# alibaba-damo-academy/Inferix

Measured on AMD Instinct MI355X. Metric: latent_frames_per_sec, higher is better.
Workload: dtype bf16; 1 GPU; Self-Forcing 480p bf16 (Wan2.1-T2V-1.3B causal DiT, 30 layers), block_size=3, 21 latent frames = 7 blocks x (4 denoise + 1 context) generator forwards, KV prefix 4680..32760 keys in the KV manager's cache (identity page map; page-table form: `streaming_steady`); `value` counts the generator calls (SURVEY 8d), the per-block VAE decode of config 2 is measured beside it under --full (`per_block_decod; batch=1, parallelism=single, layers=30, pair_forwards=True, pair_mode=streams

## Files before the change

### include/inferix_hip.h

```cpp
#ifndef INFERIX_HIP_H
#define INFERIX_HIP_H

#include <stdint.h>

#ifdef __cplusplus
extern "C" {
#endif

#define IFX_OK 0
#define IFX_EINVAL (-1)
#define IFX_ELAUNCH (-2)
#define IFX_EUNSUP (-3)

typedef uint16_t ifx_bf16;

#define IFX_ABI_MINOR 7
int ifx_version(void);
const char* ifx_last_error(void);
const char* ifx_arch(void);
int ifx_set_option(const char* key, int32_t value);
int ifx_get_option(const char* key, int32_t* value);
int32_t ifx_device_error(int32_t clear);

typedef struct {
  ifx_bf16* k;
  ifx_bf16* v;
  const int32_t* page_table;
  int32_t page_size;
  int32_t num_slots;
  int32_t kv_heads;
  int32_t head_dim;
  int32_t seg_split;
  int32_t seg_delta;
} ifx_kv_view;

int ifx_attn_fwd_paged(const ifx_bf16* q, ifx_bf16* out, float* lse, const ifx_kv_view* kv,
                       int32_t q_rows, int32_t heads, int32_t kv_start, int32_t kv_len, float scale,
                       void* stream);

int32_t ifx_attn_split_plan(int32_t q_rows, int32_t heads, int32_t kv_start, int32_t kv_len,
                            int64_t* workspace_bytes);
int ifx_attn_fwd_paged_split(const ifx_bf16* q, ifx_bf16* out, float* lse, const ifx_kv_view* kv,
                             int32_t q_rows, int32_t heads, int32_t kv_start, int32_t kv_len, float scale,
                             int32_t num_splits, void* workspace, int64_t workspace_bytes, void* stream);

int ifx_attn_fwd_paged_ld(const ifx_bf16* q, int32_t ldq, ifx_bf16* out, int32_t ldo, float* lse, const ifx_kv_view* kv,
                          int32_t q_rows, int32_t heads, int32_t kv_start, int32_t kv_len, float scale, int32_t num_splits,
                          void* workspace, int64_t workspace_bytes, void* stream);

int ifx_attn_fwd_dedup(const ifx_bf16* q, ifx_bf16* out, const ifx_kv_view* kv, int32_t q_rows, int32_t heads, int32_t kv_len,
                       int32_t last_key_multiplicity, float scale, void* stream);

int ifx_attn_fwd_ranges(const ifx_bf16* q, int32_t ldq, ifx_bf16* out, int32_t ldo, const ifx_kv_view* kv, int32_t q_rows,
                        int32_t heads, int32_t n_ranges, const int32_t* q_ranges, const int32_t* k_ranges, float scale,
                        void* stream);

int ifx_attn_fwd_partial(const ifx_bf16* q, const ifx_kv_view* kv, int32_t q_rows, int32_t heads, int32_t kv_start,
                         int32_t kv_len, float scale, int32_t num_splits, void* workspace, int64_t workspace_bytes,
                         int32_t slot_base, int32_t slot_cap, int32_t* slots_used, void* stream);
int ifx_attn_merge_partials(const void* workspace, int32_t slot_cap, int32_t slots_used, ifx_bf16* out, float* lse,
                            int32_t q_rows, int32_t heads, void* stream);

int ifx_lse_merge(ifx_bf16* out_a, float* lse_a, const ifx_bf16* out_b, const float* lse_b,
                  int32_t rows, int32_t heads, void* stream);

typedef struct {
  const double* freqs;
  int32_t max_pos;
  int32_t start_frame;
  int32_t height, width;
  int32_t hw_offset;
  int32_t hw_local;
  float q_scale;
  int32_t flags;
} ifx_rope_grid;

int ifx_rmsnorm_rope_kv_append(const ifx_bf16* qkv, int32_t qkv_row_stride, ifx_bf16* q_out,
                               const ifx_bf16* wq, const ifx_bf16* wk, const ifx_rope_grid* rope,
                               const ifx_kv_view* kv, int32_t local_start, int32_t rows,
                               int32_t dim, float eps, void* stream);

int ifx_rmsnorm(const ifx_bf16* x, int32_t x_row_stride, ifx_bf16* y, int32_t y_row_stride,
                const ifx_bf16* w, int32_t rows, int32_t dim, float eps, void* stream);

enum { IFX_LN_PLAIN = 0, IFX_LN_AFFINE = 1, IFX_LN_MODULATE = 2 };
int ifx_layernorm(const ifx_bf16* x, ifx_bf16* y, int32_t rows, int32_t dim, float eps, int32_t mode,
                  const ifx_bf16* gamma, const ifx_bf16* beta, const ifx_bf16* mod,
                  int32_t mod_slots, int32_t shift_slot, int32_t scale_slot, int32_t rows_per_group,
                  void* stream);

enum { IFX_EPI_BIAS = 0, IFX_EPI_GELU_TANH = 1, IFX_EPI_RESIDUAL = 2, IFX_EPI_GATE_RES = 3, IFX_EPI_GELU_ERF = 4 };
typedef struct {
  int32_t epilogue;
  const ifx_bf16* residual;
  int32_t ld_res;
  const ifx_bf16* mod;
  int32_t mod_slots;
  int32_t gate_slot;
  int32_t rows_per_group;
  ifx_bf16* y2;
  int32_t ldy2;
  int32_t split_col;
} ifx_epilogue;
int ifx_gemm_bf16(const ifx_bf16* x, int32_t ldx, const ifx_bf16* w, const ifx_bf16* bias,
                  ifx_bf16* y, int32_t ldy, int32_t M, int32_t N, int32_t K,
                  const ifx_epilogue* epi, void* stream);

int64_t ifx_gemm_workspace_bytes(int32_t M, int32_t N, int32_t K);
int ifx_gemm_bf16_ws(const ifx_bf16* x, int32_t ldx, const ifx_bf16* w, const ifx_bf16* bias, ifx_bf16* y, int32_t ldy,
                     int32_t M, int32_t N, int32_t K, const ifx_epilogue* epi, void* workspace, int64_t workspace_bytes,
                     void* stream);

enum { IFX_Q_FP8_E4M3 = 0, IFX_Q_INT8 = 1 };
int ifx_quant_per_token(const ifx_bf16* x, int32_t ldx, void* q, int32_t ldq, float* scale, int32_t rows,
                        int32_t K, int32_t format, void* stream);
int ifx_gemm_q8(const void* xq, int32_t ldx, const float* x_scale, const void* wq, const float* w_scale,
                const ifx_bf16* bias, ifx_bf16* y, int32_t ldy, int32_t M, int32_t N, int32_t K, int32_t format,
                const ifx_epilogue* epi, void* stream);
int64_t ifx_gemm_q8_workspace_bytes(int32_t M, int32_t N, int32_t K);
int ifx_gemm_q8_ws(const void* xq, int32_t ldx, const float* x_scale, const void* wq, const float* w_scale, const ifx_bf16* bias,
                   ifx_bf16* y, int32_t ldy, int32_t M, int32_t N, int32_t K, int32_t format, const ifx_epilogue* epi,
                   void* workspace, int64_t workspace_bytes, void* stream);
int ifx_layernorm_quant(const ifx_bf16* x, void* q, int32_t ldq, float* scale, int32_t rows, int32_t dim, float eps,
                        int32_t mode, const ifx_bf16* gamma, const ifx_bf16* beta, const ifx_bf16* mod, int32_t mod_slots,
                        int32_t shift_slot, int32_t scale_slot, int32_t rows_per_group, int32_t format, void* stream);

int ifx_gemm_q8_quant_out(const void* xq, int32_t ldx, const float* x_scale, const void* wq, const float* w_scale,
                          const ifx_bf16* bias, void* yq, int32_t ldyq, int32_t M, int32_t N, int32_t K, int32_t format,
                          const ifx_epilogue* epi, const float* out_divisor, int32_t via_bf16, void* stream);
int ifx_layernorm_quant_static(const ifx_bf16* x, void* q, int32_t ldq, const float* divisors, int32_t n_out, int32_t rows,
                               int32_t dim, float eps, int32_t mode, const ifx_bf16* gamma, const ifx_bf16* beta,
                               int32_t via_bf16, void* stream);

int ifx_quant_static(const ifx_bf16* x, int32_t ldx, void* q, int32_t ldq, const float* divisor, int32_t divisor_len,
                     float* row_scale, int32_t rows, int32_t K, int32_t format, int32_t via_bf16, void* stream);
int ifx_quant_per_tensor(const ifx_bf16* x, int32_t ldx, void* q, int32_t ldq, float* row_scale, void* amax_workspace,
                         int32_t rows, int32_t K, int32_t format, void* stream);

int ifx_kv_roll(const ifx_kv_view* kv, int32_t sink_tokens, int32_t evicted, int32_t rolled,
                ifx_bf16* scratch, void* stream);

int ifx_kv_scatter_shards(const ifx_bf16* gathered, int32_t world, int32_t frames, int32_t hw_local,
                          int32_t frame_tokens, int32_t local_start, const ifx_kv_view* kv, void* stream);

#define IFX_MAX_PEERS 8
#define IFX_PEER_HANDLE_BYTES 64
typedef struct {
  int32_t count;
  ifx_bf16* k[IFX_MAX_PEERS];
  ifx_bf16* v[IFX_MAX_PEERS];
} ifx_peer_caches;
typedef struct {
  int32_t count;
  int32_t* flags[IFX_MAX_PEERS];
} ifx_peer_flags;
int ifx_peer_alloc(int64_t bytes, int32_t fine_grained, void** ptr);
int ifx_peer_free(void* ptr);
int ifx_peer_export(const void* ptr, uint8_t* handle, int64_t* offset);
int ifx_peer_open(const uint8_t* handle, void** ptr);
int ifx_peer_close(void* ptr);
int ifx_rmsnorm_rope_kv_push(const ifx_bf16* kv_rows, int32_t kv_row_stride, const ifx_bf16* wk, const ifx_rope_grid* rope,
                             const ifx_peer_caches* peers, const ifx_kv_view* geometry, int32_t local_start, int32_t frame_tokens,
                             int32_t slot_hw_local, int32_t slot_hw_offset, int32_t rows, int32_t dim, float eps, void* stream);
int ifx_peer_signal(const ifx_peer_flags* peers, int32_t index, int32_t value, void* stream);
int ifx_peer_wait(const int32_t* flags, int32_t count, int32_t value, int32_t timeout_ms, int32_t* status, void* stream);

typedef struct {
  const ifx_bf16* x;
  int64_t in_frame_stride;
  const int32_t* in_slots;
  int32_t hs, ws, cin, upsample;
  const ifx_bf16* w;
  const ifx_bf16* bias;
  int32_t kt, ks;
  ifx_bf16* y;
  int64_t out_frame_stride;
  const int32_t* out_slots;
  int32_t cout, t_out;
  const ifx_bf16* residual;
  const void* zero_page;
  int32_t in_planar;
} ifx_conv3d_desc;
int ifx_conv3d_cl(const ifx_conv3d_desc* desc, void* stream);

#define IFX_NORM_SILU 1
#define IFX_NORM_OUT_PLANAR 2
int ifx_rmsnorm_cl(const ifx_bf16* x, const ifx_bf16* gamma, ifx_bf16* y, int64_t out_frame_stride,
                   const int32_t* out_slots, int32_t frames, int32_t frame_pixels, int32_t channels,
                   int32_t flags, void* stream);

int ifx_softmax_rows(const ifx_bf16* scores, ifx_bf16* probs, int32_t rows, int32_t cols, int32_t ld, float scale,
                     void* stream);

int ifx_t5_attention(const ifx_bf16* q, int32_t ldq, const ifx_bf16* k, int32_t ldk, const ifx_bf16* v, int32_t ldv,
                     ifx_bf16* out, int32_t ldo, const ifx_bf16* rel_bias, const int32_t* seq_lens, int32_t batch,
                     int32_t seq_len_padded, int32_t heads, void* stream);

int ifx_t5_gated_gelu(const ifx_bf16* gate_fc1, ifx_bf16* h, int32_t rows, int32_t ffn, void* stream);

typedef struct {
  const ifx_bf16* in;
  int32_t ld_in, rows, layout, q_heads, kv_heads, head_dim;
  const float* rope;
  const float *qn_w, *qn_b, *kn_w, *kn_b;
  const ifx_bf16 *xn_w, *xn_b;
  float eps;
  int32_t layernorm_1p;
  ifx_bf16* q_out;
  int32_t ld_q;
  ifx_bf16* qx_out;
  int32_t ld_qx;
  ifx_bf16* k_out;
  ifx_bf16* v_out;
  int32_t ld_kv, kv_head_stride;
  int32_t row0, split, row1;
  float q_scale;
  int32_t rope_half;
  int32_t q_group;
  int64_t q_group_stride;
} ifx_magi_head_prep_desc;
int ifx_magi_head_prep(const ifx_magi_head_prep_desc* desc, void* stream);

int ifx_magi_gate_norm_residual(const ifx_bf16* x, int32_t ldx, const ifx_bf16* residual, int32_t ld_res,
                                const int32_t* condition_map, const ifx_bf16* gate, int32_t ld_gate, const float* norm_w,
                                const float* norm_b, int32_t layernorm_1p, ifx_bf16* y, int32_t ldy, int32_t rows, int32_t dim,
                                float eps, void* stream);

enum { IFX_ACT_SILU = 0, IFX_ACT_TANH = 1 };
int ifx_act_rows(const ifx_bf16* x, ifx_bf16* y, int64_t n, int32_t mode, void* stream);
int ifx_silu_and_mul(const ifx_bf16* x, int32_t ldx, ifx_bf16* y, int32_t ldy, void* q, int32_t ldq, const float* divisor,
                     int32_t divisor_len, int32_t rows, int32_t f, void* stream);
int ifx_kv_split_rows(const ifx_bf16* kv, ifx_bf16* k_cache, ifx_bf16* v_cache, int32_t rows, int32_t heads, int32_t row0,
                      int32_t split, int32_t row1, void* stream);

int ifx_vit_head_prep(ifx_bf16* qkv, int32_t ld, const ifx_bf16* sin_table, const ifx_bf16* cos_table, int32_t batch, int32_t tokens,
                      int32_t heads, int32_t cls_tokens, int32_t do_norm, int32_t do_rope, float eps, void* stream);
// ... 14 lines not shown
```

### inferix_amd/_hip.py

```python
from __future__ import annotations

import ctypes as C
import os
from typing import Optional

import torch

_HERE = os.path.dirname(os.path.abspath(__file__))
LIB_PATH = os.environ.get("IFX_HIP_LIB", os.path.join(_HERE, "libinferix_hip.so"))

IFX_LN_PLAIN, IFX_LN_AFFINE, IFX_LN_MODULATE = 0, 1, 2
IFX_EPI_BIAS, IFX_EPI_GELU_TANH, IFX_EPI_RESIDUAL, IFX_EPI_GATE_RES, IFX_EPI_GELU_ERF = 0, 1, 2, 3, 4
IFX_ACT_SILU, IFX_ACT_TANH = 0, 1
IFX_Q_FP8_E4M3, IFX_Q_INT8 = 0, 1


class HipLibraryMissing(RuntimeError):
    pass


class HipKernelError(RuntimeError):
    pass


class KvView(C.Structure):
    _fields_ = [("k", C.c_void_p), ("v", C.c_void_p), ("page_table", C.c_void_p),
                ("page_size", C.c_int32), ("num_slots", C.c_int32), ("kv_heads", C.c_int32),
                ("head_dim", C.c_int32), ("seg_split", C.c_int32), ("seg_delta", C.c_int32)]


class RopeGrid(C.Structure):
    _fields_ = [("freqs", C.c_void_p), ("max_pos", C.c_int32), ("start_frame", C.c_int32),
                ("height", C.c_int32), ("width", C.c_int32), ("hw_offset", C.c_int32),
                ("hw_local", C.c_int32), ("q_scale", C.c_float), ("flags", C.c_int32)]


class Conv3dDesc(C.Structure):
    _fields_ = [("x", C.c_void_p), ("in_frame_stride", C.c_int64), ("in_slots", C.POINTER(C.c_int32)),
                ("hs", C.c_int32), ("ws", C.c_int32), ("cin", C.c_int32), ("upsample", C.c_int32),
                ("w", C.c_void_p), ("bias", C.c_void_p), ("kt", C.c_int32), ("ks", C.c_int32),
                ("y", C.c_void_p), ("out_frame_stride", C.c_int64), ("out_slots", C.POINTER(C.c_int32)),
                ("cout", C.c_int32), ("t_out", C.c_int32), ("residual", C.c_void_p), ("zero_page", C.c_void_p),
                ("in_planar", C.c_int32)]


class Epilogue(C.Structure):
    _fields_ = [("epilogue", C.c_int32), ("residual", C.c_void_p), ("ld_res", C.c_int32),
                ("mod", C.c_void_p), ("mod_slots", C.c_int32), ("gate_slot", C.c_int32),
                ("rows_per_group", C.c_int32), ("y2", C.c_void_p), ("ldy2", C.c_int32), ("split_col", C.c_int32)]


class MagiHeadPrepDesc(C.Structure):
    _fields_ = [("inp", C.c_void_p), ("ld_in", C.c_int32), ("rows", C.c_int32), ("layout", C.c_int32),
                ("q_heads", C.c_int32), ("kv_heads", C.c_int32), ("head_dim", C.c_int32), ("rope", C.c_void_p),
                ("qn_w", C.c_void_p), ("qn_b", C.c_void_p), ("kn_w", C.c_void_p), ("kn_b", C.c_void_p),
                ("xn_w", C.c_void_p), ("xn_b", C.c_void_p), ("eps", C.c_float), ("layernorm_1p", C.c_int32),
                ("q_out", C.c_void_p), ("ld_q", C.c_int32), ("qx_out", C.c_void_p), ("ld_qx", C.c_int32),
                ("k_out", C.c_void_p), ("v_out", C.c_void_p), ("ld_kv", C.c_int32), ("kv_head_stride", C.c_int32),
                ("row0", C.c_int32), ("split", C.c_int32), ("row1", C.c_int32), ("q_scale", C.c_float), ("rope_half", C.c_int32),
                ("q_group", C.c_int32), ("q_group_stride", C.c_int64)]


IFX_MAX_PEERS, IFX_PEER_HANDLE_BYTES = 8, 64


class PeerCaches(C.Structure):
    _fields_ = [("count", C.c_int32), ("k", C.c_void_p * IFX_MAX_PEERS), ("v", C.c_void_p * IFX_MAX_PEERS)]


class PeerFlags(C.Structure):
    _fields_ = [("count", C.c_int32), ("flags", C.c_void_p * IFX_MAX_PEERS)]


_vp, _i32, _f32 = C.c_void_p, C.c_int32, C.c_float
SIGNATURES = {
    "ifx_version": (C.c_int, []),
    "ifx_last_error": (C.c_char_p, []),
    "ifx_arch": (C.c_char_p, []),
    "ifx_set_option": (C.c_int, [C.c_char_p, _i32]),
    "ifx_get_option": (C.c_int, [C.c_char_p, C.POINTER(_i32)]),
    "ifx_device_error": (_i32, [_i32]),
    "ifx_attn_fwd_paged": (C.c_int, [_vp, _vp, _vp, C.POINTER(KvView), _i32, _i32, _i32, _i32, _f32, _vp]),
    "ifx_attn_split_plan": (_i32, [_i32, _i32, _i32, _i32, C.POINTER(C.c_int64)]),
    "ifx_attn_fwd_paged_split": (C.c_int, [_vp, _vp, _vp, C.POINTER(KvView), _i32, _i32, _i32, _i32, _f32, _i32, _vp,
                                           C.c_int64, _vp]),
    "ifx_conv3d_cl": (C.c_int, [C.POINTER(Conv3dDesc), _vp]),
    "ifx_rmsnorm_cl": (C.c_int, [_vp, _vp, _vp, C.c_int64, C.POINTER(_i32), _i32, _i32, _i32, _i32, _vp]),
    "ifx_softmax_rows": (C.c_int, [_vp, _vp, _i32, _i32, _i32, _f32, _vp]),
    "ifx_t5_attention": (C.c_int, [_vp, _i32, _vp, _i32, _vp, _i32, _vp, _i32, _vp, _vp, _i32, _i32, _i32, _vp]),
    "ifx_t5_gated_gelu": (C.c_int, [_vp, _vp, _i32, _i32, _vp]),
    "ifx_kv_scatter_shards": (C.c_int, [_vp, _i32, _i32, _i32, _i32, _i32, C.POINTER(KvView), _vp]),
    "ifx_peer_alloc": (C.c_int, [C.c_int64, _i32, C.POINTER(C.c_void_p)]),
    "ifx_peer_free": (C.c_int, [_vp]),
    "ifx_peer_export": (C.c_int, [_vp, C.c_char_p, C.POINTER(C.c_int64)]),
    "ifx_peer_open": (C.c_int, [C.c_char_p, C.POINTER(C.c_void_p)]),
    "ifx_peer_close": (C.c_int, [_vp]),
    "ifx_rmsnorm_rope_kv_push": (C.c_int, [_vp, _i32, _vp, C.POINTER(RopeGrid), C.POINTER(PeerCaches), C.POINTER(KvView), _i32, _i32,
                                           _i32, _i32, _i32, _i32, _f32, _vp]),
    "ifx_peer_signal": (C.c_int, [C.POINTER(PeerFlags), _i32, _i32, _vp]),
    "ifx_peer_wait": (C.c_int, [_vp, _i32, _i32, _i32, _vp, _vp]),
    "ifx_attn_fwd_partial": (C.c_int, [_vp, C.POINTER(KvView), _i32, _i32, _i32, _i32, _f32, _i32, _vp, C.c_int64, _i32,
                                       _i32, C.POINTER(_i32), _vp]),
    "ifx_attn_merge_partials": (C.c_int, [_vp, _i32, _i32, _vp, _vp, _i32, _i32, _vp]),
    "ifx_lse_merge": (C.c_int, [_vp, _vp, _vp, _vp, _i32, _i32, _vp]),
    "ifx_rmsnorm_rope_kv_append": (C.c_int, [_vp, _i32, _vp, _vp, _vp, C.POINTER(RopeGrid), C.POINTER(KvView),
                                             _i32, _i32, _i32, _f32, _vp]),
    "ifx_rmsnorm": (C.c_int, [_vp, _i32, _vp, _i32, _vp, _i32, _i32, _f32, _vp]),
    "ifx_layernorm": (C.c_int, [_vp, _vp, _i32, _i32, _f32, _i32, _vp, _vp, _vp, _i32, _i32, _i32, _i32, _vp]),
    "ifx_gemm_bf16": (C.c_int, [_vp, _i32, _vp, _vp, _vp, _i32, _i32, _i32, _i32, C.POINTER(Epilogue), _vp]),
    "ifx_kv_roll": (C.c_int, [C.POINTER(KvView), _i32, _i32, _i32, _vp, _vp]),
    "ifx_quant_per_token": (C.c_int, [_vp, _i32, _vp, _i32, _vp, _i32, _i32, _i32, _vp]),
    "ifx_layernorm_quant": (C.c_int, [_vp, _vp, _i32, _vp, _i32, _i32, _f32, _i32, _vp, _vp, _vp, _i32, _i32, _i32, _i32, _i32, _vp]),
    "ifx_gemm_q8": (C.c_int, [_vp, _i32, _vp, _vp, _vp, _vp, _vp, _i32, _i32, _i32, _i32, _i32, C.POINTER(Epilogue), _vp]),
    "ifx_gemm_q8_ws": (C.c_int, [_vp, _i32, _vp, _vp, _vp, _vp, _vp, _i32, _i32, _i32, _i32, _i32, C.POINTER(Epilogue), _vp, C.c_int64, _vp]),
    "ifx_gemm_q8_workspace_bytes": (C.c_int64, [_i32, _i32, _i32]),
    "ifx_attn_fwd_paged_ld": (C.c_int, [_vp, _i32, _vp, _i32, _vp, C.POINTER(KvView), _i32, _i32, _i32, _i32, _f32, _i32, _vp,
                                        C.c_int64, _vp]),
    "ifx_gemm_q8_quant_out": (C.c_int, [_vp, _i32, _vp, _vp, _vp, _vp, _vp, _i32, _i32, _i32, _i32, _i32, C.POINTER(Epilogue), _vp, _i32, _vp]),
    "ifx_layernorm_quant_static": (C.c_int, [_vp, _vp, _i32, _vp, _i32, _i32, _i32, _f32, _i32, _vp, _vp, _i32, _vp]),
    "ifx_quant_static": (C.c_int, [_vp, _i32, _vp, _i32, _vp, _i32, _vp, _i32, _i32, _i32, _i32, _vp]),
    "ifx_quant_per_tensor": (C.c_int, [_vp, _i32, _vp, _i32, _vp, _vp, _i32, _i32, _i32, _vp]),
    "ifx_magi_head_prep": (C.c_int, [C.POINTER(MagiHeadPrepDesc), _vp]),
    "ifx_magi_gate_norm_residual": (C.c_int, [_vp, _i32, _vp, _i32, _vp, _vp, _i32, _vp, _vp, _i32, _vp, _i32, _i32, _i32, _f32,
                                              _vp]),
    "ifx_act_rows": (C.c_int, [_vp, _vp, C.c_int64, _i32, _vp]),
    "ifx_silu_and_mul": (C.c_int, [_vp, _i32, _vp, _i32, _vp, _i32, _vp, _i32, _i32, _i32, _vp]),
    "ifx_kv_split_rows": (C.c_int, [_vp, _vp, _vp, _i32, _i32, _i32, _i32, _i32, _vp]),
    "ifx_attn_fwd_dedup": (C.c_int, [_vp, _vp, C.POINTER(KvView), _i32, _i32, _i32, _i32, _f32, _vp]),
    "ifx_attn_fwd_ranges": (C.c_int, [_vp, _i32, _vp, _i32, C.POINTER(KvView), _i32, _i32, _i32, C.POINTER(_i32), C.POINTER(_i32), _f32, _vp]),
    "ifx_gemm_workspace_bytes": (C.c_int64, [_i32, _i32, _i32]),
    "ifx_gemm_bf16_ws": (C.c_int, [_vp, _i32, _vp, _vp, _vp, _i32, _i32, _i32, _i32, C.POINTER(Epilogue), _vp, C.c_int64, _vp]),
    "ifx_vit_head_prep": (C.c_int, [_vp, _i32, _vp, _vp, _i32, _i32, _i32, _i32, _i32, _i32, _f32, _vp]),
    "ifx_vit_attention": (C.c_int, [_vp, _i32, _vp, _i32, _vp, _i32, _vp, _i32, _i32, _i32, _i32, _vp]),
    "ifx_vit_unpatch_conv": (C.c_int, [_vp, _i32, _i32, _i32, _vp, _vp, _vp, _i32, _i32, _i32, _i32, _i32, _i32, _i32, _i32, _vp]),
    "ifx_vit_tile_blend": (C.c_int, [_vp, _vp, _vp, _vp] + [_i32] * 14 + [_vp]),
}

_lib: Optional[C.CDLL] = None
ABI_MINOR = 7


def load() -> C.CDLL:
    global _lib
    if _lib is not None:
        return _lib
    if not os.path.exists(LIB_PATH):
        raise HipLibraryMissing(
            f"{LIB_PATH} not found: build it with `python -c 'import __graft_entry__ as g; g.build()'` "
            "(hipcc --offload-arch=gfx950).  inferix_amd has no CPU or eager fallback.")
    lib = C.CDLL(LIB_PATH)
    for name, (res, args) in SIGNATURES.items():
        fn = getattr(lib, name)
        fn.restype = res
        fn.argtypes = args
    got = (lib.ifx_version() >> 8) & 255
    if got != ABI_MINOR:
        raise HipLibraryMissing(f"{LIB_PATH} has ABI minor {got}, these bindings are for {ABI_MINOR} (include/inferix_hip.h "
                                "IFX_ABI_MINOR): rebuild with __graft_entry__.build()")
    _lib = lib
    return lib


def check(rc: int, what: str) -> None:
    if rc != 0:
        msg = load().ifx_last_error().decode("utf-8", "replace")
        raise HipKernelError(f"{what} failed (code {rc}): {msg}")


def version() -> str:
    v = load().ifx_version()
    return f"{v >> 16}.{(v >> 8) & 255}.{v & 255}"
```

### inferix_amd/csrc/ifx_gemm.hip

```cpp
#include "ifx_gemm_epilogue.h"

namespace ifx {

constexpr int BM = 128, BN = 128, BK = 64;

template <int EPI>
__global__ __launch_bounds__(256, 2) void gemm_bf16_kernel(const unsigned short* __restrict__ x, int ldx,
                                                           const unsigned short* __restrict__ w,
                                                           unsigned short* __restrict__ y, int ldy, int M, int N,
                                                           int K, int tiles_m, int tiles_n, EpiArgs ea) {
  extern __shared__ __attribute__((aligned(16))) unsigned char smem[];
  const int tid = threadIdx.x, lane = tid & 63, wave = tid >> 6;
  const int wm = wave & 1, wn = wave >> 1;
  constexpr int GM = 8;
  const int total = tiles_m * tiles_n, per_xcd = (total + 7) / 8;
  const int t_id = (blockIdx.x & 7) * per_xcd + (blockIdx.x >> 3);
  if ((int)(blockIdx.x >> 3) >= per_xcd || t_id >= total) return;
  const int grp_sz = GM * tiles_n;
  const int first_m = (t_id / grp_sz) * GM;
  const int gm = min(GM, tiles_m - first_m);
  const int rem = t_id % grp_sz;
  const int tile_m = first_m + rem % gm, tile_n = rem / gm;
  const int m_base = tile_m * BM, n_base = tile_n * BN;

  const unsigned short* gx[4];
  const unsigned short* gw[4];
  int lds_off[4];
#pragma unroll
  for (int p = 0; p < 4; ++p) {
    const int q = tid + 256 * p, row = q >> 3, c = q & 7;
    const int mr = min(m_base + row, M - 1), nr = min(n_base + row, N - 1);
    gx[p] = x + (size_t)mr * ldx + c * 8;
    gw[p] = w + (size_t)nr * K + c * 8;
    lds_off[p] = row * 128 + ((c ^ (row & 7)) << 4);
  }
  u32x4 rx[4], rw[4];
  auto gload = [&](int kt) {
#pragma unroll
    for (int p = 0; p < 4; ++p) {
      rx[p] = *reinterpret_cast<const u32x4*>(gx[p] + (size_t)kt * BK);
      rw[p] = *reinterpret_cast<const u32x4*>(gw[p] + (size_t)kt * BK);
    }
  };
  auto lstore = [&](int buf) {
    unsigned char* bx = smem + buf * 32768;
    unsigned char* bw = bx + 16384;
#pragma unroll
    for (int p = 0; p < 4; ++p) {
      *reinterpret_cast<u32x4*>(bx + lds_off[p]) = rx[p];
      *reinterpret_cast<u32x4*>(bw + lds_off[p]) = rw[p];
    }
  };

  f32x4 acc[4][4];
#pragma unroll
  for (int i = 0; i < 4; ++i)
#pragma unroll
    for (int j = 0; j < 4; ++j) acc[i][j] = f32x4{0.f, 0.f, 0.f, 0.f};

  const int KT = K / BK;
  gload(0);
  lstore(0);
  __syncthreads();

  const int fr = lane & 15, fq = lane >> 4;
  for (int kt = 0; kt < KT; ++kt) {
    const int buf = kt & 1;
    if (kt + 1 < KT) gload(kt + 1);
    const unsigned char* bx = smem + buf * 32768;
    const unsigned char* bw = bx + 16384;
#pragma unroll
    for (int ks = 0; ks < 2; ++ks) {
      bf16x8 a[4], b[4];
      const int c = ks * 4 + fq;
#pragma unroll
      for (int i = 0; i < 4; ++i) {
        const int row = wn * 64 + i * 16 + fr;
        a[i] = *reinterpret_cast<const bf16x8*>(bw + row * 128 + ((c ^ (row & 7)) << 4));
      }
#pragma unroll
      for (int j = 0; j < 4; ++j) {
        const int row = wm * 64 + j * 16 + fr;
        b[j] = *reinterpret_cast<const bf16x8*>(bx + row * 128 + ((c ^ (row & 7)) << 4));
      }
#pragma unroll
      for (int i = 0; i < 4; ++i)
#pragma unroll
        for (int j = 0; j < 4; ++j)
          acc[i][j] = __builtin_amdgcn_mfma_f32_16x16x32_bf16(a[i], b[j], acc[i][j], 0, 0, 0);
    }
    if (kt + 1 < KT) lstore(buf ^ 1);
    __syncthreads();
  }

#pragma unroll
  for (int j = 0; j < 4; ++j) {
    const int m = m_base + wm * 64 + j * 16 + fr;
    if (m >= M) continue;
    const unsigned short* gate_row = nullptr;
    if (EPI == IFX_EPI_GATE_RES)
      gate_row = ea.mod + ((size_t)(m / ea.rows_per_group) * ea.mod_slots + ea.gate_slot) * N;
#pragma unroll
    for (int i = 0; i < 4; ++i) {
      const int n = n_base + wn * 64 + i * 16 + fq * 4;
      if (n >= N) continue;
      float v[4] = {acc[i][j][0], acc[i][j][1], acc[i][j][2], acc[i][j][3]};
      if (ea.bias) {
        const u16x4 bv = *reinterpret_cast<const u16x4*>(ea.bias + n);
#pragma unroll
        for (int e = 0; e < 4; ++e) v[e] += bf2f(bv[e]);
      }
      u16x4 vb, rv = {}, gv = {};
#pragma unroll
      for (int e = 0; e < 4; ++e) vb[e] = f2bf(v[e]);
      if (EPI == IFX_EPI_RESIDUAL || EPI == IFX_EPI_GATE_RES)
        rv = *reinterpret_cast<const u16x4*>(ea.residual + (size_t)m * ea.ld_res + n);
      if (EPI == IFX_EPI_GATE_RES) gv = *reinterpret_cast<const u16x4*>(gate_row + n);
      const u16x4 o = epi_combine<EPI, 4>(vb, rv, gv, ea.gelu_erf());
      *reinterpret_cast<u16x4*>(y + (size_t)m * ldy + n) = o;
    }
  }
}

}

using namespace ifx;

extern "C" int ifx_gemm_bf16_ws(const ifx_bf16* x, int32_t ldx, const ifx_bf16* w, const ifx_bf16* bias, ifx_bf16* y,
                                int32_t ldy, int32_t M, int32_t N, int32_t K, const ifx_epilogue* epi, void* workspace,
                                int64_t workspace_bytes, void* stream) {
  IFX_REQUIRE(x && w && y && M >= 0 && N > 0 && K > 0, "ifx_gemm_bf16: null/empty operand");
  IFX_REQUIRE(K % BK == 0, "ifx_gemm_bf16: K (%d) must be a multiple of %d", K, BK);
  IFX_REQUIRE(N % 4 == 0 && ldx % 8 == 0 && ldy % 4 == 0, "ifx_gemm_bf16: N %% 4, ldx %% 8, ldy %% 4 required");
  int mode;
  EpiArgsP ea;
  if (const int rc = resolve_epilogue(epi, bias, "ifx_gemm_bf16", &mode, &ea)) return rc;
  IFX_REQUIRE(!(((uintptr_t)x | (uintptr_t)w) & 15), "ifx_gemm_bf16: x and w must be 16-byte aligned");
  IFX_REQUIRE(!(((uintptr_t)y | (uintptr_t)bias | (uintptr_t)ea.residual | (uintptr_t)ea.mod) & 7),
              "ifx_gemm_bf16: y, bias, residual and mod must be 8-byte aligned");
  if (M == 0) return IFX_OK;
  GemmRequest r = gemm_request(M, N, K, mode, ea, y, ldy, workspace, workspace_bytes);
  r.y2 = epi != nullptr && epi->y2 != nullptr;
  const GemmPlan plan = gemm_plan(r, gemm_variant(), gemm_small_split());
  IFX_REQUIRE(plan.path != kGemmPathRefuseY2,
              "ifx_gemm_bf16: the second destination (y2) needs the bias epilogue, N %% 64 == 0, 8-byte aligned bias and the ping-pong tiles");
  hipStream_t s = (hipStream_t)stream;
  void* const ws = plan.ws_bytes > 0 ? workspace : nullptr;
  switch (plan.path) {
    case kGemmPathW4: return launch_gemm_w4(x, ldx, w, y, ldy, M, N, K, mode, ea, s, plan.ks, ws);
    case kGemmPathPp:
      if (plan.y2) ea.y2 = epi->y2, ea.ldy2 = epi->ldy2, ea.split_col = epi->split_col;
      return launch_gemm_pp(x, ldx, w, y, ldy, M, N, K, mode, ea, s, plan.tj, plan.ks, ws);
    case kGemmPathLdsDma: return launch_gemm_lds_dma(plan.tile, x, ldx, w, y, ldy, M, N, K, mode, ea, s);
    default: break;
  }
  const int tiles_m = (M + BM - 1) / BM, tiles_n = (N + BN - 1) / BN;
  const dim3 grid(((tiles_m * tiles_n + 7) / 8) * 8), block(256);
  const size_t lds = 65536;
  const int rc = dispatch_epilogue(mode, "ifx_gemm_bf16", [&](auto epi_c) {
    constexpr int E = decltype(epi_c)::value;
    static bool attr_set = false;
    if (!attr_set) {
      (void)hipFuncSetAttribute((const void*)gemm_bf16_kernel<E>, hipFuncAttributeMaxDynamicSharedMemorySize, (int)lds);
      attr_set = true;
    }
    hipLaunchKernelGGL((gemm_bf16_kernel<E>), grid, block, lds, s, x, ldx, w, y, ldy, M, N, K, tiles_m, tiles_n, ea);
  });
  if (rc != IFX_OK) return rc;
  return check_launch("ifx_gemm_bf16");
}

extern "C" int ifx_gemm_bf16(const ifx_bf16* x, int32_t ldx, const ifx_bf16* w, const ifx_bf16* bias, ifx_bf16* y,
                             int32_t ldy, int32_t M, int32_t N, int32_t K, const ifx_epilogue* epi, void* stream) {
  return ifx_gemm_bf16_ws(x, ldx, w, bias, y, ldy, M, N, K, epi, nullptr, 0, stream);
}

extern "C" int64_t ifx_gemm_workspace_bytes(int32_t M, int32_t N, int32_t K) {
  if (M <= 0 || N <= 0 || K <= 0) return 0;
  const GemmVariant v = gemm_variant_row(gemm_variant());
  const bool mult64 = N % 64 == 0 && K % 64 == 0;
  if (v.kind == kGemmPp && v.takes_ws) return (int64_t)gemm_pp_workspace_bytes(M, N, K);
  if (v.kind == kGemmPpStreamK) return mult64 ? (int64_t)gemm_pp_stream_k_workspace_bytes() : 0;
  if (v.kind == kGemmPpKParts) return mult64 && (K / 64) % v.ks == 0 ? (int64_t)gemm_pp_small_workspace_bytes(M, N, v.ks) : 0;
  GemmRequest r{M, N, K, IFX_EPI_BIAS};
  r.ws_bytes = INT64_MAX;
  return gemm_plan(r, gemm_variant(), gemm_small_split()).ws_bytes;
}
```

### inferix_amd/csrc/ifx_gemm_epilogue.h

```cpp
#pragma once
#include <type_traits>

#include "ifx_common.h"
#include "ifx_gemm_plan.h"

namespace ifx {

struct EpiArgs {
  const unsigned short* bias = nullptr;
  const unsigned short* residual = nullptr;
  int ld_res = 0;
  const unsigned short* mod = nullptr;
  int mod_slots = 1, gate_slot = 0, rows_per_group = 1;
  __host__ __device__ bool gelu_erf() const { return gate_slot != 0; }
};

struct EpiArgsQ : EpiArgs {
  const float* sa = nullptr;
  const float* sw = nullptr;
  const float* qdiv = nullptr;
  int q_via_bf16 = 0;
};

struct EpiArgsP : EpiArgsQ {
  unsigned short* y2 = nullptr;
  int ldy2 = 0, split_col = 0;
};

template <int W>
using u16v = unsigned short __attribute__((ext_vector_type(W)));

template <int EPI, int W>
__device__ __forceinline__ u16v<W> epi_combine(const u16v<W> vv, const u16v<W> rv, const u16v<W> gv, const bool erf) {
  u16v<W> o;
  if constexpr (EPI == IFX_EPI_BIAS) {
    o = vv;
  } else if constexpr (EPI == IFX_EPI_GELU_TANH) {
    if (erf) {
#pragma unroll
      for (int e = 0; e < W; ++e) o[e] = f2bf(gelu_erf_f(bf2f(vv[e])));
    } else {
#pragma unroll
      for (int e = 0; e < W; ++e) o[e] = f2bf(gelu_tanh_fast(bf2f(vv[e])));
    }
  } else if constexpr (EPI == IFX_EPI_RESIDUAL) {
#pragma unroll
    for (int e = 0; e < W; ++e) o[e] = f2bf(bf2f(rv[e]) + bf2f(vv[e]));
  } else {
    static_assert(EPI == IFX_EPI_GATE_RES, "epilogue");
#pragma unroll
    for (int e = 0; e < W; ++e) o[e] = f2bf(bf2f(rv[e]) + rbf(bf2f(vv[e]) * bf2f(gv[e])));
  }
  return o;
}

template <int EPI, int W>
__device__ __forceinline__ u16v<W> epi_apply(const u16v<W> vv, int m, int n, int N, const EpiArgs& ea) {
  u16v<W> rv = vv, gv = vv;
  if constexpr (EPI == IFX_EPI_RESIDUAL || EPI == IFX_EPI_GATE_RES)
    rv = *reinterpret_cast<const u16v<W>*>(ea.residual + (size_t)m * ea.ld_res + n);
  if constexpr (EPI == IFX_EPI_GATE_RES)
    gv = *reinterpret_cast<const u16v<W>*>(ea.mod + ((size_t)(m / ea.rows_per_group) * ea.mod_slots + ea.gate_slot) * N + n);
  return epi_combine<EPI, W>(vv, rv, gv, ea.gelu_erf());
}

template <int EPI>
__device__ __forceinline__ void epi_store_row(const u16x8 vv, int m, int n, int N, const EpiArgs& ea, unsigned short* __restrict__ y,
                                              int ldy) {
  *reinterpret_cast<u16x8*>(y + (size_t)m * ldy + n) = epi_apply<EPI, 8>(vv, m, n, N, ea);
}


template <typename F>
static inline int dispatch_epilogue(int mode, const char* what, F&& launch) {
  switch (mode) {
    case IFX_EPI_BIAS: launch(std::integral_constant<int, IFX_EPI_BIAS>{}); return IFX_OK;
    case IFX_EPI_GELU_TANH: launch(std::integral_constant<int, IFX_EPI_GELU_TANH>{}); return IFX_OK;
    case IFX_EPI_RESIDUAL: launch(std::integral_constant<int, IFX_EPI_RESIDUAL>{}); return IFX_OK;
    case IFX_EPI_GATE_RES: launch(std::integral_constant<int, IFX_EPI_GATE_RES>{}); return IFX_OK;
    default: set_error("%s: unknown epilogue %d", what, mode); return IFX_EINVAL;
  }
}

static inline int resolve_epilogue(const ifx_epilogue* epi, const unsigned short* bias, const char* who, int* mode, EpiArgs* ea) {
  *mode = epi ? epi->epilogue : IFX_EPI_BIAS;
  *ea = EpiArgs{};
  ea->bias = bias;
  if (*mode == IFX_EPI_GELU_ERF) {
    *mode = IFX_EPI_GELU_TANH;
    ea->gate_slot = 1;
  }
  if (*mode == IFX_EPI_RESIDUAL || *mode == IFX_EPI_GATE_RES) {
    IFX_REQUIRE(epi->residual && epi->ld_res % 4 == 0, "%s: residual epilogue needs residual/ld_res", who);
    ea->residual = epi->residual;
    ea->ld_res = epi->ld_res;
  }
  if (*mode == IFX_EPI_GATE_RES) {
    IFX_REQUIRE(epi->mod && epi->rows_per_group > 0 && epi->gate_slot >= 0 && epi->gate_slot < epi->mod_slots,
                "%s: gate epilogue needs mod/mod_slots/gate_slot/rows_per_group", who);
    ea->mod = epi->mod;
    ea->mod_slots = epi->mod_slots;
    ea->gate_slot = epi->gate_slot;
    ea->rows_per_group = epi->rows_per_group;
  }
  return IFX_OK;
}

static inline PpOperands pp_operands(const EpiArgs& ea) {
  return {!((uintptr_t)ea.bias & 7), !((uintptr_t)ea.residual & 15) && ea.ld_res % 8 == 0, !((uintptr_t)ea.mod & 15), ea.rows_per_group};
}

static inline GemmRequest gemm_request(int M, int N, int K, int mode, const EpiArgs& ea, const void* y, int ldy, const void* workspace,
                                       int64_t workspace_bytes) {
  GemmRequest r;
  r.M = M, r.N = N, r.K = K, r.mode = mode;
  r.wide_ok = N % 8 == 0 && ldy % 8 == 0 && (ea.residual == nullptr || ea.ld_res % 8 == 0) &&
              !(((uintptr_t)y | (uintptr_t)ea.residual | (uintptr_t)ea.mod) & 15);
  r.ops = pp_operands(ea);
  r.ws_bytes = workspace != nullptr ? workspace_bytes : 0;
  return r;
}

int launch_gemm_lds_dma(int tile, const unsigned short* x, int ldx, const unsigned short* w, unsigned short* y, int ldy, int M, int N,
                        int K, int mode, const EpiArgs& ea, hipStream_t s);
int launch_gemm_w4(const unsigned short* x, int ldx, const unsigned short* w, unsigned short* y, int ldy, int M, int N, int K,
                   int mode, const EpiArgs& ea, hipStream_t s, int splits, void* workspace);
int launch_gemm_pp(const unsigned short* x, int ldx, const unsigned short* w, unsigned short* y, int ldy, int M, int N, int K,
                   int mode, const EpiArgsP& ea, hipStream_t s, int tj, int ks, void* workspace, int q8_int8 = 0);

}
```

### inferix_amd/csrc/ifx_gemm_pp.hip

```cpp
#include <limits.h>
#include <stdlib.h>

#include "ifx_gemm_epilogue.h"

#ifndef IFX_PP_TRACE
#define IFX_PP_TRACE 0
#endif
#ifndef IFX_PP_LAB
#define IFX_PP_LAB IFX_PP_TRACE
#endif


namespace ifx {

namespace gpp {
constexpr int BN = 256, BK = 64;
constexpr int SLOT = 16384, STAGE = 4 * SLOT, SCRATCH = 2 * STAGE;
constexpr int LDS_BYTES = SCRATCH + 32768;
constexpr int X_UP = 0, W_LO = SLOT, W_HI = 2 * SLOT, X_DN = 3 * SLOT;
constexpr int LX_STAGE = 16384, LX_DN = 8192, LW_BASE = 32768, LW_STAGE = 32768;
typedef int v4i __attribute__((ext_vector_type(4)));
typedef int v8i __attribute__((ext_vector_type(8)));
typedef int v16i __attribute__((ext_vector_type(16)));
typedef __attribute__((address_space(3))) void* lds_ptr_t;

__device__ __forceinline__ void dma16(v4i rsrc, unsigned lds, int voff, int soff) {
  asm volatile("s_mov_b32 m0, %0\n\ts_nop 0\n\tbuffer_load_dwordx4 %1, %2, %3 offen lds"
               :
               : "s"(lds), "v"(voff), "s"(rsrc), "s"(soff)
               : "memory");
}
__device__ __forceinline__ v4i make_rsrc(const void* base, unsigned num_bytes) {
  const unsigned long long a = (unsigned long long)base;
  v4i r;
  r[0] = (int)(unsigned)a;
  r[1] = (int)((unsigned)(a >> 32) & 0xffffu);
  r[2] = (int)num_bytes;
  r[3] = 0x00020000;
  return r;
}
template <int N>
__device__ __forceinline__ void wait_vm() {
  asm volatile("s_waitcnt vmcnt(%0)" ::"n"(N) : "memory");
}
template <int N, bool ON>
__device__ __forceinline__ void wait_vm_if() {
  if constexpr (ON) wait_vm<N>();
}
__device__ __forceinline__ void wait_lds() { __builtin_amdgcn_s_waitcnt(0xC07F); }

struct Cursor {
  int i, kt, g, rot, k0, len;
  int kb;
  unsigned stg;
  v4i rs;
};
}

template <int EPI, int TJ, int KS, int Q8 = 0, int LW = 0>
__global__ __launch_bounds__(LW ? 768 : 512, LW ? 3 : 2) void gemm_pp_kernel(const unsigned short* __restrict__ x, int ldx,
                                                         const unsigned short* __restrict__ w, unsigned short* __restrict__ y,
                                                         int ldy, int M, int N, int K, int tiles_m, int total, int per_xcd,
                                                         int wg_per_xcd, EpiArgsP ea, unsigned long long* __restrict__ trace, int dbg,
                                                         float* __restrict__ ws_part, unsigned* __restrict__ ws_flag,
                                                         unsigned* __restrict__ err_word, long long spin_ticks) {
  using namespace gpp;
  static_assert(!LW || (TJ == 2 && KS == 1 && Q8 == 0), "the loader-wave form is the unsplit bf16 128-token tile");
  dbg = IFX_PP_LAB ? dbg : (dbg & 32);
  constexpr int BM = 64 * TJ;
  constexpr int GM = 4;
  constexpr bool RES = EPI == IFX_EPI_RESIDUAL || EPI == IFX_EPI_GATE_RES;
  extern __shared__ __attribute__((aligned(16))) unsigned char smem[];
  const int tid = threadIdx.x, lane = tid & 63;
  const int wave = __builtin_amdgcn_readfirstlane(tid >> 6);
  const int grp = wave >> 2, w4 = wave & 3;
  constexpr int ES = Q8 ? 1 : 2;
  const unsigned char* const xb = reinterpret_cast<const unsigned char*>(x);
  const unsigned char* const wb = reinterpret_cast<const unsigned char*>(w);
  constexpr bool SK = KS == 0;
  constexpr int KSD = KS > 0 ? KS : 1;
  const int S = K * ES / 128;
  const int KT = S / KSD;
  const int tiles_n = total / KSD / tiles_m;

  const int xcd = blockIdx.x & 7, slot_i = blockIdx.x >> 3;
  const int id_first = xcd * per_xcd + slot_i;
  const int id_end = min(xcd * per_xcd + per_xcd, total);
  if (!SK && id_first >= id_end) return;
  const int sk_P = (int)gridDim.x, sk_p = xcd * (sk_P >> 3) + slot_i;
  auto sk_start = [&](int q) __attribute__((always_inline)) { return (int)((long)q * total * S / sk_P); };
  const int sk_u0 = SK ? sk_start(sk_p) : 0, sk_u1 = SK ? sk_start(sk_p + 1) : 0;
  const int sk_t0 = SK ? sk_u0 / S : 0;
  const int n_my = SK ? (sk_u1 - 1) / S - sk_t0 + 1 : (id_end - id_first + wg_per_xcd - 1) / wg_per_xcd;
  const int G = SK ? sk_u1 - sk_u0 : n_my * KT;
  auto item_split = [&](int i) __attribute__((always_inline)) { return KS > 1 ? (id_first + i * wg_per_xcd) % KSD : 0; };
  auto item_tile = [&](int i) __attribute__((always_inline)) { return SK ? sk_t0 + i : (id_first + i * wg_per_xcd) / KSD; };
  auto item_k0 = [&](int i) __attribute__((always_inline)) { return SK ? (i == 0 ? sk_u0 - sk_t0 * S : 0) : item_split(i) * KT; };
  auto item_len = [&](int i) __attribute__((always_inline)) {
    return SK ? min(S, sk_u1 - (sk_t0 + i) * S) - (i == 0 ? sk_u0 - sk_t0 * S : 0) : KT;
  };
  auto item_dumps = [&](int i) __attribute__((always_inline)) { return SK ? (i == 0 && sk_u0 > sk_t0 * S) : (KS > 1 && item_split(i) >= 1); };
  auto item_parts = [&](int i) __attribute__((always_inline)) {
    if (!SK) return KS > 1 ? KS - 1 : 0;
    const int t_end = (sk_t0 + i + 1) * S;
    int n = 0;
    while (sk_p + 1 + n < sk_P && sk_start(sk_p + 1 + n) < t_end) ++n;
    return sk_u1 < t_end ? n : 0;
  };
  auto tile_base = [&](int i, int& m_base, int& n_base) __attribute__((always_inline)) {
    const int t_id = item_tile(i);
    const int grp_sz = GM * tiles_n;
    const int first_m = (t_id / grp_sz) * GM;
    const int gm = min(GM, tiles_m - first_m);
    const int rem = t_id % grp_sz;
    m_base = (first_m + rem % gm) * BM;
    n_base = (rem / gm) * BN;
  };

  const int r8 = lane >> 3, pc = lane & 7;
  const int prow = w4 * 8 + r8;
  const int ld_op = grp == 0 ? K : ldx;
  const int voff = prow * ld_op * ES + ((pc ^ ((prow >> 1) & 7)) << 4);
  const int voff_w = LW ? prow * K * ES + ((pc ^ ((prow >> 1) & 7)) << 4) : 0;
  const int voff_x = LW ? prow * ldx * ES + ((pc ^ ((prow >> 1) & 7)) << 4) : 0;
  const unsigned lds_piece0 = (unsigned)(unsigned long long)(lds_ptr_t)smem + w4 * 1024;
  auto cur_desc = [&](Cursor& c, bool is_w) __attribute__((always_inline)) {
    int mb, nb;
    tile_base(c.i, mb, nb);
    if (dbg & 1) mb = nb = 0;
    c.rot = (!SK && (dbg & 4)) ? ((nb / BN) * 3) % KT : 0;
    c.k0 = item_k0(c.i);
    c.len = item_len(c.i);
    c.kb = c.k0 * 128;
    if (is_w) c.rs = make_rsrc(wb + (size_t)nb * K * ES, (unsigned)min(((long)N - nb) * (long)K * ES, 0xffffffffL));
    else c.rs = make_rsrc(xb + (size_t)mb * ldx * ES, (unsigned)min(((long)M - mb - 1) * (long)ldx * ES + (long)K * ES, 0xffffffffL));
  };
  auto cur_init = [&](Cursor& c, bool is_w) __attribute__((always_inline)) {
    c.i = 0, c.kt = 0, c.g = 0, c.stg = 0;
    cur_desc(c, is_w);
  };
  auto cur_next = [&](Cursor& c, bool is_w) __attribute__((always_inline)) {
    ++c.g;
    if constexpr (LW) c.stg = !is_w ? c.stg ^ LX_STAGE : c.stg == 2 * LW_STAGE ? 0 : c.stg + LW_STAGE;
    else c.stg ^= STAGE;
    c.kb += 128;
    if (++c.kt == c.len) {
      c.kt = 0;
      if (++c.i < n_my) cur_desc(c, is_w);
    }
  };
  auto issue = [&](const Cursor& c, bool is_w, int slot, int row0, int pieces) __attribute__((always_inline)) {
    const int kk = c.kt + c.rot;
    const int kb = IFX_PP_LAB ? ((!SK && kk >= KT ? kk - KT : kk) + c.k0) * 128 : c.kb;
    const unsigned p = lds_piece0 + c.stg + slot;
    if ((dbg & 8) && c.g >= 2) return;
    const int vo = LW ? (is_w ? voff_w : voff_x) : voff;
    const int pitch = LW ? (is_w ? K : ldx) : ld_op;
#pragma unroll
    for (int q = 0; q < 4; ++q)
      if (q < pieces) dma16(c.rs, p + q * 4096, vo, kb + (row0 + q * 32) * pitch * ES);
  };
  const bool opw = grp == 0;
  auto req_w = [&](Cursor& c) __attribute__((always_inline)) {
    if constexpr (!LW) issue(c, opw, W_LO, 0, 4), issue(c, opw, W_HI, 128, 4), cur_next(c, opw);
  };
  auto req_x = [&](Cursor& c, int slot, int row0) __attribute__((always_inline)) {
    if constexpr (!LW) issue(c, opw, slot, row0, TJ), cur_next(c, opw);
  };
  Cursor ca, cb;
  cur_init(ca, opw);
  cur_init(cb, opw);

  constexpr bool MF16 = Q8 == 0;
  const int l31 = lane & 31, hi = lane >> 5, l15 = lane & 15, q4 = lane >> 4;
  int lane_ks[4];
#pragma unroll
  for (int ks = 0; ks < 4; ++ks)
    lane_ks[ks] = MF16 ? l15 * 128 + ((((4 * ks + q4) & 7) ^ ((l15 >> 1) & 7)) << 4)
                       : l31 * 128 + (((2 * ks + hi) ^ ((l31 >> 1) & 7)) << 4);
  const int w_frag_off = (w4 >> 1) * SLOT + (w4 & 1) * 8192 + W_LO;
  const int x_frag_off = grp == 0 ? X_UP : X_DN;
  bf16x8 fx[4][TJ], fw[4][2], fx16[2 * TJ][2];
  int rg = 0;
  int rw = 0;
  const int w_off_lw = (w4 >> 1) * SLOT + (w4 & 1) * 8192, x_off_lw = grp == 0 ? 0 : LX_DN;
  auto read_frags = [&]() __attribute__((always_inline)) {
    const unsigned char* st = smem + (rg & 1) * STAGE;
    const unsigned char* const wst = LW ? smem + LW_BASE + rw * LW_STAGE + w_off_lw : st + w_frag_off;
    const unsigned char* const xst = LW ? smem + (rg & 1) * LX_STAGE + x_off_lw : st + x_frag_off;
    if constexpr (LW) rw = rw == 2 ? 0 : rw + 1;
    if constexpr (MF16) {
#pragma unroll
      for (int kk = 0; kk < 2; ++kk) {
#pragma unroll
        for (int c = 0; c < 4; ++c) fw[c][kk] = *reinterpret_cast<const bf16x8*>(wst + lane_ks[kk] + c * 2048);
#pragma unroll
        for (int t = 0; t < 2 * TJ; ++t) fx16[t][kk] = *reinterpret_cast<const bf16x8*>(xst + lane_ks[kk] + t * 2048);
      }
    } else {
#pragma unroll
      for (int ks = 0; ks < 4; ++ks) {
#pragma unroll
        for (int i = 0; i < 2; ++i) fw[ks][i] = *reinterpret_cast<const bf16x8*>(st + w_frag_off + lane_ks[ks] + i * 4096);
#pragma unroll
        for (int j = 0; j < TJ; ++j) fx[ks][j] = *reinterpret_cast<const bf16x8*>(st + x_frag_off + lane_ks[ks] + j * 4096);
      }
    }
    ++rg;
  };

  f32x16 acc[2][TJ];
  f32x4 acc16[4][2 * TJ];
  auto quad = [&](int i, int j, int g) __attribute__((always_inline)) {
    if constexpr (MF16) return acc16[g][2 * j + i];
    else return f32x4{acc[i][j][4 * g], acc[i][j][4 * g + 1], acc[i][j][4 * g + 2], acc[i][j][4 * g + 3]};
  };
  auto mfma16 = [&](bool first) __attribute__((always_inline)) {
    const f32x4 z = {0.f, 0.f, 0.f, 0.f};
#pragma unroll
    for (int kk = 0; kk < 2; ++kk)
// ... 173 lines not shown
        const int g_lo = min(e_m0, M - 1) / ea.rows_per_group, g_hi = m_hi / ea.rows_per_group;
        e_split = (g_lo + 1) * ea.rows_per_group;
        e_gate[0] = *reinterpret_cast<const u32x4*>(ea.mod + ((size_t)g_lo * ea.mod_slots + ea.gate_slot) * N + e_n0 + cc * 8);
        e_gate[1] = *reinterpret_cast<const u32x4*>(ea.mod + ((size_t)g_hi * ea.mod_slots + ea.gate_slot) * N + e_n0 + cc * 8);
      }
    }
    unsigned char* const wr = MF16 ? tw + (ln & 15) * 128 + ((ln >> 4) & 1) * 8 : tw + l31 * 128 + hi * 8;
    const unsigned char* const rd = tw + rr * 128;
    const bool to_y2 = ea.y2 != nullptr && e_n0 >= ea.split_col;
    const int ldo = to_y2 ? ea.ldy2 : ldy;
    unsigned short* const yrow = (to_y2 ? ea.y2 - ea.split_col : y) + (size_t)(e_m0 + rr) * ldo + e_n0 + cc * 8;
    if constexpr (PRIV) {
      asm volatile("" : "+v"(q_bias[0]), "+v"(q_bias[1]), "+v"(q_sw[0]), "+v"(q_sw[1]), "+v"(q_sw[2]), "+v"(q_sw[3]));
    } else {
#pragma unroll
      for (int i = 0; i < (MF16 ? 1 : 2); ++i)
#pragma unroll
        for (int g = 0; g < 4; ++g) asm volatile("" : "+v"(e_bias[i][g]));
    }
    if constexpr (Q8) {
      if constexpr (!PRIV) {
#pragma unroll
        for (int i = 0; i < 2; ++i)
#pragma unroll
          for (int g = 0; g < 4; ++g) asm volatile("" : "+v"(e_sw[i][g]));
      }
#pragma unroll
      for (int j = 0; j < TJ; ++j) asm volatile("" : "+v"(e_sa[j]));
      if constexpr (EPI == IFX_EPI_GELU_TANH) asm volatile("" : "+v"(e_qd[0]), "+v"(e_qd[1]));
    }
#pragma unroll
    for (int j = 0; j < TJ; ++j) {
      if (j + 1 < TJ) fetch_res(j + 1);
#pragma unroll
      for (int i = 0; i < 2; ++i) {
#pragma unroll
        for (int g = 0; g < 4; ++g) {
          const f32x4 aq = quad(i, j, g);
          float v[4] = {aq[0], aq[1], aq[2], aq[3]};
          if constexpr (Q8 == 2 && KS <= 1) {
#pragma unroll
            for (int e = 0; e < 4; ++e) v[e] = (float)__builtin_bit_cast(int, v[e]);
          }
          if constexpr (KS > 1) {
            f32x4 pq[KSD - 1];
#pragma unroll
            for (int q = 0; q < KSD - 1; ++q)
              pq[q] = __builtin_bit_cast(f32x4, __builtin_amdgcn_raw_buffer_load_b128(rs_ws, ln * 16 + ((i * TJ + j) * 4 + g) * 1024,
                                                                                      part_so + q * (BM * BN * 4), 16));
            if constexpr (Q8 == 2) {
              int vi[4];
#pragma unroll
              for (int e = 0; e < 4; ++e) vi[e] = __builtin_bit_cast(int, v[e]);
#pragma unroll
              for (int q = 0; q < KSD - 1; ++q)
#pragma unroll
                for (int e = 0; e < 4; ++e) {
                  const float pe = pq[q][e];
                  vi[e] += __builtin_bit_cast(int, pe);
                }
#pragma unroll
              for (int e = 0; e < 4; ++e) v[e] = (float)vi[e];
            } else {
#pragma unroll
              for (int q = 0; q < KSD - 1; ++q)
#pragma unroll
                for (int e = 0; e < 4; ++e) v[e] += pq[q][e];
            }
          }
          if constexpr (SK) {
            for (int q = 0; q < part_n; ++q) {
              const f32x4 pq = __builtin_bit_cast(f32x4, __builtin_amdgcn_raw_buffer_load_b128(
                                                             rs_ws, ln * 16 + ((i * TJ + j) * 4 + g) * 1024, part_so + q * (BM * BN * 4), 16));
#pragma unroll
              for (int e = 0; e < 4; ++e) v[e] += pq[e];
            }
          }
          if constexpr (Q8) {
            f32x4 swv;
            if constexpr (PRIV) {
#pragma unroll
              for (int e = 0; e < 4; ++e)
                swv[e] = __builtin_bit_cast(float, __builtin_amdgcn_ds_bpermute(((ln & 32) | (i * 4 + g)) << 2, q_sw[e]));
            } else {
              swv = e_sw[i][g];
            }
#pragma unroll
            for (int e = 0; e < 4; ++e) v[e] = __fmul_rn(v[e], __fmul_rn(e_sa[j], swv[e]));
          }
          u32x2 b;
          if constexpr (PRIV) {
            b[0] = (unsigned)__builtin_amdgcn_ds_bpermute(((ln & 32) | (i * 4 + g)) << 2, q_bias[0]);
            b[1] = (unsigned)__builtin_amdgcn_ds_bpermute(((ln & 32) | (i * 4 + g)) << 2, q_bias[1]);
          } else {
            b = e_bias[MF16 ? 0 : i][g];
          }
          v[0] += __builtin_bit_cast(float, b[0] << 16);
          v[1] += __builtin_bit_cast(float, b[0] & 0xffff0000u);
          v[2] += __builtin_bit_cast(float, b[1] << 16);
          v[3] += __builtin_bit_cast(float, b[1] & 0xffff0000u);
          u16x4 o;
#pragma unroll
          for (int e = 0; e < 4; ++e) o[e] = f2bf(v[e]);
          if constexpr (MF16) *reinterpret_cast<u16x4*>(wr + i * 2048 + (((2 * g + hi) ^ cc) << 4)) = o;
          else *reinterpret_cast<u16x4*>(wr + (((i * 4 + g) ^ (l31 & 7)) << 4)) = o;
        }
      }
      wait_lds();
#pragma unroll
      for (int p = 0; p < 4; ++p) {
        const int mrow = p * 8 + rr;
        const int m = e_m0 + j * 32 + mrow;
        const u16x8 vv = *reinterpret_cast<const u16x8*>(rd + p * 1024 + ((cc ^ (mrow & 7)) << 4));
        if constexpr (RES) asm volatile("" : "+v"(e_res[j & 1][p]));
        if constexpr (EPI == IFX_EPI_GATE_RES) {
          if (j == 0 && p == 0) asm volatile("" : "+v"(e_gate[0]), "+v"(e_gate[1]));
        }
        u16x8 o;
        if constexpr (EPI == IFX_EPI_GELU_TANH) {
          if (ea.gelu_erf()) {
#pragma unroll
            for (int e = 0; e < 8; ++e) o[e] = f2bf(gelu_erf_f(bf2f(vv[e])));
          } else {
#pragma unroll
            for (int e = 0; e < 8; ++e) o[e] = f2bf(gelu_tanh_fast(bf2f(vv[e])));
          }
        } else {
          u16x8 rv = vv, gv = vv;
          if constexpr (RES) rv = __builtin_bit_cast(u16x8, e_res[j & 1][p]);
          if constexpr (EPI == IFX_EPI_GATE_RES) gv = __builtin_bit_cast(u16x8, m >= e_split ? e_gate[1] : e_gate[0]);
          o = epi_combine<EPI, 8>(vv, rv, gv, false);
        }
        if constexpr (Q8 && EPI == IFX_EPI_GELU_TANH) {
          if (ea.qdiv != nullptr) {
            unsigned wq[2];
#pragma unroll
            for (int h = 0; h < 2; ++h) {
              float t[4];
#pragma unroll
              for (int e = 0; e < 4; ++e) {
                const float q = fminf(fmaxf(bf2f(o[4 * h + e]) / e_qd[h][e], -448.0f), 448.0f);
                t[e] = ea.q_via_bf16 ? rbf(q) : q;
              }
              unsigned pk = __builtin_amdgcn_cvt_pk_fp8_f32(t[0], t[1], 0u, false);
              wq[h] = __builtin_amdgcn_cvt_pk_fp8_f32(t[2], t[3], pk, true);
            }
            if (m < M && n_ok)
              *reinterpret_cast<u32x2*>(reinterpret_cast<unsigned char*>(y) + (size_t)(e_m0 + rr + j * 32 + p * 8) * ldy + e_n0 + cc * 8) =
                  u32x2{wq[0], wq[1]};
            continue;
          }
        }
        if (m < M && n_ok) *reinterpret_cast<u16x8*>(yrow + (size_t)(j * 32 + p * 8) * ldo) = o;
      }
    }
  };

#if IFX_PP_TRACE
  unsigned long long seg[6] = {0, 0, 0, 0, 0, 0};
  unsigned long long t_last = __builtin_readcyclecounter();
  int seg_i = 0;
#define PP_STAMP()                                                 \
  do {                                                             \
    const unsigned long long t_now = __builtin_readcyclecounter(); \
    seg[seg_i] += t_now - t_last;                                  \
    t_last = t_now;                                                \
    seg_i = seg_i == 5 ? 0 : seg_i + 1;                            \
  } while (0)
#else
#define PP_STAMP() \
  do {             \
  } while (0)
#endif
#ifndef IFX_PP_STAGGER
#define IFX_PP_STAGGER 0
#endif
  auto roles = [&](auto stagger_tag) __attribute__((always_inline)) {
  constexpr bool reads_first = decltype(stagger_tag)::value;

  int kt = 0, it = 0;
  int klen = item_len(0);
  if (grp == 0) {
    req_w(ca);
    wait_vm_if<0, !LW>();
    __builtin_amdgcn_s_barrier();
    for (int g = 0; g < G; ++g) {
      PP_STAMP();
      const bool epi = g > 0 && kt == 0;
      const bool issued = ca.g < G;
      const bool early_reads = reads_first && !epi;
      if (epi && KS != 1 && item_dumps(it - 1)) {
        if (issued) req_w(ca);
        PP_STAMP();
        dump_partial(it - 1);
        wait_vm<0>();
        flag_pending = flag_of(it - 1) + 1;
        PP_STAMP();
        read_frags();
      } else if (epi) {
        if (KS != 1) consumer_sync(it - 1);
        epilogue(it - 1, [&]() __attribute__((always_inline)) {
          if (issued) req_w(ca);
          PP_STAMP();
        });
        PP_STAMP();
        read_frags();
      } else if (early_reads) {
        read_frags();
        if (issued) req_w(ca);
        PP_STAMP();
        PP_STAMP();
      } else {
        if (issued) req_w(ca);
        PP_STAMP();
        PP_STAMP();
        read_frags();
      }
      wait_lds();
      __builtin_amdgcn_sched_barrier(0);
      PP_STAMP();
      __builtin_amdgcn_s_barrier();
      __builtin_amdgcn_sched_barrier(0);
      PP_STAMP();
      if (KS != 1 && flag_pending) {
        if (wave == 0 && !(dbg & 32)) __hip_atomic_store(ws_flag + flag_pending - 1, 1u, __ATOMIC_RELAXED, __HIP_MEMORY_SCOPE_AGENT);
        flag_pending = 0;
      }
      if (!(dbg & 2)) {
        if (kt == 0) mfma_first();
        else mfma_next();
      }
      if (++kt == klen) kt = 0, ++it, klen = it < n_my ? item_len(it) : 0;
      wait_vm_if<0, !LW>();
      __builtin_amdgcn_sched_barrier(0);
      PP_STAMP();
      __builtin_amdgcn_s_barrier();
      __builtin_amdgcn_sched_barrier(0);
    }
    if (KS != 1 && item_dumps(it - 1)) {
      dump_partial(it - 1);
      wait_vm<0>();
      flag_pending = flag_of(it - 1) + 1;
    } else {
      if (KS != 1) consumer_sync(it - 1);
      epilogue(it - 1, [&]() __attribute__((always_inline)) {});
    }
    if (KS != 1) {
      __builtin_amdgcn_s_barrier();
      if (flag_pending && wave == 0 && !(dbg & 32)) __hip_atomic_store(ws_flag + flag_pending - 1, 1u, __ATOMIC_RELAXED, __HIP_MEMORY_SCOPE_AGENT);
    }
  } else {
    req_x(cb, X_UP, 0);
    req_x(ca, X_DN, 32 * TJ);
    if (cb.g < G) req_x(cb, X_UP, 0);
    if (G > 1) wait_vm_if<2 * TJ, !LW>();
    else wait_vm_if<TJ, !LW>();
    __builtin_amdgcn_s_barrier();
    if (G > 1) wait_vm_if<TJ, !LW>();
    else wait_vm_if<0, !LW>();
    __builtin_amdgcn_s_barrier();
    for (int g = 0; g < G; ++g) {
      PP_STAMP();
      const bool lower = ca.g < G, upper = cb.g < G;
      if (reads_first) {
        read_frags();
        if (lower) req_x(ca, X_DN, 32 * TJ);
        if (upper) req_x(cb, X_UP, 0);
        PP_STAMP();
        PP_STAMP();
      } else {
        if (lower) req_x(ca, X_DN, 32 * TJ);
        if (upper) req_x(cb, X_UP, 0);
        PP_STAMP();
        PP_STAMP();
        read_frags();
      }
      wait_lds();
      if (upper) wait_vm_if<2 * TJ, !LW>();
      else if (lower) wait_vm_if<TJ, !LW>();
      else wait_vm_if<0, !LW>();
      __builtin_amdgcn_sched_barrier(0);
      PP_STAMP();
      __builtin_amdgcn_s_barrier();
      __builtin_amdgcn_sched_barrier(0);
      PP_STAMP();
      if (!(dbg & 2)) {
        if (kt == 0) mfma_first();
        else mfma_next();
      }
      if (++kt == klen) kt = 0, ++it, klen = it < n_my ? item_len(it) : 0;
      if (upper) wait_vm_if<TJ, !LW>();
      else wait_vm_if<0, !LW>();
      __builtin_amdgcn_sched_barrier(0);
      PP_STAMP();
      if (kt == 0) {
        if (KS != 1 && item_dumps(it - 1)) {
          dump_partial(it - 1);
          wait_vm<0>();
        } else {
          if (KS != 1) consumer_sync(it - 1);
          epilogue(it - 1, [&]() __attribute__((always_inline)) {});
        }
      }
      if (g + 1 < G || KS != 1) {
        __builtin_amdgcn_s_barrier();
        __builtin_amdgcn_sched_barrier(0);
      }
    }
  }
  };
  auto loader = [&]() __attribute__((always_inline)) {
    Cursor cw, cu, cl;
    cur_init(cw, true), cur_init(cu, false), cur_init(cl, false);
    auto w_step = [&]() __attribute__((always_inline)) {
      issue(cw, true, LW_BASE, 0, 4), issue(cw, true, LW_BASE + SLOT, 128, 4), cur_next(cw, true);
    };
    auto up_step = [&]() __attribute__((always_inline)) { issue(cu, false, 0, 0, TJ), cur_next(cu, false); };
    auto lo_step = [&]() __attribute__((always_inline)) { issue(cl, false, LX_DN, 32 * TJ, TJ), cur_next(cl, false); };
    w_step(), up_step();
    if (G > 1) w_step();
    lo_step();
    if (G > 1) up_step(), wait_vm<8 + 2 * TJ>();
    else wait_vm<TJ>();
    __builtin_amdgcn_s_barrier();
    __builtin_amdgcn_sched_barrier(0);
#if IFX_PP_TRACE
    t_last = __builtin_readcyclecounter();
#endif
    for (int g = 0; g < G; ++g) {
      const bool more = g + 1 < G, more2 = g + 2 < G;
      if (more2) w_step();
      PP_STAMP();
      if (more2) wait_vm<TJ + 8>();
      else if (more) wait_vm<TJ>();
      else wait_vm<0>();
      __builtin_amdgcn_sched_barrier(0);
      PP_STAMP();
      __builtin_amdgcn_s_barrier();
      __builtin_amdgcn_sched_barrier(0);
      PP_STAMP();
      if (more) lo_step();
      if (more2) up_step();
      PP_STAMP();
      if (more2) wait_vm<8 + 2 * TJ>();
      else if (more) wait_vm<TJ>();
      else wait_vm<0>();
      __builtin_amdgcn_sched_barrier(0);
      PP_STAMP();
      __builtin_amdgcn_s_barrier();
      __builtin_amdgcn_sched_barrier(0);
      PP_STAMP();
    }
  };
  if (LW && grp == 2) loader();
  else if (IFX_PP_STAGGER && (w4 & 1)) roles(std::true_type{});
  else roles(std::false_type{});
#if IFX_PP_TRACE
  if (trace != nullptr && blockIdx.x == 0 && lane == 0 && (wave & 3) == 0) {
#pragma unroll
    for (int k = 0; k < 6; ++k) trace[grp * 8 + k] = seg[k];
    trace[grp * 8 + 6] = (unsigned long long)G;
  }
#endif
}

int launch_gemm_pp(const unsigned short* x, int ldx, const unsigned short* w, unsigned short* y, int ldy, int M, int N, int K,
                   int mode, const EpiArgsP& ea, hipStream_t s, int tj, int ks, void* workspace, int q8_int8) {
  using namespace gpp;
  const bool q8 = ea.sa != nullptr;
  IFX_REQUIRE(ea.y2 == nullptr || !(q8 || ea.split_col <= 0 || ea.split_col % BN != 0 || ea.split_col >= N || ea.ldy2 % 8 != 0 || ((uintptr_t)ea.y2 & 15)),
              "ifx_gemm_bf16: the second destination needs bf16 operands, 0 < split_col < N a multiple of %d, ldy2 %% 8 == 0 and a 16-byte aligned y2", BN);
  IFX_REQUIRE(!q8 || !(K % 128 != 0 || ldx % 16 != 0 || ((uintptr_t)ea.sw & 15) || ((uintptr_t)ea.qdiv & 15)),
              "ifx_gemm_q8: the ping-pong tile needs K %% 128 == 0, ldx %% 16 == 0 and 16-byte aligned scale vectors (K = %d, ldx = %d)", K, ldx);
  IFX_REQUIRE(N % 64 == 0 && K % 64 == 0, "ifx_gemm_bf16: the ping-pong tile needs N and K to be multiples of 64 (N = %d, K = %d)", N, K);
  IFX_REQUIRE(mode != IFX_EPI_GATE_RES || ea.rows_per_group >= 32 * tj,
              "ifx_gemm_bf16: the ping-pong tile needs gate groups of at least %d rows (rows_per_group = %d)", 32 * tj, ea.rows_per_group);
  IFX_REQUIRE(pp_epilogue_fits(mode, pp_operands(ea), 0),
              "ifx_gemm_bf16: the ping-pong tile needs 8-byte aligned bias and 16-byte aligned residual / gate rows");
  static int cu_of_dev[16] = {0};
  int dev = 0, n_cu = 0;
  if (hipGetDevice(&dev) == hipSuccess && dev >= 0 && dev < 16) {
    if (cu_of_dev[dev] == 0) {
      int v = 0;
      cu_of_dev[dev] = hipDeviceGetAttribute(&v, hipDeviceAttributeMultiprocessorCount, dev) == hipSuccess && v > 0 ? v : 256;
    }
    n_cu = cu_of_dev[dev];
  }
  if (n_cu <= 0) n_cu = 256;
  const int BM = 64 * tj;
  const int tiles_m = (M + BM - 1) / BM, tiles_n = (N + BN - 1) / BN;
  const int steps = K / (q8 ? 128 : 64);
  const bool halves = ks == 2 && (tj == 4 || (tj == 3 && !q8)) && steps % 2 == 0, parts = !q8 && tj == 2 && (ks == 2 || ks == 4 || ks == 8) && steps % ks == 0;
  IFX_REQUIRE(ks == 0 || ks == 1 || (workspace != nullptr && tiles_m * tiles_n * (ks - 1) <= 1024 && (halves || parts)),
              tj >= 3 ? "ifx_gemm_bf16: the %d-way K split on the 256- / 192-token tile needs two parts (8-bit operands: 256 tokens), a workspace, an even number of K-steps and at most 1024 tiles"
                      : "ifx_gemm_bf16: the %d-way K split needs the bf16 128-token tile, a workspace, K / 64 divisible by it and at most 1024 partial slots", ks);
  const int total = tiles_m * tiles_n * (ks ? ks : 1), per_xcd = (total + 7) / 8;
  int wg_per_xcd = min(per_xcd, max(1, n_cu / 8));
  if (ks == 0) {
    const long units = (long)total * (K * (q8 ? 1 : 2) / 128);
    IFX_REQUIRE(!q8 && tj == 2 && workspace != nullptr && units >= 8, "ifx_gemm_bf16: stream-K needs the bf16 128-token tile, a workspace and at least 8 K-steps");
    wg_per_xcd = (int)max(1L, min((long)min(n_cu, 256) / 8, units / 6 / 8));
  }
  const dim3 grid(wg_per_xcd * 8);
  unsigned* ws_flag = ks == 1 ? nullptr : (unsigned*)workspace;
  float* ws_part = ws_flag ? (float*)((char*)workspace + 4096) : nullptr;
  static unsigned long long* trace = nullptr;
  static const int dbg = lab_env_int("IFX_PP_DEBUG", 0);
  const int dbg_launch = dbg | (spin_fault() ? 32 : 0);
  unsigned* const err_word = device_error_word();
  const long long spin_ticks = spin_timeout_ticks();
#if IFX_PP_TRACE
  if (!trace) {
    const char* e = getenv("IFX_PP_TRACE_PTR");
    if (e) trace = (unsigned long long*)strtoull(e, nullptr, 0);
  }
#endif
#define IFX_LAUNCH_PP(E, T, S, Q, L)                                                                                                 \
  do {                                                                                                                               \
    static bool attr_set = false;                                                                                                    \
    if (!attr_set) {                                                                                                                 \
      (void)hipFuncSetAttribute((const void*)gemm_pp_kernel<E, T, S, Q, L>, hipFuncAttributeMaxDynamicSharedMemorySize, (int)LDS_BYTES); \
      attr_set = true;                                                                                                               \
    }                                                                                                                                \
    hipLaunchKernelGGL((gemm_pp_kernel<E, T, S, Q, L>), grid, dim3(L ? 768 : 512), LDS_BYTES, s, x, ldx, w, y, ldy, M, N, K, tiles_m, \
                       total, per_xcd, wg_per_xcd, ea, trace, dbg_launch, ws_part, ws_flag, err_word, spin_ticks);                   \
  } while (0)
  const int fmt = !q8 ? 0 : q8_int8 ? 2 : 1;
  const int lw = fmt == 0 && tj == 2 && ks == 1 && gemm_pp_variant() != 1;
  int rc = INT_MIN;
#define IFX_PP_CASE(T, S, Q, L) \
  if (tj == T && ks == S && fmt == Q && lw == L) rc = dispatch_epilogue(mode, "ifx_gemm(pp)", [&](auto epi_c) { IFX_LAUNCH_PP(decltype(epi_c)::value, T, S, Q, L); });
  IFX_PP_CASE(4, 1, 0, 0) IFX_PP_CASE(3, 1, 0, 0) IFX_PP_CASE(2, 1, 0, 0) IFX_PP_CASE(2, 1, 0, 1)
  IFX_PP_CASE(4, 2, 0, 0) IFX_PP_CASE(3, 2, 0, 0)
  IFX_PP_CASE(2, 0, 0, 0) IFX_PP_CASE(2, 2, 0, 0) IFX_PP_CASE(2, 4, 0, 0) IFX_PP_CASE(2, 8, 0, 0)
  IFX_PP_CASE(4, 1, 1, 0) IFX_PP_CASE(3, 1, 1, 0) IFX_PP_CASE(2, 1, 1, 0) IFX_PP_CASE(4, 2, 1, 0)
  IFX_PP_CASE(4, 1, 2, 0) IFX_PP_CASE(3, 1, 2, 0) IFX_PP_CASE(2, 1, 2, 0) IFX_PP_CASE(4, 2, 2, 0)
#undef IFX_PP_CASE
#undef IFX_LAUNCH_PP
  IFX_REQUIRE(rc != INT_MIN, q8 ? "ifx_gemm_q8: no ping-pong tile of %d tokens" : "ifx_gemm_bf16: no ping-pong tile of %d tokens", 64 * tj);
  if (rc != IFX_OK) return rc;
  return check_launch("ifx_gemm_bf16(pp)");
}

}
```

### inferix_amd/csrc/ifx_norm.hip

```cpp
#include "ifx_rows.h"

namespace ifx {

template <int NCH, int QUANT = 0>
__global__ __launch_bounds__(256) void layernorm_kernel(
    const unsigned short* __restrict__ x, unsigned short* __restrict__ y, int rows, int dim, float eps,
    int mode, const unsigned short* __restrict__ gamma, const unsigned short* __restrict__ beta,
    const unsigned short* __restrict__ mod, int mod_slots, int shift_slot, int scale_slot,
    int rows_per_group, unsigned char* __restrict__ q, int ldq, float* __restrict__ qscale, int n_out, int via_bf16) {
  const int lane = threadIdx.x & 63;
  const int r = blockIdx.x * 4 + (threadIdx.x >> 6);
  if (r >= rows) return;
  u16x8 xr[NCH], pa[NCH], pb[NCH];
  load_chunks<NCH>(xr, x + (size_t)r * dim, dim, lane);
  {
    const unsigned short* pa_p = nullptr;
    const unsigned short* pb_p = nullptr;
    if (mode == IFX_LN_MODULATE) {
      const size_t g0 = (size_t)(r / rows_per_group) * mod_slots;
      pa_p = mod + (g0 + scale_slot) * dim;
      pb_p = mod + (g0 + shift_slot) * dim;
    } else if (mode == IFX_LN_AFFINE) {
      pa_p = gamma;
      pb_p = beta;
    }
    if (pa_p != nullptr) {
      load_chunks<NCH>(pa, pa_p, dim, lane);
      load_chunks<NCH>(pb, pb_p, dim, lane);
    } else {
#pragma unroll
      for (int c = 0; c < NCH; ++c) {
        pa[c] = u16x8{0, 0, 0, 0, 0, 0, 0, 0};
        pb[c] = u16x8{0, 0, 0, 0, 0, 0, 0, 0};
      }
    }
  }
  Row<NCH> row;
  row.from(xr, dim, lane);
  float mean, rstd;
  ln_stats(row, dim, eps, lane, mean, rstd);

  u16x8 qrow[QUANT != 0 ? NCH : 1];
  if (QUANT != 0) {
#pragma unroll
    for (int c = 0; c < NCH; ++c) qrow[c] = u16x8{0, 0, 0, 0, 0, 0, 0, 0};
  }
#pragma unroll
  for (int c = 0; c < NCH; ++c) {
    const int col = c * 512 + lane * 8;
    if (col >= dim) continue;
    u16x8 o;
    if (mode == IFX_LN_MODULATE) {
      const u16x8 sc = pa[c], sh = pb[c];
#pragma unroll
      for (int i = 0; i < 8; ++i) {
        float t = rbf((row.v[c][i] - mean) * rstd);
        float s1 = rbf(1.0f + bf2f(sc[i]));
        t = rbf(t * s1);
        o[i] = f2bf(t + bf2f(sh[i]));
      }
    } else if (mode == IFX_LN_AFFINE) {
      const u16x8 g = pa[c], b = pb[c];
#pragma unroll
      for (int i = 0; i < 8; ++i)
        o[i] = f2bf((row.v[c][i] - mean) * rstd * bf2f(g[i]) + bf2f(b[i]));
    } else {
#pragma unroll
      for (int i = 0; i < 8; ++i) o[i] = f2bf((row.v[c][i] - mean) * rstd);
    }
    if (QUANT == 0) *reinterpret_cast<u16x8*>(y + (size_t)r * dim + col) = o;
    else qrow[c] = o;
  }
  if constexpr (QUANT == 3) {
    const float* divs = qscale;
    for (int j = 0; j < n_out; ++j) {
#pragma unroll
      for (int c = 0; c < NCH; ++c) {
        const int col = c * 512 + lane * 8;
        if (col >= dim) continue;
        const f32x4 d0 = *reinterpret_cast<const f32x4*>(divs + (size_t)j * dim + col);
        const f32x4 d1 = *reinterpret_cast<const f32x4*>(divs + (size_t)j * dim + col + 4);
        float v[8];
#pragma unroll
        for (int i = 0; i < 8; ++i) v[i] = bf2f(qrow[c][i]);
        *reinterpret_cast<u32x2*>(q + (size_t)r * ldq + (size_t)j * dim + col) = div_clamp8<true>(v, d0, d1, via_bf16);
      }
    }
  } else if constexpr (QUANT != 0) {
    quant_row_dynamic<QUANT == 1, NCH>(qrow, q + (size_t)r * ldq, qscale + r, dim, lane);
  }
}

template <int NCH>
__global__ __launch_bounds__(256) void rmsnorm_kernel(const unsigned short* __restrict__ x, int ldx,
                                                      unsigned short* __restrict__ y, int ldy,
                                                      const unsigned short* __restrict__ w, int rows,
                                                      int dim, float eps) {
  const int lane = threadIdx.x & 63;
  const int r = blockIdx.x * 4 + (threadIdx.x >> 6);
  if (r >= rows) return;
  u16x8 xr[NCH], wv[NCH];
  load_chunks<NCH>(xr, x + (size_t)r * ldx, dim, lane);
  load_chunks<NCH>(wv, w, dim, lane);
  Row<NCH> row;
  row.from(xr, dim, lane);
  const float rs = 1.0f / sqrtf(wave_sum(row.sumsq()) / (float)dim + eps);
#pragma unroll
  for (int c = 0; c < NCH; ++c) {
    const int col = c * 512 + lane * 8;
    u16x8 o;
#pragma unroll
    for (int i = 0; i < 8; ++i) o[i] = f2bf(rbf(row.v[c][i] * rs) * bf2f(wv[c][i]));
    if (col < dim) *reinterpret_cast<u16x8*>(y + (size_t)r * ldy + col) = o;
  }
}

template <int NCH>
__global__ __launch_bounds__(256) void rmsnorm_rope_append_kernel(
    const unsigned short* __restrict__ qkv, int ld, unsigned short* __restrict__ q_out,
    const unsigned short* __restrict__ wq, const unsigned short* __restrict__ wk, RopeArgs ra, int has_rope,
    unsigned short* __restrict__ kc, unsigned short* __restrict__ vc, KvAddr ka, int local_start, int rows,
    int dim, int head_dim, float eps) {
  const int lane = threadIdx.x & 63;
  const int r = blockIdx.x * 4 + (threadIdx.x >> 6);
  if (r >= rows) return;
  const unsigned short* base = qkv + (size_t)r * ld;

  size_t slot_off = 0;
  if (kc != nullptr) slot_off = (size_t)ka.slot(local_start + r) * dim;
  const RopeToken tk(ra, has_rope, r, head_dim, lane);

  const bool has_kv = kc != nullptr;
  const bool copy_v = vc != nullptr;
  u16x8 qraw[NCH], kraw[NCH], vraw[NCH], wqv[NCH], wkv[NCH];
  load_chunks<NCH>(qraw, base, dim, lane);
  load_chunks<NCH>(wqv, wq, dim, lane);
  if (has_kv) {
    load_chunks<NCH>(kraw, base + dim, dim, lane);
    if (copy_v) load_chunks<NCH>(vraw, base + 2 * dim, dim, lane);
    load_chunks<NCH>(wkv, wk, dim, lane);
  }
  if (has_kv && copy_v) {
#pragma unroll
    for (int c = 0; c < NCH; ++c) {
      const int col = c * 512 + lane * 8;
      if (col < dim) *reinterpret_cast<u16x8*>(vc + slot_off + col) = vraw[c];
    }
  }
  Row<NCH> row;
  rmsnorm_rope_row<NCH>(row, qraw, wqv, tk, ra, has_rope, ra.q_scale, dim, head_dim, eps, lane,
                        [&](int, int col, const u16x8& o) { *reinterpret_cast<u16x8*>(q_out + (size_t)r * dim + col) = o; });
  if (!has_kv) return;
  rmsnorm_rope_row<NCH>(row, kraw, wkv, tk, ra, has_rope, 1.0f, dim, head_dim, eps, lane,
                        [&](int, int col, const u16x8& o) { *reinterpret_cast<u16x8*>(kc + slot_off + col) = o; });
}

__global__ __launch_bounds__(256) void kv_copy_rows_kernel(const unsigned short* __restrict__ src,
                                                           unsigned short* __restrict__ dst, KvAddr ka,
                                                           int src_tok0, int dst_tok0, int ntok, int row_elems,
                                                           int src_is_paged, int dst_is_paged) {
  const int chunks = row_elems / 8;
  const size_t total = (size_t)ntok * chunks;
  for (size_t i = (size_t)blockIdx.x * blockDim.x + threadIdx.x; i < total; i += (size_t)gridDim.x * blockDim.x) {
    const int t = (int)(i / chunks), c = (int)(i - (size_t)t * chunks);
    const size_t s = (size_t)(src_is_paged ? ka.slot(src_tok0 + t) : (src_tok0 + t)) * row_elems + c * 8;
    const size_t d = (size_t)(dst_is_paged ? ka.slot(dst_tok0 + t) : (dst_tok0 + t)) * row_elems + c * 8;
    *reinterpret_cast<u16x8*>(dst + d) = *reinterpret_cast<const u16x8*>(src + s);
  }
}

__global__ __launch_bounds__(256) void kv_scatter_shards_kernel(const unsigned short* __restrict__ gathered,
                                                                unsigned short* __restrict__ kc,
                                                                unsigned short* __restrict__ vc, KvAddr ka, int world,
                                                                int frames, int hw_local, int frame_tokens,
                                                                int local_start, int row_elems) {
  const int n_local = frames * hw_local;
  const int chunks = row_elems / 8;
  const size_t total = (size_t)world * n_local * chunks;
  for (size_t i = (size_t)blockIdx.x * blockDim.x + threadIdx.x; i < total; i += (size_t)gridDim.x * blockDim.x) {
    const int row = (int)(i / chunks), c = (int)(i - (size_t)row * chunks);
    const int r = row / n_local, j = row - r * n_local;
    const int f = j / hw_local, w = j - f * hw_local;
    const int tok = local_start + f * frame_tokens + r * hw_local + w;
    const size_t d = (size_t)ka.slot(tok) * row_elems + c * 8;
    const unsigned short* ks = gathered + ((size_t)(2 * r) * n_local + j) * row_elems + c * 8;
    *reinterpret_cast<u16x8*>(kc + d) = *reinterpret_cast<const u16x8*>(ks);
    *reinterpret_cast<u16x8*>(vc + d) = *reinterpret_cast<const u16x8*>(ks + (size_t)n_local * row_elems);
  }
}

template <typename F>
static int dispatch_norm(int dim, F&& f, const char* too_wide = "row kernels support dim <= 5120 (got %d)") {
  return dispatch_nch<1, 2, 3, 4, 6, 8, 10>(dim, too_wide, f);
}

template <typename F>
static int dispatch_layernorm(int dim, F&& f) {
  if (dim > 5120 && dim <= 6144 && dim % 512 == 0) return f(std::integral_constant<int, 12>{});
  return dispatch_norm(dim, f, "LayerNorm row kernels support dim <= 5120, and 5632 and 6144 (got %d)");
}

}

using namespace ifx;

extern "C" int ifx_layernorm(const ifx_bf16* x, ifx_bf16* y, int32_t rows, int32_t dim, float eps, int32_t mode,
                             const ifx_bf16* gamma, const ifx_bf16* beta, const ifx_bf16* mod, int32_t mod_slots,
                             int32_t shift_slot, int32_t scale_slot, int32_t rows_per_group, void* stream) {
  IFX_REQUIRE(x && y && rows >= 0 && dim > 0 && dim % 8 == 0, "ifx_layernorm: bad x/y/rows/dim(%d)", dim);
  if (const int rc = check_ln_mode("ifx_layernorm", mode, gamma, beta, mod, mod_slots, shift_slot, scale_slot, rows_per_group))
    return rc;
  if (rows == 0) return IFX_OK;
  return dispatch_layernorm(dim, [&](auto nch) {
    return launch_rows("ifx_layernorm", layernorm_kernel<decltype(nch)::value, 0>, rows, stream, x, y, rows, dim, eps, mode, gamma, beta,
                       mod, mod_slots, shift_slot, scale_slot, rows_per_group > 0 ? rows_per_group : 1, (unsigned char*)nullptr, 0,
                       (float*)nullptr, 0, 0);
  });
}

extern "C" int ifx_layernorm_quant(const ifx_bf16* x, void* q, int32_t ldq, float* scale, int32_t rows, int32_t dim, float eps,
                                   int32_t mode, const ifx_bf16* gamma, const ifx_bf16* beta, const ifx_bf16* mod,
                                   int32_t mod_slots, int32_t shift_slot, int32_t scale_slot, int32_t rows_per_group,
                                   int32_t format, void* stream) {
  IFX_REQUIRE(x && q && scale && rows >= 0 && dim > 0 && dim % 8 == 0 && ldq >= dim && ldq % 8 == 0,
              "ifx_layernorm_quant: bad x/q/scale/rows/dim(%d)/ldq(%d)", dim, ldq);
  IFX_REQUIRE(format == IFX_Q_FP8_E4M3 || format == IFX_Q_INT8, "ifx_layernorm_quant: unknown format %d", format);
  if (const int rc = check_ln_mode("ifx_layernorm_quant", mode, gamma, beta, mod, mod_slots, shift_slot, scale_slot, rows_per_group))
    return rc;
  if (rows == 0) return IFX_OK;
  return dispatch_layernorm(dim, [&](auto nch) {
    return dispatch_q8_format(format, [&](auto fp8) {
      return launch_rows("ifx_layernorm_quant", layernorm_kernel<decltype(nch)::value, decltype(fp8)::value ? 1 : 2>, rows, stream, x,
                         (unsigned short*)nullptr, rows, dim, eps, mode, gamma, beta, mod, mod_slots, shift_slot, scale_slot,
                         rows_per_group > 0 ? rows_per_group : 1, (unsigned char*)q, ldq, scale, 0, 0);
    });
  });
}

extern "C" int ifx_layernorm_quant_static(const ifx_bf16* x, void* q, int32_t ldq, const float* divisors, int32_t n_out, int32_t rows,
                                          int32_t dim, float eps, int32_t mode, const ifx_bf16* gamma, const ifx_bf16* beta,
                                          int32_t via_bf16, void* stream) {
  IFX_REQUIRE(x && q && divisors && rows >= 0 && dim > 0 && dim % 8 == 0 && n_out >= 1 && n_out <= 8 && ldq >= n_out * dim && ldq % 8 == 0,
              "ifx_layernorm_quant_static: bad x/q/divisors/rows/dim(%d)/n_out(%d)/ldq(%d)", dim, n_out, ldq);
  IFX_REQUIRE(mode == IFX_LN_PLAIN || mode == IFX_LN_AFFINE, "ifx_layernorm_quant_static: mode %d (plain or affine)", mode);
  if (mode == IFX_LN_AFFINE) IFX_REQUIRE(gamma && beta, "ifx_layernorm_quant_static: affine mode needs gamma/beta");
  if (rows == 0) return IFX_OK;
  return dispatch_layernorm(dim, [&](auto nch) {
    return launch_rows("ifx_layernorm_quant_static", layernorm_kernel<decltype(nch)::value, 3>, rows, stream, x, (unsigned short*)nullptr,
                       rows, dim, eps, mode, gamma, beta, (const unsigned short*)nullptr, 0, 0, 0, 1, (unsigned char*)q, ldq,
                       const_cast<float*>(divisors), n_out, via_bf16);
  });
}

extern "C" int ifx_rmsnorm(const ifx_bf16* x, int32_t ldx, ifx_bf16* y, int32_t ldy, const ifx_bf16* w,
                           int32_t rows, int32_t dim, float eps, void* stream) {
  IFX_REQUIRE(x && y && w && rows >= 0 && dim > 0 && dim % 8 == 0 && ldx % 8 == 0 && ldy % 8 == 0,
              "ifx_rmsnorm: bad arguments (dim %d)", dim);
  IFX_REQUIRE(ldx >= dim && ldy >= dim, "ifx_rmsnorm: row strides ldx (%d) and ldy (%d) must be >= dim (%d)", ldx, ldy, dim);
  if (rows == 0) return IFX_OK;
  return dispatch_norm(dim, [&](auto nch) {
    return launch_rows("ifx_rmsnorm", rmsnorm_kernel<decltype(nch)::value>, rows, stream, x, ldx, y, ldy, w, rows, dim, eps);
  });
}

extern "C" int ifx_rmsnorm_rope_kv_append(const ifx_bf16* qkv, int32_t ld, ifx_bf16* q_out, const ifx_bf16* wq,
                                          const ifx_bf16* wk, const ifx_rope_grid* rope, const ifx_kv_view* kv,
                                          int32_t local_start, int32_t rows, int32_t dim, float eps,
                                          void* stream) {
  IFX_REQUIRE(qkv && q_out && wq && rows >= 0 && dim > 0 && dim % 8 == 0 && ld % 8 == 0,
              "ifx_rmsnorm_rope_kv_append: bad arguments");
  int head_dim = 128;
  KvAddr ka{nullptr, 1};
  unsigned short *kc = nullptr, *vc = nullptr;
  if (kv) {
    IFX_REQUIRE(wk && kv->k && kv->v && kv->kv_heads * kv->head_dim == dim,
                "ifx_rmsnorm_rope_kv_append: kv view (heads %d x head_dim %d) does not match dim %d",
                kv->kv_heads, kv->head_dim, dim);
    IFX_REQUIRE(local_start >= 0 && local_start + rows <= kv->num_slots,
                "ifx_rmsnorm_rope_kv_append: append [%d, %d) exceeds cache capacity %d", local_start,
                local_start + rows, kv->num_slots);
    if (const int rc = check_writer_view("ifx_rmsnorm_rope_kv_append", kv)) return rc;
    head_dim = kv->head_dim;
    kc = kv->k;
    vc = kv->v;
    ka = KvAddr{kv->page_table, kv->page_size};
  }
  RopeArgs ra{};
  if (const int rc = resolve_rope("ifx_rmsnorm_rope_kv_append", rope, head_dim, dim, rows, &ra)) return rc;
  if (rope) {
    IFX_REQUIRE(rope->q_scale >= 0.f && rope->q_scale == rope->q_scale, "ifx_rmsnorm_rope_kv_append: q_scale must be >= 0 (0 = 1)");
    ra.q_scale = rope->q_scale > 0.f ? rope->q_scale : 1.0f;
    if (rope->flags & 1) {
      IFX_REQUIRE(kv != nullptr, "ifx_rmsnorm_rope_kv_append: flags bit 0 (V in place) needs a cache view");
      vc = nullptr;
    }
  }
  {
    const int cols = kc == nullptr ? 1 : (vc == nullptr ? 2 : 3);
    IFX_REQUIRE(ld >= cols * dim, "ifx_rmsnorm_rope_kv_append: qkv_row_stride (ld %d) must cover the %d x dim (%d) columns read", ld, cols,
                dim);
  }
  if (rows == 0) return IFX_OK;
  return dispatch_norm(dim, [&](auto nch) {
    return launch_rows("ifx_rmsnorm_rope_kv_append", rmsnorm_rope_append_kernel<decltype(nch)::value>, rows, stream, qkv, ld, q_out, wq,
                       wk, ra, rope ? 1 : 0, kc, vc, ka, local_start, rows, dim, head_dim, eps);
  });
}

struct PeerDest {
  unsigned short* k[IFX_MAX_PEERS];
  unsigned short* v[IFX_MAX_PEERS];
  int n;
};

template <int NCH>
__global__ __launch_bounds__(256) void rmsnorm_rope_kv_push_kernel(
    const unsigned short* __restrict__ kv, int ld, const unsigned short* __restrict__ wk, RopeArgs ra, int has_rope, PeerDest pd,
    KvAddr ka, int local_start, int frame_tokens, int slot_hw_local, int slot_hw_offset, int rows, int dim, int head_dim, float eps) {
  const int lane = threadIdx.x & 63;
  const int r = blockIdx.x * 4 + (threadIdx.x >> 6);
  if (r >= rows) return;
  const unsigned short* base = kv + (size_t)r * ld;
  const int sf = r / slot_hw_local;
  const size_t slot_off = (size_t)ka.slot(local_start + sf * frame_tokens + slot_hw_offset + (r - sf * slot_hw_local)) * dim;
  const RopeToken tk(ra, has_rope, r, head_dim, lane);
  u16x8 kraw[NCH], vraw[NCH], wkv[NCH];
  load_chunks<NCH>(kraw, base, dim, lane);
  load_chunks<NCH>(vraw, base + dim, dim, lane);
  load_chunks<NCH>(wkv, wk, dim, lane);
  Row<NCH> row;
  rmsnorm_rope_row<NCH>(row, kraw, wkv, tk, ra, has_rope, 1.0f, dim, head_dim, eps, lane, [&](int c, int col, const u16x8& o) {
    for (int p = 0; p < pd.n; ++p) {
      *reinterpret_cast<u16x8*>(pd.k[p] + slot_off + col) = o;
      *reinterpret_cast<u16x8*>(pd.v[p] + slot_off + col) = vraw[c];
    }
  });
}

extern "C" int ifx_rmsnorm_rope_kv_push(const ifx_bf16* kv_rows, int32_t ld, const ifx_bf16* wk, const ifx_rope_grid* rope,
                                        const ifx_peer_caches* peers, const ifx_kv_view* geometry, int32_t local_start,
                                        int32_t frame_tokens, int32_t slot_hw_local, int32_t slot_hw_offset, int32_t rows, int32_t dim,
                                        float eps, void* stream) {
  IFX_REQUIRE(kv_rows && wk && peers && geometry && rows >= 0 && dim > 0 && dim % 8 == 0 && ld % 8 == 0 && ld >= 2 * dim,
              "ifx_rmsnorm_rope_kv_push: bad arguments");
  IFX_REQUIRE(peers->count >= 1 && peers->count <= IFX_MAX_PEERS, "ifx_rmsnorm_rope_kv_push: %d destinations (1..%d)", peers->count,
              IFX_MAX_PEERS);
  IFX_REQUIRE(geometry->kv_heads * geometry->head_dim == dim, "ifx_rmsnorm_rope_kv_push: cache rows (heads %d x head_dim %d) != dim %d",
              geometry->kv_heads, geometry->head_dim, dim);
  IFX_REQUIRE(slot_hw_local > 0 && frame_tokens >= slot_hw_local && slot_hw_offset >= 0 && slot_hw_offset + slot_hw_local <= frame_tokens,
              "ifx_rmsnorm_rope_kv_push: bad shard geometry (frame %d tokens, shard [%d, %d))", frame_tokens, slot_hw_offset,
              slot_hw_offset + slot_hw_local);
  if (rows == 0) return IFX_OK;
  const int last_f = (rows - 1) / slot_hw_local;
  const int last_token = local_start + last_f * frame_tokens + slot_hw_offset + (rows - 1 - last_f * slot_hw_local);
  IFX_REQUIRE(local_start >= 0 && last_token < geometry->num_slots, "ifx_rmsnorm_rope_kv_push: token %d exceeds the cache capacity %d",
              last_token, geometry->num_slots);
  if (geometry->page_table) IFX_REQUIRE(geometry->page_size > 0, "ifx_rmsnorm_rope_kv_push: page_size must be > 0");
  PeerDest pd{};
  pd.n = peers->count;
  for (int p = 0; p < pd.n; ++p) {
    IFX_REQUIRE(peers->k[p] && peers->v[p], "ifx_rmsnorm_rope_kv_push: destination %d is null", p);
    pd.k[p] = peers->k[p];
    pd.v[p] = peers->v[p];
  }
  const int head_dim = geometry->head_dim;
  RopeArgs ra{};
  if (const int rc = resolve_rope("ifx_rmsnorm_rope_kv_push", rope, head_dim, dim, rows, &ra)) return rc;
  const KvAddr ka{geometry->page_table, geometry->page_size, geometry->page_table ? 0 : geometry->seg_split,
                  geometry->page_table ? 0 : geometry->seg_delta};
  return dispatch_norm(dim, [&](auto nch) {
    return launch_rows("ifx_rmsnorm_rope_kv_push", rmsnorm_rope_kv_push_kernel<decltype(nch)::value>, rows, stream, kv_rows, ld, wk, ra,
                       rope ? 1 : 0, pd, ka, local_start, frame_tokens, slot_hw_local, slot_hw_offset, rows, dim, head_dim, eps);
  });
}

extern "C" int ifx_kv_roll(const ifx_kv_view* kv, int32_t sink_tokens, int32_t evicted, int32_t rolled,
                           ifx_bf16* scratch, void* stream) {
  IFX_REQUIRE(kv && kv->k && kv->v && scratch, "ifx_kv_roll: null argument");
  IFX_REQUIRE(sink_tokens >= 0 && evicted >= 0 && rolled >= 0 &&
                  sink_tokens + evicted + rolled <= kv->num_slots,
              "ifx_kv_roll: span out of range");
  if (const int rc = check_writer_view("ifx_kv_roll", kv)) return rc;
  if (rolled == 0 || evicted == 0) return IFX_OK;
  const int row_elems = kv->kv_heads * kv->head_dim;
  KvAddr ka{kv->page_table, kv->page_size};
  const int blocks = 1024;
  for (int which = 0; which < 2; ++which) {
    unsigned short* c = which == 0 ? kv->k : kv->v;
    hipLaunchKernelGGL(kv_copy_rows_kernel, dim3(blocks), dim3(256), 0, (hipStream_t)stream, c, scratch, ka,
                       sink_tokens + evicted, 0, rolled, row_elems, 1, 0);
    hipLaunchKernelGGL(kv_copy_rows_kernel, dim3(blocks), dim3(256), 0, (hipStream_t)stream, scratch, c, ka, 0,
                       sink_tokens, rolled, row_elems, 0, 1);
  }
  return check_launch("ifx_kv_roll");
}

extern "C" int ifx_kv_scatter_shards(const ifx_bf16* gathered, int32_t world, int32_t frames, int32_t hw_local,
                                     int32_t frame_tokens, int32_t local_start, const ifx_kv_view* kv, void* stream) {
  IFX_REQUIRE(gathered && kv && kv->k && kv->v, "ifx_kv_scatter_shards: null argument");
  IFX_REQUIRE(world > 0 && frames > 0 && hw_local > 0 && world * hw_local <= frame_tokens && local_start >= 0,
              "ifx_kv_scatter_shards: bad shard geometry (world %d, frames %d, hw_local %d, frame_tokens %d)", world,
              frames, hw_local, frame_tokens);
  IFX_REQUIRE(local_start + (frames - 1) * frame_tokens + world * hw_local <= kv->num_slots,
              "ifx_kv_scatter_shards: tokens [%d, %d) exceed the cache capacity %d", local_start,
              local_start + (frames - 1) * frame_tokens + world * hw_local, kv->num_slots);
  if (const int rc = check_writer_view("ifx_kv_scatter_shards", kv)) return rc;
  const int row_elems = kv->kv_heads * kv->head_dim;
  IFX_REQUIRE(row_elems % 8 == 0, "ifx_kv_scatter_shards: row of %d elements is not 16-byte granular", row_elems);
  const size_t total = (size_t)world * frames * hw_local * (row_elems / 8);
  const int blocks = (int)((total + 255) / 256 < 4096 ? (total + 255) / 256 : 4096);
  hipLaunchKernelGGL(kv_scatter_shards_kernel, dim3(blocks), dim3(256), 0, (hipStream_t)stream, gathered, kv->k, kv->v,
                     KvAddr{kv->page_table, kv->page_size}, world, frames, hw_local, frame_tokens, local_start, row_elems);
  return check_launch("ifx_kv_scatter_shards");
}
// ... 1 lines not shown
```

### inferix_amd/csrc/ifx_rows.h

```cpp
#pragma once
#include <type_traits>

#include "ifx_common.h"

namespace ifx {

template <int NCH>
__device__ __forceinline__ void load_chunks(u16x8 (&u)[NCH], const unsigned short* p, int dim, int lane) {
#pragma unroll
  for (int c = 0; c < NCH; ++c) {
    const int col = c * 512 + lane * 8;
    u[c] = *reinterpret_cast<const u16x8*>(p + (col < dim ? col : 0));
  }
}

template <int NCH>
struct Row {
  float v[NCH][8];
  __device__ __forceinline__ void from(const u16x8 (&u)[NCH], int dim, int lane) {
#pragma unroll
    for (int c = 0; c < NCH; ++c) {
      const bool ok = c * 512 + lane * 8 < dim;
#pragma unroll
      for (int i = 0; i < 8; ++i) v[c][i] = ok ? bf2f(u[c][i]) : 0.f;
    }
  }
  __device__ __forceinline__ float sum() const {
    float s = 0.f;
#pragma unroll
    for (int c = 0; c < NCH; ++c)
#pragma unroll
      for (int i = 0; i < 8; ++i) s += v[c][i];
    return s;
  }
  __device__ __forceinline__ float sumsq() const {
    float s = 0.f;
#pragma unroll
    for (int c = 0; c < NCH; ++c)
#pragma unroll
      for (int i = 0; i < 8; ++i) s += v[c][i] * v[c][i];
    return s;
  }
};

template <int NCH>
__device__ __forceinline__ void ln_stats(const Row<NCH>& row, int dim, float eps, int lane, float& mean, float& rstd) {
  const float inv_n = 1.0f / (float)dim;
  mean = wave_sum(row.sum()) * inv_n;
  float ss = 0.f;
#pragma unroll
  for (int c = 0; c < NCH; ++c) {
    if (c * 512 + lane * 8 < dim) {
#pragma unroll
      for (int i = 0; i < 8; ++i) {
        const float d = row.v[c][i] - mean;
        ss += d * d;
      }
    }
  }
  rstd = 1.0f / sqrtf(wave_sum(ss) * inv_n + eps);
}

template <bool FP8>
__device__ __forceinline__ u32x2 pack8(const float (&v)[8]) {
  if (FP8) {
    unsigned w0 = 0, w1 = 0;
    w0 = __builtin_amdgcn_cvt_pk_fp8_f32(v[0], v[1], w0, false);
    w0 = __builtin_amdgcn_cvt_pk_fp8_f32(v[2], v[3], w0, true);
    w1 = __builtin_amdgcn_cvt_pk_fp8_f32(v[4], v[5], w1, false);
    w1 = __builtin_amdgcn_cvt_pk_fp8_f32(v[6], v[7], w1, true);
    return u32x2{w0, w1};
  }
  unsigned w[2] = {0, 0};
#pragma unroll
  for (int i = 0; i < 8; ++i) w[i >> 2] |= ((unsigned)(int)rintf(v[i]) & 0xffu) << (8 * (i & 3));
  return u32x2{w[0], w[1]};
}

template <bool FP8, int NCH>
__device__ __forceinline__ void quant_row_dynamic(const u16x8 (&u)[NCH], unsigned char* qr, float* scale, int dim, int lane) {
  constexpr float QMAX = FP8 ? 448.0f : 127.0f;
  float amax = 0.f;
#pragma unroll
  for (int c = 0; c < NCH; ++c)
#pragma unroll
    for (int i = 0; i < 8; ++i) amax = fmaxf(amax, fabsf(bf2f(u[c][i])));
  amax = wave_max(amax);
  const float s = amax > 0.f ? amax / QMAX : 1.0f;
  if (lane == 0) *scale = s;
  const RowDivisor rdiv(s);
  auto emit = [&](auto fastc) {
#pragma unroll
    for (int c = 0; c < NCH; ++c) {
      const int col = c * 512 + lane * 8;
      float v[8];
#pragma unroll
      for (int i = 0; i < 8; ++i) v[i] = fminf(fmaxf(rdiv.template div<decltype(fastc)::value>(bf2f(u[c][i])), -QMAX), QMAX);
      const u32x2 pk = pack8<FP8>(v);
      if (col < dim) *reinterpret_cast<u32x2*>(qr + col) = pk;
    }
  };
  if (rdiv.fast()) emit(std::true_type{});
  else emit(std::false_type{});
}

template <bool FP8>
__device__ __forceinline__ u32x2 div_clamp8(const float (&x)[8], const f32x4 d0, const f32x4 d1, int via_bf16) {
  constexpr float QMAX = FP8 ? 448.0f : 127.0f;
  float v[8];
#pragma unroll
  for (int i = 0; i < 8; ++i) {
    const float t = fminf(fmaxf(x[i] / (i < 4 ? d0[i] : d1[i - 4]), -QMAX), QMAX);
    v[i] = via_bf16 ? rbf(t) : t;
  }
  return pack8<FP8>(v);
}

struct RopeArgs {
  const double* freqs;
  int max_pos, start_frame, height, width, hw_offset, hw_local;
  float q_scale = 1.0f;
};

__device__ __forceinline__ void rope4(float (&t)[8], int jp0, const RopeArgs& ra, int half, int n_t,
                                      int n_h, int pos_t, int pos_h, int pos_w) {
#pragma unroll
  for (int p = 0; p < 4; ++p) {
    const int j = jp0 + p;
    const int pos = (j < n_t) ? pos_t : ((j < n_t + n_h) ? pos_h : pos_w);
    const double2 cs = *reinterpret_cast<const double2*>(ra.freqs + ((size_t)pos * half + j) * 2);
    const double a = (double)t[2 * p], b = (double)t[2 * p + 1];
    const double re = __dmul_rn(a, cs.x) - __dmul_rn(b, cs.y);
    const double im = __dmul_rn(a, cs.y) + __dmul_rn(b, cs.x);
    t[2 * p] = (float)re;
    t[2 * p + 1] = (float)im;
  }
}

__device__ __forceinline__ void rope4_cs(float (&t)[8], const double2 (&cs)[4]) {
#pragma unroll
  for (int p = 0; p < 4; ++p) {
    const double a = (double)t[2 * p], b = (double)t[2 * p + 1];
    const double re = __dmul_rn(a, cs[p].x) - __dmul_rn(b, cs[p].y);
    const double im = __dmul_rn(a, cs[p].y) + __dmul_rn(b, cs[p].x);
    t[2 * p] = (float)re;
    t[2 * p + 1] = (float)im;
  }
}

struct RopeToken {
  int pos_t = 0, pos_h = 0, pos_w = 0;
  int half, n_t, n_h;
  bool shared_cs;
  double2 cs4[4];
  __device__ __forceinline__ RopeToken(const RopeArgs& ra, int has_rope, int r, int head_dim, int lane)
      : half(head_dim >> 1), n_t(half - 2 * (half / 3)), n_h(half / 3), shared_cs(has_rope && (512 % head_dim) == 0) {
    if (has_rope) {
      const int f = r / ra.hw_local;
      const int p = ra.hw_offset + (r - f * ra.hw_local);
      pos_t = ra.start_frame + f;
      pos_h = p / ra.width;
      pos_w = p - pos_h * ra.width;
    }
    if (shared_cs) {
      const int jp0 = ((lane * 8) % head_dim) >> 1;
#pragma unroll
      for (int p = 0; p < 4; ++p) {
        const int j = jp0 + p;
        const int pos = (j < n_t) ? pos_t : ((j < n_t + n_h) ? pos_h : pos_w);
        cs4[p] = *reinterpret_cast<const double2*>(ra.freqs + ((size_t)pos * half + j) * 2);
      }
    }
  }
};

template <int NCH, typename Put>
__device__ __forceinline__ void rmsnorm_rope_row(Row<NCH>& row, const u16x8 (&raw)[NCH], const u16x8 (&wv)[NCH], const RopeToken& tk,
                                                 const RopeArgs& ra, int has_rope, float out_scale, int dim, int head_dim, float eps,
                                                 int lane, Put&& put) {
  row.from(raw, dim, lane);
  const float rs = 1.0f / sqrtf(wave_sum(row.sumsq()) / (float)dim + eps);
#pragma unroll
  for (int c = 0; c < NCH; ++c) {
    const int col = c * 512 + lane * 8;
    float t[8];
#pragma unroll
    for (int i = 0; i < 8; ++i) t[i] = rbf(rbf(row.v[c][i] * rs) * bf2f(wv[c][i]));
    if (tk.shared_cs) rope4_cs(t, tk.cs4);
    else if (has_rope && col < dim) rope4(t, (col % head_dim) >> 1, ra, tk.half, tk.n_t, tk.n_h, tk.pos_t, tk.pos_h, tk.pos_w);
    u16x8 o;
#pragma unroll
    for (int i = 0; i < 8; ++i) o[i] = f2bf(t[i] * out_scale);
    if (col < dim) put(c, col, o);
  }
}

// ... 53 lines not shown
```

### inferix_amd/hip_ops.py

```python
from __future__ import annotations

import ctypes as C
import threading
from dataclasses import dataclass
from typing import Sequence, Optional, Tuple

import torch

from . import _hip

BF16 = torch.bfloat16
F32 = torch.float32


class KernelTimer:

    def __init__(self, names=("attn_self",)):
        self.names = set(names)
        self.records = []

    def wants(self, name: str) -> bool:
        return name in self.names

    def summary(self):
# ... 692 lines not shown
def magi_head_prep(mixed: torch.Tensor, *, layout: int, q_heads: int, kv_heads: int, eps: float, layernorm_1p: bool,
                   k_out: torch.Tensor, v_out: torch.Tensor, kv_head_stride: int, ld_kv: int, row0: int = 0,
                   split: Optional[int] = None, row1: int = 0, rope: Optional[torch.Tensor] = None, qn=None, kn=None, xn=None,
                   q_out: Optional[torch.Tensor] = None, qx_out: Optional[torch.Tensor] = None, q_scale: float = 0.0,
                   q_group: int = 0) -> None:
    rows = mixed.shape[0]
    assert mixed.dim() == 2 and mixed.stride(1) == 1
    d = _hip.MagiHeadPrepDesc()
    d.inp, d.ld_in, d.rows, d.layout = _dev(mixed, "mixed"), mixed.stride(0), rows, layout
    d.q_heads, d.kv_heads, d.head_dim = q_heads, kv_heads, 128
    d.eps, d.layernorm_1p = float(eps), 1 if layernorm_1p else 0
    if layout == 0:
        assert rope is not None and rope.is_contiguous() and rope.dim() == 2 and rope.shape[0] == rows
        assert rope.shape[1] % 16 == 0 and rope.shape[1] <= 128, "rope rows are (sin | cos) of at most 64 pairs, a multiple of 8 each"
        d.rope = _dev(rope, "rope", F32)
        d.rope_half = rope.shape[1] // 2
        d.qn_w, d.qn_b = _dev(qn[0], "q_layernorm.weight", F32), _dev(qn[1], "q_layernorm.bias", F32)
        d.kn_w, d.kn_b = _dev(kn[0], "k_layernorm.weight", F32), _dev(kn[1], "k_layernorm.bias", F32)
        if q_group > 0:
            assert q_out.dim() == 3 and q_out.is_contiguous() and q_out.shape == (q_heads // q_group, rows, q_group * 128), q_out.shape
            d.q_out, d.ld_q, d.q_group, d.q_group_stride = _dev(q_out, "q_out"), q_group * 128, int(q_group), rows * q_group * 128
        else:
            d.q_out, d.ld_q = _dev(q_out, "q_out"), q_out.stride(0)
            assert q_out.shape[0] >= rows
        d.qx_out, d.ld_qx = _dev(qx_out, "qx_out"), qx_out.stride(0)
        assert qx_out.shape[0] >= rows
    d.xn_w, d.xn_b = _dev(xn[0], "layernorm_xattn.weight"), _dev(xn[1], "layernorm_xattn.bias")
    d.k_out, d.v_out, d.ld_kv, d.kv_head_stride = _dev(k_out, "k_out"), _dev(v_out, "v_out"), int(ld_kv), int(kv_head_stride)
    d.row0, d.split, d.row1 = int(row0), int(rows if split is None else split), int(row1)
    d.q_scale = float(q_scale)
    n_heads = (2 * q_heads + 2 * kv_heads) if layout == 0 else 2 * kv_heads
    with _timed("magi_head_prep", 0.0, 4.0 * rows * n_heads * 128):
        _hip.check(_hip.load().ifx_magi_head_prep(C.byref(d), _stream()), "ifx_magi_head_prep")


def kv_split_rows(kv: torch.Tensor, k_cache: torch.Tensor, v_cache: torch.Tensor, row0: int, split: int, row1: int) -> None:
    n, heads, hd2 = kv.shape
    assert hd2 == 256 and kv.is_contiguous() and k_cache.is_contiguous() and v_cache.is_contiguous()
    assert k_cache.shape[1:] == (heads, 128) and v_cache.shape == k_cache.shape
    assert 0 <= split <= n and row0 + split <= k_cache.shape[0] and row1 + (n - split) <= k_cache.shape[0]
    _hip.check(_hip.load().ifx_kv_split_rows(_dev(kv, "kv"), _dev(k_cache, "k_cache"), _dev(v_cache, "v_cache"), n, heads, int(row0),
                                             int(split), int(row1), _stream()), "ifx_kv_split_rows")


def magi_gate_norm_residual(x: torch.Tensor, residual: torch.Tensor, condition_map: torch.Tensor, gate: torch.Tensor,
                            norm_w: torch.Tensor, norm_b: torch.Tensor, eps: float, layernorm_1p: bool,
                            out: Optional[torch.Tensor] = None) -> torch.Tensor:
    rows, dim, ldx = _rows2d(x, "x")
    _, _, ldr = _rows2d(residual, "residual")
    out = torch.empty(rows, dim, dtype=BF16, device=x.device) if out is None else out
    _, _, ldy = _rows2d(out, "out")
    assert gate.dim() == 2 and gate.shape[1] == dim and gate.stride(1) == 1
    assert condition_map.dtype == torch.int32 and condition_map.is_cuda and condition_map.numel() == rows and condition_map.is_contiguous()
    with _timed("magi_gate_norm", 0.0, 6.0 * rows * dim):
        _hip.check(_hip.load().ifx_magi_gate_norm_residual(
            _dev(x, "x"), ldx, _dev(residual, "residual"), ldr, condition_map.data_ptr(), _dev(gate, "gate"), gate.stride(0),
            _dev(norm_w, "norm_w", F32), _dev(norm_b, "norm_b", F32), 1 if layernorm_1p else 0, _dev(out, "out"), ldy, rows, dim,
            float(eps), _stream()), "ifx_magi_gate_norm_residual")
    return out


def act_rows(x: torch.Tensor, mode: int, out: Optional[torch.Tensor] = None) -> torch.Tensor:
    assert x.is_contiguous()
    out = torch.empty_like(x) if out is None else out
    _hip.check(_hip.load().ifx_act_rows(_dev(x, "x"), _dev(out, "out"), x.numel(), int(mode), _stream()), "ifx_act_rows")
    return out


def silu_and_mul(x: torch.Tensor, out: Optional[torch.Tensor] = None, quant_divisor: Optional[torch.Tensor] = None,
                 q: Optional[torch.Tensor] = None):
    xp = _dev(x, "x")
    rows, two_f, ldx = _rows2d(x, "x")
    if two_f % 2:
        raise ValueError(f"silu_and_mul: x has {two_f} columns, not gate | up halves")
    f = two_f // 2
    dp, dn, qp, ldq = None, 0, None, 0
    if quant_divisor is not None:
        quant_divisor = quant_divisor.reshape(-1)
        q = torch.empty(rows, f, dtype=torch.uint8, device=x.device) if q is None else q
        dp, dn, qp, ldq = _dev(quant_divisor, "quant_divisor", F32), quant_divisor.numel(), _dev(q, "q", torch.uint8), q.stride(0)
    elif q is not None:
        raise ValueError("silu_and_mul: q needs quant_divisor")
    elif out is None:
        out = torch.empty(rows, f, dtype=BF16, device=x.device)
    yp, ldy = (_dev(out, "out"), out.stride(0)) if out is not None else (None, 0)
    for t, name in ((out, "out"), (q if quant_divisor is not None else None, "q")):
        if t is not None and (t.dim() != 2 or tuple(t.shape) != (rows, f)):
            raise ValueError(f"silu_and_mul: {name} must be [{rows}, {f}], got {tuple(t.shape)}")
    with _timed("silu_and_mul", 0.0, rows * f * (4.0 + (2.0 if out is not None else 0.0) + (1.0 if qp is not None else 0.0))):
        _hip.check(_hip.load().ifx_silu_and_mul(xp, ldx, yp, ldy, qp, ldq, dp, dn, rows, f, _stream()), "ifx_silu_and_mul")
    if quant_divisor is None:
        return out
    return q if out is None else (out, q)


def quant_static(x: torch.Tensor, divisor: torch.Tensor, fmt: int, via_bf16: bool, q: Optional[torch.Tensor] = None,
                 row_scale: Optional[torch.Tensor] = None) -> torch.Tensor:
    rows, K, ldx = _rows2d(x, "x")
    q = torch.empty(rows, K, dtype=torch.uint8, device=x.device) if q is None else q
    divisor = divisor.reshape(-1)
    with _timed("quant_static", 0.0, 3.0 * rows * K):
        _hip.check(_hip.load().ifx_quant_static(_dev(x, "x"), ldx, _dev(q, "q", torch.uint8), q.stride(0), _dev(divisor, "divisor", F32),
                                                divisor.numel(), _dev(row_scale, "row_scale", F32) if row_scale is not None else None,
                                                rows, K, int(fmt), 1 if via_bf16 else 0, _stream()), "ifx_quant_static")
    return q


_AMAX_WS: dict = {}


def quant_per_tensor(x: torch.Tensor, fmt: int, q: Optional[torch.Tensor] = None,
                     scale: Optional[torch.Tensor] = None) -> Tuple[torch.Tensor, torch.Tensor]:
    rows, K, ldx = _rows2d(x, "x")
    q = torch.empty(rows, K, dtype=torch.uint8, device=x.device) if q is None else q
    scale = torch.empty(rows, dtype=F32, device=x.device) if scale is None else scale
    key = (x.device.index, _stream())
    ws = _AMAX_WS.get(key)
    if ws is None:
        ws = _AMAX_WS[key] = torch.zeros(1, dtype=torch.int32, device=x.device)
    _hip.check(_hip.load().ifx_quant_per_tensor(_dev(x, "x"), ldx, _dev(q, "q", torch.uint8), q.stride(0), _dev(scale, "scale", F32),
                                                ws.data_ptr(), rows, K, int(fmt), _stream()), "ifx_quant_per_tensor")
    return q, scale


def attention_ranges(q: torch.Tensor, kv: KvCacheView, q_ranges, k_ranges, out: torch.Tensor, heads: int, scale: float = 0.0,
                     tag: str = "attn") -> torch.Tensor:
    n = len(q_ranges)
    assert 1 <= n <= 8 and len(k_ranges) == n and q.dim() == 2 and out.dim() == 2 and q.stride(1) == 1 and out.stride(1) == 1
    rows = q.shape[0]
    qa = (C.c_int32 * (2 * n))(*[int(v) for r in q_ranges for v in r])
    ka = (C.c_int32 * (2 * n))(*[int(v) for r in k_ranges for v in r])
    ks = kv.struct()
    d = heads * 128
    flops = sum(4.0 * (qe - qs) * (ke - kb) * d for (qs, qe), (kb, ke) in zip(q_ranges, k_ranges))
    with _timed(tag, flops, 0.0):
        _hip.check(_hip.load().ifx_attn_fwd_ranges(_dev(q, "q"), q.stride(0), _dev(out, "out"), out.stride(0), C.byref(ks), rows, heads,
                                                   n, qa, ka, float(scale), _stream()), "ifx_attn_fwd_ranges")
    return out


def attention_dedup(q: torch.Tensor, kv: KvCacheView, kv_len: int, last_key_multiplicity: int, out: Optional[torch.Tensor] = None,
                    scale: float = 0.0, tag: str = "attn") -> torch.Tensor:
    assert q.dim() == 3 and q.is_contiguous()
    rows, heads, hd = q.shape
    out = torch.empty_like(q) if out is None else out
    ks = kv.struct()
    nk = kv_len - 1 + last_key_multiplicity
    with _timed(tag, 4.0 * rows * nk * heads * hd, 0.0):
        _hip.check(_hip.load().ifx_attn_fwd_dedup(_dev(q, "q"), _dev(out, "out"), C.byref(ks), rows, heads, int(kv_len),
                                                  int(last_key_multiplicity), float(scale), _stream()), "ifx_attn_fwd_dedup")
    return out


def vit_head_prep(qkv: torch.Tensor, *, batch: int, heads: int, cls_tokens: int, norm: bool, eps: float = 1e-5,
                  sin: Optional[torch.Tensor] = None, cos: Optional[torch.Tensor] = None) -> torch.Tensor:
    rows, width, ld = _rows2d(qkv, "qkv")
    assert qkv.dim() == 2 and width == 3 * heads * 64 and rows % batch == 0, (qkv.shape, batch, heads)
    tokens = rows // batch
    if sin is not None:
        assert cos is not None and sin.shape == cos.shape == (tokens - cls_tokens, 64) and sin.is_contiguous() and cos.is_contiguous()
    rope = sin is not None and tokens > cls_tokens
    with _timed("vit_head_prep", 0.0, 4.0 * rows * width):
        _hip.check(_hip.load().ifx_vit_head_prep(_dev(qkv, "qkv"), ld, _dev(sin, "sin") if rope else None, _dev(cos, "cos") if rope else None,
                                                 batch, tokens, heads, int(cls_tokens), int(bool(norm)), int(rope), float(eps), _stream()),
                   "ifx_vit_head_prep")
    return qkv


def vit_attention(q: torch.Tensor, k: torch.Tensor, v: torch.Tensor, *, batch: int, heads: int,
                  out: Optional[torch.Tensor] = None) -> torch.Tensor:
    rows = q.shape[0]
    assert q.dim() == 2 and q.shape[1] == heads * 64 and k.shape == q.shape and v.shape == q.shape and rows % batch == 0
    tokens = rows // batch
    out = torch.empty(rows, heads * 64, dtype=BF16, device=q.device) if out is None else out
    assert out.dim() == 2 and out.shape == q.shape
    with _timed("vit_attention", 4.0 * batch * heads * tokens * tokens * 64, 0.0):
        _hip.check(_hip.load().ifx_vit_attention(_dev(q, "q"), q.stride(0), _dev(k, "k"), k.stride(0), _dev(v, "v"), v.stride(0),
                                                 _dev(out, "out"), out.stride(0), batch, tokens, heads, _stream()), "ifx_vit_attention")
    return out


def vit_unpatch_conv(x: torch.Tensor, weight: torch.Tensor, bias: torch.Tensor, *, batch: int, cls_tokens: int, latent: Tuple[int, int, int],
                     patch: Tuple[int, int, int], out: Optional[torch.Tensor] = None) -> torch.Tensor:
    rows, width, ld = _rows2d(x, "x")
    (lt, lh, lw), (pt, ph, pw) = latent, patch
    assert x.dim() == 2 and rows % batch == 0 and weight.dim() == 5 and weight.is_contiguous() and bias.is_contiguous()
    ch = weight.shape[1]
    assert tuple(weight.shape) == (3, ch, 3, 3, 3) and tuple(bias.shape) == (3,) and width == pt * ph * pw * ch, (weight.shape, x.shape)
    T, H, W = lt * pt, lh * ph, lw * pw
    out = torch.empty(batch, 3, T, H, W, dtype=BF16, device=x.device) if out is None else out
    assert tuple(out.shape) == (batch, 3, T, H, W) and out.is_contiguous()
    with _timed("vit_unpatch_conv", 2.0 * 27 * ch * 3 * batch * T * H * W, 0.0):
        _hip.check(_hip.load().ifx_vit_unpatch_conv(_dev(x, "x"), ld, rows // batch, int(cls_tokens), _dev(weight, "weight"), _dev(bias, "bias"),
                                                    _dev(out, "out"), batch, T, H, W, pt, ph, pw, ch, _stream()), "ifx_vit_unpatch_conv")
    return out


def vit_tile_blend(arena: torch.Tensor, desc, table: torch.Tensor, *, out=True, out_u8=False):
    T, H, W = desc.out_shape
    B = desc.batch
    assert arena.dim() == 1 and arena.is_contiguous() and arena.numel() >= desc.arena_elements, (arena.shape, desc.arena_elements)
    assert table.dtype == torch.int64 and table.is_contiguous() and table.numel() == len(desc.words) and table.device == arena.device
    if out is True:
        out = torch.empty(B, 3, T, H, W, dtype=BF16, device=arena.device)
    if out_u8 is True:
        out_u8 = torch.empty(B * T, 3, H, W, dtype=torch.uint8, device=arena.device)
    out = None if out is False else out
    out_u8 = None if out_u8 is False else out_u8
    assert out is None or (tuple(out.shape) == (B, 3, T, H, W) and out.is_contiguous())
    assert out_u8 is None or (tuple(out_u8.shape) == (B * T, 3, H, W) and out_u8.is_contiguous())
    (nt, nh, nw), (et, eh, ew), (lt, lh, lw) = desc.grid, desc.blends, desc.limits
    nbytes = float(B * 3 * T * H * W) * ((2 if out is not None else 0) + (1 if out_u8 is not None else 0))
    with _timed("vit_tile_blend", 0.0, nbytes):
        _hip.check(_hip.load().ifx_vit_tile_blend(_dev(arena, "arena"), _dev(table, "table", torch.int64),
                                                  _dev(out, "out") if out is not None else None,
                                                  _dev(out_u8, "out_u8", torch.uint8) if out_u8 is not None else None, B, T, H, W, nt, nh, nw,
                                                  et, eh, ew, lt, lh, lw, int(desc.vec_x), _stream()), "ifx_vit_tile_blend")
    return out, out_u8
```

### inferix_amd/wan/causal_model.py

```python
from __future__ import annotations

import math
import os
from dataclasses import dataclass
from typing import Dict, List, Optional, Sequence, Tuple

import torch
import torch.nn.functional as F

from .. import _hip, hip_ops as ops
from ..kvcache_manager import KVCacheManager, KVCacheRequest
from ..kvcache_manager.model import SelfForcingKVCacheManagerFactory
from . import components as C

BF16 = torch.bfloat16


class ParallelConfig:

    def __init__(self, ulysses_size=1, ring_size=1, local_rank=0, rank=0, world_size=1,
                 ring_strategy="pass-kv", attn_backend=None):
        from ..attention import collect_supported_attn
        ulysses_size, ring_size, world_size = int(ulysses_size), int(ring_size), int(world_size)
        if ulysses_size < 1 or ring_size < 1:
            raise ValueError(f"ulysses_size={ulysses_size} / ring_size={ring_size}: degrees must be >= 1")
        if ulysses_size * ring_size not in (1, world_size):
            raise ValueError(f"ulysses_size={ulysses_size} x ring_size={ring_size} != world_size={world_size}: the sequence-parallel "
                             "degree is ulysses_size * ring_size and must equal the number of ranks")
        self.ulysses_size, self.ring_size = ulysses_size, ring_size
        self.local_rank, self.rank, self.world_size = local_rank, rank, world_size
        self.ring_strategy = ring_strategy
        supported = collect_supported_attn()
        if attn_backend is None:
            attn_backend = "HipPagedFA"
        if attn_backend not in supported:
            raise ValueError(f"Specified attention backend '{attn_backend}' is not available. "
                             f"Available backends: {list(supported)}")
        self.attn_backend = attn_backend


@dataclass
class KVIndexStep:
    local_start: int
    local_end: int
    global_end: int
    evicted: int
    rolled: int
    sink_tokens: int


def kv_index_update(global_end: int, local_end: int, current_start: int, num_new: int, cache_size: int,
                    local_attn_size: int, sink_tokens: int) -> KVIndexStep:
    current_end = current_start + num_new
    evicted = rolled = 0
    if local_attn_size != -1 and current_end > global_end and num_new + local_end > cache_size:
        evicted = num_new + local_end - cache_size
        rolled = local_end - evicted - sink_tokens
    new_local_end = local_end + current_end - global_end - evicted
    return KVIndexStep(new_local_end - num_new, new_local_end, current_end, evicted, rolled, sink_tokens)


class _Block:

    def __init__(self, layer_idx: int, num_heads: int, head_dim: int, enable_kv_offload: bool):
        self.layer_idx = layer_idx
        self.kv_cache_manager = SelfForcingKVCacheManagerFactory.create_manager(
            layer_idx, num_heads, head_dim, enable_kv_offload=enable_kv_offload)
        self.w: Dict[str, torch.Tensor] = {}
        self.cross_meta = {"is_init": False}

    @property
    def is_cross_attn_init(self) -> bool:
        return self.cross_meta["is_init"]

    @is_cross_attn_init.setter
    def is_cross_attn_init(self, v: bool) -> None:
        self.cross_meta["is_init"] = bool(v)


class HipCausalWanModel(torch.nn.Module):
    def __init__(self, model_type="t2v", patch_size=(1, 2, 2), text_len=512, in_dim=16, dim=2048, ffn_dim=8192,
                 freq_dim=256, text_dim=4096, out_dim=16, num_heads=16, num_layers=32, local_attn_size=-1,
                 sink_size=0, qk_norm=True, cross_attn_norm=True, eps=1e-6, enable_kv_offload=False,
                 parallel_config: Optional[ParallelConfig] = None, device="cuda"):
        super().__init__()
        if model_type != "t2v":
            raise NotImplementedError("HipCausalWanModel: only the t2v cross-attention path is built")
        if not (qk_norm and cross_attn_norm):
            raise NotImplementedError("HipCausalWanModel: qk_norm and cross_attn_norm are always on (Wan2.1 config)")
        if dim % num_heads or dim // num_heads != 128:
            raise NotImplementedError("HipCausalWanModel: kernels are built for head_dim 128")
        _hip.load()
        self.model_type, self.patch_size, self.text_len = model_type, tuple(patch_size), text_len
        self.in_dim, self.dim, self.ffn_dim, self.freq_dim = in_dim, dim, ffn_dim, freq_dim
        self.text_dim, self.out_dim, self.num_heads, self.num_layers = text_dim, out_dim, num_heads, num_layers
        self.head_dim = dim // num_heads
        self.local_attn_size, self.sink_size, self.eps = local_attn_size, sink_size, eps
        self.qk_norm, self.cross_attn_norm = qk_norm, cross_attn_norm
        self.enable_kv_offload = enable_kv_offload
        self.parallel_config = parallel_config if parallel_config is not None else ParallelConfig()
        pc = self.parallel_config
        u, r = int(getattr(pc, "ulysses_size", 1)), int(getattr(pc, "ring_size", 1))
        if u * r not in (1, int(getattr(pc, "world_size", 1))):
            raise ValueError(f"CausalWanModel: ulysses_size={u} x ring_size={r} must equal world_size={getattr(pc, 'world_size', 1)} "
                             "(both degrees map onto the one sequence-parallel exchange; see ParallelConfig)")
        self.num_frame_per_block = 1
        self.independent_first_frame = False
        self.device_ = torch.device(device)
        self.blocks: List[_Block] = [_Block(i, num_heads, self.head_dim, enable_kv_offload) for i in range(num_layers)]
        self.g: Dict[str, torch.Tensor] = {}
        self.mod_all: Optional[torch.Tensor] = None
        self.freqs = C.rope_table(self.head_dim).to(self.device_)
        self._scratch: Dict[Tuple, torch.Tensor] = {}
        self.cross_dedup = True
        self._cross_dedup: Dict[str, Tuple[int, int]] = {}
        self._roll_scratch: Optional[torch.Tensor] = None
        self.v_direct = os.environ.get("IFX_V_DIRECT", "1") != "0"
        self._temb_cache: Dict[Tuple, Tuple] = {}
        self.index_trace: Optional[list] = None
        self._chain = 0
        self._pair_stream: Optional[torch.cuda.Stream] = None
        self.cp = None
        self.q_prescale = self.head_dim == 128

    def parameters(self, recurse: bool = True):
        for t in self.g.values():
            yield t
        for b in self.blocks:
            for t in b.w.values():
                if isinstance(t, torch.Tensor):
                    yield t

    def state_dict_keys(self) -> List[str]:
        keys = ["patch_embedding.weight", "patch_embedding.bias"]
        for n in ("text_embedding.0", "text_embedding.2", "time_embedding.0", "time_embedding.2", "time_projection.1"):
            keys += [n + ".weight", n + ".bias"]
        for i in range(self.num_layers):
            p = f"blocks.{i}."
            keys += [p + "modulation", p + "norm3.weight", p + "norm3.bias"]
            for a in ("self_attn", "cross_attn"):
                for n in ("q", "k", "v", "o"):
                    keys += [p + f"{a}.{n}.weight", p + f"{a}.{n}.bias"]
                keys += [p + f"{a}.norm_q.weight", p + f"{a}.norm_k.weight"]
            keys += [p + "ffn.0.weight", p + "ffn.0.bias", p + "ffn.2.weight", p + "ffn.2.bias"]
        keys += ["head.modulation", "head.head.weight", "head.head.bias"]
        return keys

    def load_state_dict(self, sd: Dict[str, torch.Tensor], strict: bool = True, assign: bool = False):
        missing = [k for k in self.state_dict_keys() if k not in sd]
        if missing and strict:
            raise KeyError(f"missing keys in state_dict: {missing[:5]}{'...' if len(missing) > 5 else ''}")
        dev = self.device_

        def t(name):
            return sd[name].detach().to(device=dev, dtype=BF16).contiguous()

        g = self.g
        g["patch_w"] = t("patch_embedding.weight").flatten(1).contiguous()
        g["patch_b"] = t("patch_embedding.bias")
        for short, n in (("text0", "text_embedding.0"), ("text2", "text_embedding.2"), ("time0", "time_embedding.0"),
                         ("time2", "time_embedding.2"), ("tproj", "time_projection.1"), ("head", "head.head")):
            g[short + "_w"], g[short + "_b"] = t(n + ".weight"), t(n + ".bias")
        g["head_mod"] = t("head.modulation")
        mods = []
        for i, blk in enumerate(self.blocks):
            p = f"blocks.{i}."
            w = blk.w
            w["qkv_w"] = torch.cat([t(p + f"self_attn.{n}.weight") for n in "qkv"], dim=0).contiguous()
            w["qkv_b"] = torch.cat([t(p + f"self_attn.{n}.bias") for n in "qkv"], dim=0).contiguous()
            w["nq"], w["nk"] = t(p + "self_attn.norm_q.weight"), t(p + "self_attn.norm_k.weight")
            w["o_w"], w["o_b"] = t(p + "self_attn.o.weight"), t(p + "self_attn.o.bias")
            w["n3_w"], w["n3_b"] = t(p + "norm3.weight"), t(p + "norm3.bias")
            for n in "qkvo":
                w[f"c{n}_w"], w[f"c{n}_b"] = t(p + f"cross_attn.{n}.weight"), t(p + f"cross_attn.{n}.bias")
            w["cnq"], w["cnk"] = t(p + "cross_attn.norm_q.weight"), t(p + "cross_attn.norm_k.weight")
            w["f0_w"], w["f0_b"] = t(p + "ffn.0.weight"), t(p + "ffn.0.bias")
            w["f2_w"], w["f2_b"] = t(p + "ffn.2.weight"), t(p + "ffn.2.bias")
            mods.append(t(p + "modulation"))
        self.mod_all = torch.stack(mods, dim=0).contiguous()
        self._temb_cache.clear()
        return self

    def _buf(self, name: str, *shape) -> torch.Tensor:
        key = (self._chain, name, shape)
        b = self._scratch.get(key)
        if b is None:
            b = torch.empty(*shape, dtype=BF16, device=self.device_)
            self._scratch[key] = b
        return b

    @staticmethod
    def _meta_int(v) -> int:
        return int(v.item()) if isinstance(v, torch.Tensor) else int(v)

    @staticmethod
    def _meta_set(meta: dict, key: str, value: int) -> None:
        cur = meta.get(key)
        if isinstance(cur, torch.Tensor):
            cur.fill_(value)
        else:
            meta[key] = value

    def _kv_view(self, mgr: KVCacheManager, req: KVCacheRequest, name: str) -> ops.KvCacheView:
        t = mgr.get_raw(req, name)
        pt = mgr.page_table(req, name) if hasattr(mgr, "page_table") else None
        caches = getattr(mgr, "request_to_kv_caches", {}).get(getattr(req, "request_id", None))
        store = getattr(caches, "views", None)
        key = (t.data_ptr(), None if pt is None else (pt.device.data_ptr(), pt.page_size))
        if store is not None:
            hit = store.get(name)
            if hit is not None and hit[0] == key:
                return hit[1]
        if not t.is_cuda:
            raise _hip.HipKernelError(
                f"KV cache '{name}' lives on {t.device}: the HIP path reads pages in place from HBM "
                "(create the model with enable_kv_offload=False)")
        if pt is not None:
            v = ops.KvCacheView.from_manager_tensor(t, pt.device, pt.page_size)
        else:
            v = ops.KvCacheView.from_manager_tensor(t)
        if store is not None:
            store[name] = (key, v)
        return v

    def _evict(self, mgr, req, name: str, view: ops.KvCacheView, step: KVIndexStep) -> None:
        pt = mgr.page_table(req, name) if hasattr(mgr, "page_table") else None
        if pt is not None and step.sink_tokens % pt.page_size == 0 and step.evicted % pt.page_size == 0 \
                and step.rolled % pt.page_size == 0:
            mgr.rotate_pages(req, name, step.sink_tokens // pt.page_size, step.evicted // pt.page_size,
                             step.rolled // pt.page_size)
            return
        need = step.rolled * self.dim
        if self._chain:
            ops.kv_roll(view, step.sink_tokens, step.evicted, step.rolled, self._buf("roll", need))
            return
        if self._roll_scratch is None or self._roll_scratch.numel() < need:
            self._roll_scratch = torch.empty(need, dtype=BF16, device=self.device_)
        ops.kv_roll(view, step.sink_tokens, step.evicted, step.rolled, self._roll_scratch)

    def _q8_scratch(self, rows: int, cols: int, device):
        c = self._chain
        xq = self._scratch.get((c, "xq", rows, cols))
        if xq is None:
            xq = torch.empty(rows, cols, dtype=torch.uint8, device=device)
            self._scratch[(c, "xq", rows, cols)] = xq
            self._scratch[(c, "xs", rows)] = torch.empty(rows, dtype=torch.float32, device=device)
        return xq, self._scratch[(c, "xs", rows)]

    def _lin(self, w: Dict[str, torch.Tensor], key: str, x: torch.Tensor, **kw) -> torch.Tensor:
        if key + "_q" in w:
            fmt = w[key + "_fmt"]
            xq, xs = self._q8_scratch(x.shape[0], x.shape[1], x.device)
            if w.get(key + "_act") == "per_tensor":
                ops.quant_per_tensor(x, fmt, q=xq, scale=xs)
            else:
                ops.quant_per_token(x, fmt, q=xq, scale=xs)
            return ops.linear_q8(xq, xs, w[key + "_q"], w[key + "_s"], w[key + "_b"], fmt, **kw)
        return ops.linear(x, w[key + "_w"], w[key + "_b"], **kw)

    def _norm_lin(self, w: Dict[str, torch.Tensor], key: str, x: torch.Tensor, h: torch.Tensor, norm_kw: dict, **kw) -> torch.Tensor:
        if key + "_q" in w:
            fmt = w[key + "_fmt"]
            xq, xs = self._q8_scratch(x.shape[0], x.shape[1], x.device)
            if w.get(key + "_act") == "per_tensor":
                ops.layernorm(x, self.eps, out=h, **norm_kw)
                ops.quant_per_tensor(h, fmt, q=xq, scale=xs)
            else:
                ops.layernorm_quant(x, self.eps, fmt, q=xq, scale=xs, **norm_kw)
            return ops.linear_q8(xq, xs, w[key + "_q"], w[key + "_s"], w[key + "_b"], fmt, **kw)
        ops.layernorm(x, self.eps, out=h, **norm_kw)
        return ops.linear(h, w[key + "_w"], w[key + "_b"], **kw)

    def _run_block(self, l: int, xact: torch.Tensor, El: torch.Tensor, st: dict, meta: dict, cmeta: dict,
                   kv_cache_manager, kv_cache_requests) -> None:
        blk = self.blocks[l]
        w = blk.w
        d, H, hd = self.dim, self.num_heads, self.head_dim
        B, N, rows_per_group, rope = st["B"], st["N"], st["rows_per_group"], st["rope"]
        sink_tokens, current_start, ctx = st["sink_tokens"], st["current_start"], st["ctx"]
        h = self._buf("h", B * N, d)
        qkv = self._buf("qkv", B * N, 3 * d)
        qb = self._buf("q", B * N, d)
        ab = self._buf("a", B * N, d)
        ub = self._buf("u", B * N, self.ffn_dim)
        explicit0 = st.get("explicit_slots")
        samples = st.get("samples")
        if samples is None:
            samples = [dict(req=req, rope=rope, current_start=current_start, explicit=explicit0, ctx_index=b)
                       for b, req in enumerate(kv_cache_requests)]
        lockstep = bool(st.get("lockstep"))
        explicit_any = any(smp["explicit"] is not None for smp in samples)
        if not explicit_any:
            g_end, l_end = self._meta_int(meta["global_end_index"]), self._meta_int(meta["local_end_index"])
        else:
            g_end = l_end = 0
        steps_done: List[KVIndexStep] = []

        def index_state(smp=None):
            if lockstep and smp is not None and smp.get("fwd", 0) > 0:
                prev = [stp for stp, s0 in zip(steps_done, samples) if s0.get("fwd", 0) == smp["fwd"] - 1]
                if prev:
                    return prev[-1].global_end, prev[-1].local_end
            return g_end, l_end
        step = None
        kv_first = self.cp is not None and self.cp.kv_first and "qkv_q" not in w
        if kv_first:
            ops.layernorm(xact, self.eps, out=h, mod=El, shift_slot=0, scale_slot=1, rows_per_group=rows_per_group)
            kvp = self._buf("kvp", B * N, 2 * d)
            ops.linear(h, w["qkv_w"][d:], w["qkv_b"][d:], out=kvp)
            name = blk.kv_cache_manager.self_name
            pending = []
            for b, smp in enumerate(samples):
                ge, le = index_state(smp)
                pst = self.cp.begin(self, l, self._kv_view(kv_cache_manager, smp["req"], name), kvp[b * N:(b + 1) * N], w, smp["rope"],
                                    smp["current_start"], ge, le, sink_tokens, kv_cache_manager, smp["req"], name)
                pending.append(pst)
                steps_done.append(pst["step"])
            qraw = self._buf("qraw", B * N, d)
            ops.linear(h, w["qkv_w"][:d], w["qkv_b"][:d], out=qraw)
            for b, pst in enumerate(pending):
                ops.rmsnorm_rope_kv_append(qraw[b * N:(b + 1) * N], w["nq"], None, self.eps, samples[b]["rope"], None, 0, d,
                                           q_out=qb[b * N:(b + 1) * N])
                step = self.cp.finish(self, pst, qb[b * N:(b + 1) * N], ab[b * N:(b + 1) * N])
        planned: List[Tuple[KVIndexStep, ops.KvCacheView]] = []
        v_direct = None

        def plan(smp):
            name = blk.kv_cache_manager.self_name
            view = self._kv_view(kv_cache_manager, smp["req"], name)
            ge, le = index_state(smp)
            if smp["explicit"] is not None:
                step = KVIndexStep(smp["explicit"][0], smp["explicit"][1], smp["explicit"][1], 0, 0, 0)
            else:
                step = kv_index_update(ge, le, smp["current_start"], N, view.k.shape[0], self.local_attn_size, sink_tokens)
            if step.local_start < 0 or step.local_end > view.k.shape[0]:
                raise _hip.HipKernelError(f"KV cache overflow: slots [{step.local_start}, {step.local_end}) of "
                                          f"{view.k.shape[0]} (layer {l})")
            if step.evicted:
                self._evict(kv_cache_manager, smp["req"], name, view, step)
                view = self._kv_view(kv_cache_manager, smp["req"], name)
            steps_done.append(step)
            return step, view
        if not kv_first and self.cp is None and not lockstep:
            planned = [plan(smp) for smp in samples]
            step0, view0 = planned[0]
            if (self.v_direct and len(samples) == 1 and B * N >= 2048 and "qkv_q" not in w and view0.page_table is None
                    and not view0.seg_split and d % 256 == 0 and ops.get_option("gemm_variant") in (0, 22, 23, 24, 25)):
                v_direct = view0.v.view(view0.v.shape[0], d)[step0.local_start:step0.local_start + N]
        if not kv_first:
            extra = dict(out2=v_direct, split_col=2 * d) if v_direct is not None else {}
            self._norm_lin(w, "qkv", xact, h, dict(mod=El, shift_slot=0, scale_slot=1, rows_per_group=rows_per_group), out=qkv, **extra)
        for b, smp in enumerate(() if kv_first else samples):
            req, rope_b = smp["req"], smp["rope"]
            name = blk.kv_cache_manager.self_name
            if self.cp is not None:
                view = self._kv_view(kv_cache_manager, req, name)
                ge, le = index_state(smp)
                step = self.cp.self_attention(self, l, b, view, qkv[b * N:(b + 1) * N], qb[b * N:(b + 1) * N],
                                              ab[b * N:(b + 1) * N], w, rope_b, smp["current_start"], ge, le,
                                              sink_tokens, kv_cache_manager, req, name)
                steps_done.append(step)
                continue
            step, view = planned[b] if planned else plan(smp)
            ops.rmsnorm_rope_kv_append(qkv[b * N:(b + 1) * N], w["nq"], w["nk"], self.eps, rope_b, view,
                                       step.local_start, d, q_out=qb[b * N:(b + 1) * N], v_in_place=v_direct is not None)
            ops.attention(qb[b * N:(b + 1) * N].view(N, H, hd), view, step.local_end, scale=st.get("attn_scale", 0.0),
                          out=ab[b * N:(b + 1) * N].view(N, H, hd), tag="attn_self")
        if not explicit_any:
            self._meta_set(meta, "global_end_index", step.global_end)
            self._meta_set(meta, "local_end_index", step.local_end)
        if self.index_trace is not None and l == 0:
            for smp, stp in zip(samples, steps_done if steps_done else [step] * len(samples)):
                if smp["ctx_index"] == 0:
                    self.index_trace.append((int(smp["current_start"]), int(stp.global_end), int(stp.local_end)))
        self._lin(w, "o", ab, epilogue=_hip.IFX_EPI_GATE_RES, residual=xact, mod=El, gate_slot=2,
                  rows_per_group=rows_per_group, out=xact)
        self._norm_lin(w, "cq", xact, h, dict(gamma=w["n3_w"], beta=w["n3_b"]), out=qb)
        ops.rmsnorm(qb, w["cnq"], self.eps, out=qb)
        b = 0
        while b < len(samples):
            req = samples[b]["req"]
            nb = 1
            while b + nb < len(samples) and samples[b + nb]["req"] is req:
                nb += 1
            cview = self._kv_view(kv_cache_manager, req, blk.kv_cache_manager.cross_name)
            if not cmeta["is_init"]:
                ci = samples[b]["ctx_index"]
                cb = ctx[ci * self.text_len:(ci + 1) * self.text_len]
                kx = self._lin(w, "ck", cb)
                ops.rmsnorm(kx, w["cnk"], self.eps, out=cview.k.view(self.text_len, d))
                self._lin(w, "cv", cb, out=cview.v.view(self.text_len, d))
            nkeys, mult = self._cross_dedup.get(req.request_id, (self.text_len, 1)) if self.cross_dedup else (self.text_len, 1)
            qv, av = qb[b * N:(b + nb) * N].view(nb * N, H, hd), ab[b * N:(b + nb) * N].view(nb * N, H, hd)
            if mult > 1:
                ops.attention_dedup(qv, cview, nkeys, mult, out=av, tag="attn_cross")
            else:
                ops.attention(qv, cview, self.text_len, out=av, tag="attn_cross")
            b += nb
        cmeta["is_init"] = True
        self._lin(w, "co", ab, epilogue=_hip.IFX_EPI_RESIDUAL, residual=xact, out=xact)
        self._norm_lin(w, "f0", xact, h, dict(mod=El, shift_slot=3, scale_slot=4, rows_per_group=rows_per_group),
                       epilogue=_hip.IFX_EPI_GELU_TANH, out=ub)
        self._lin(w, "f2", ub, epilogue=_hip.IFX_EPI_GATE_RES, residual=xact, mod=El, gate_slot=5,
                  rows_per_group=rows_per_group, out=xact)


    @torch.no_grad()
    def forward(self, x, t, context, seq_len=None, clip_fea=None, y=None, kv_cache_meta=None,
                crossattn_cache_meta=None, current_start: int = 0, cache_start=None,
                kv_cache_manager: Optional[KVCacheManager] = None,
                kv_cache_requests: Optional[Sequence[KVCacheRequest]] = None,
                kv_start: Optional[int] = None, kv_end: Optional[int] = None,
                current_end: Optional[int] = None) -> torch.Tensor:
        fw = self._prologue(x, t, context, kv_cache_meta, crossattn_cache_meta, current_start, kv_cache_manager, kv_cache_requests,
                            kv_start, kv_end)
        with self._small_split_scope():
            for l in range(self.num_layers):
                self._run_block(l, fw["xact"], fw["E"][l], fw["st"], fw["kv_meta"][l], fw["cross_meta"][l], kv_cache_manager,
                                kv_cache_requests)
        return self._epilogue(fw)

    def _small_split_scope(self):
        import contextlib
        return ops.option_scope("gemm_small_split", 1) if getattr(self.cp, "gemm_small_split", False) else contextlib.nullcontext()

    @torch.no_grad()
    def forward_pair(self, first: dict, second: dict):
        if self._pair_mode() == "lockstep":
            return self._forward_pair_lockstep(first, second)
        dev = self.device_
        main = torch.cuda.current_stream(dev)
        if self._pair_stream is None:
            self._pair_stream = torch.cuda.Stream(device=dev)
        side = self._pair_stream
        side.wait_stream(main)
        kvm, reqs = first["kv_cache_manager"], first["kv_cache_requests"]
        assert second["kv_cache_manager"] is kvm, "forward_pair: both forwards must address the same cache"

        def pro(kw):
            return self._prologue(kw["x"], kw["t"], kw["context"], kw.get("kv_cache_meta"), kw.get("crossattn_cache_meta"),
                                  kw.get("current_start", 0), kw["kv_cache_manager"], kw["kv_cache_requests"], kw.get("kv_start"),
                                  kw.get("kv_end"))
        try:
            fa = pro(first)
            self._chain = 1
            with torch.cuda.stream(side):
                fb = pro(second)
            with self._small_split_scope():
                for l in range(self.num_layers):
                    self._chain = 0
                    self._run_block(l, fa["xact"], fa["E"][l], fa["st"], fa["kv_meta"][l], fa["cross_meta"][l], kvm, reqs)
                    ev = torch.cuda.Event()
                    ev.record(main)
                    self._chain = 1
                    with torch.cuda.stream(side):
                        side.wait_event(ev)
                        self._run_block(l, fb["xact"], fb["E"][l], fb["st"], fb["kv_meta"][l], fb["cross_meta"][l], kvm,
                                        second["kv_cache_requests"])
            self._chain = 0
            ya = self._epilogue(fa)
            self._chain = 1
            with torch.cuda.stream(side):
                yb = self._epilogue(fb)
        finally:
            self._chain = 0
        main.wait_stream(side)
        yb.record_stream(main)
        return ya, yb

    def _pair_mode(self) -> str:
        import os
        m = getattr(self, "pair_mode", None) or os.environ.get("IFX_PAIR_MODE", "")
        return m if m in ("streams", "lockstep") else "streams"

    def _forward_pair_lockstep(self, first: dict, second: dict):
        kvm, reqs = first["kv_cache_manager"], list(first["kv_cache_requests"])
        assert second["kv_cache_manager"] is kvm and list(second["kv_cache_requests"]) == reqs, \
            "forward_pair: both forwards must address the same requests"
        d = self.dim

        def pro(kw, out):
            return self._prologue(kw["x"], kw["t"], kw["context"], kw.get("kv_cache_meta"), kw.get("crossattn_cache_meta"),
                                  kw.get("current_start", 0), kvm, reqs, kw.get("kv_start"), kw.get("kv_end"), xact_out=out)
        lat = first["x"] if isinstance(first["x"], torch.Tensor) else torch.stack(list(first["x"]))
        B = lat.shape[0]
        pt_, ph, pw = self.patch_size
        rows = B * (lat.shape[2] // pt_) * (lat.shape[3] // ph) * (lat.shape[4] // pw) // self.parallel_config.world_size
        x2 = self._buf("x2", 2 * rows, d)
        fa = pro(first, x2[:rows])
        self._chain = 1
        try:
            fb = pro(second, x2[rows:])
        finally:
            self._chain = 0
        if fa["N"] != fb["N"] or fa["rows_per_group"] != fb["rows_per_group"] or fa["grid"] != fb["grid"]:
            raise ValueError("forward_pair (lockstep): the two forwards must have the same latent geometry and timestep layout")
        N = fa["N"]
        E2 = torch.cat([fa["E"], fb["E"]], dim=1).contiguous()
        eh2 = torch.cat([fa["eh"], fb["eh"]], dim=0).contiguous()
        sa, sb = fa["st"], fb["st"]
        samples = [dict(req=r, rope=s_["rope"], current_start=s_["current_start"], explicit=s_.get("explicit_slots"), ctx_index=b, fwd=f)
                   for f, s_ in enumerate((sa, sb)) for b, r in enumerate(reqs)]
        st = dict(sa, B=2 * B, samples=samples, lockstep=True, ctx=sa["ctx"] if sa["ctx"] is not None else sb["ctx"])
        if sa["ctx"] is None and sb["ctx"] is not None or any(not m["is_init"] for m in fa["cross_meta"]):
            raise RuntimeError("forward_pair: the cross-attention cache must be initialised before two forwards are paired")
        with self._small_split_scope():
            for l in range(self.num_layers):
                self._run_block(l, x2, E2[l], st, fa["kv_meta"][l], fa["cross_meta"][l], kvm, reqs)
        h2 = self._buf("h", 2 * B * N, d)
        ops.layernorm(x2, self.eps, mod=eh2, shift_slot=0, scale_slot=1, rows_per_group=fa["rows_per_group"], out=h2)
        yv = self._lin(self.g, "head", h2)
        if self.cp is not None:
            yv = self.cp.gather_head(yv, 2 * B, fa["F_"])
        y = C.unpatchify(yv, 2 * B, fa["grid"], self.patch_size, self.out_dim)
        return y[:B], y[B:]

    def _prologue(self, x, t, context, kv_cache_meta, crossattn_cache_meta, current_start, kv_cache_manager, kv_cache_requests,
                  kv_start=None, kv_end=None, xact_out: Optional[torch.Tensor] = None) -> dict:
        explicit = None
        if kv_start is not None and kv_end is not None:
            explicit = (int(kv_start), int(kv_end))
            kv_cache_meta = [dict() for _ in range(self.num_layers)]
            crossattn_cache_meta = [b.cross_meta for b in self.blocks]
        if kv_cache_meta is None:
            raise NotImplementedError("HipCausalWanModel implements the KV-cached inference path only")
        assert kv_cache_manager is not None and kv_cache_requests is not None
        if self.mod_all is None:
            raise RuntimeError("HipCausalWanModel: weights not loaded (call load_state_dict first)")
        dev, d, L = self.device_, self.dim, self.num_layers
        lat = torch.stack(list(x)) if not isinstance(x, torch.Tensor) else x
        lat = lat.to(device=dev, dtype=BF16)
        B, _, nf, hh, ww = lat.shape
        pt_, ph, pw = self.patch_size
        grid = (nf // pt_, hh // ph, ww // pw)
        F_, fs = grid[0], grid[1] * grid[2]
        cp_ws = self.parallel_config.world_size
        cp_rank = self.parallel_config.rank
        if fs % cp_ws != 0:
            raise ValueError(f"sequence parallelism splits every frame's {fs} tokens over {cp_ws} ranks: not divisible")
        hw_local = fs // cp_ws
        fs_l = hw_local
        N = F_ * fs_l
        assert len(kv_cache_requests) == B

        patches = C.patchify(lat, self.patch_size)
        if cp_ws > 1:
            patches = patches.view(B * F_, fs, -1)[:, cp_rank * hw_local:(cp_rank + 1) * hw_local].reshape(B * N, -1)
        xact = ops.linear(patches.contiguous(), self.g["patch_w"], self.g["patch_b"],
                          out=self._buf("x", B * N, d) if xact_out is None else xact_out)
        Ft = t.shape[1]
        rows_per_group = (F_ // Ft) * fs_l
# ... 69 lines not shown
```

Measured before the change: 22.51 frames/s.

## Fuse cross-attention query RMSNorm into the Q GEMM epilogue and attention kernel

The cross-attention query GEMM now emits per-row partial sums of squares in its epilogue. A new cross-attention kernel applies the RMSNorm scale and weight to Q on load, and it handles short deduplicated text keys with a log-multiplicity bias on the last key. This removes the separate rmsnorm pass over the Q activations and the generic attention launch for small key counts. In exchange it adds an extra epilogue store in the GEMM and a new hand-written attention kernel, and it falls back to the old path when the shape conditions are not met.

After: 22.62 frames/s, median of 6. About the same (+0.5%).

```diff
diff --git a/include/inferix_hip.h b/include/inferix_hip.h
--- a/include/inferix_hip.h
+++ b/include/inferix_hip.h
@@ -11,6 +11,7 @@
 #define IFX_EINVAL (-1)
 #define IFX_ELAUNCH (-2)
 #define IFX_EUNSUP (-3)
+#define IFX_EFALLBACK (-4)
 
 typedef uint16_t ifx_bf16;
 
@@ -82,6 +83,14 @@
 
 int ifx_rmsnorm(const ifx_bf16* x, int32_t x_row_stride, ifx_bf16* y, int32_t y_row_stride,
                 const ifx_bf16* w, int32_t rows, int32_t dim, float eps, void* stream);
+
+int ifx_gemm_bf16_rowsq(const ifx_bf16* x, int32_t ldx, const ifx_bf16* w, const ifx_bf16* bias, ifx_bf16* y, int32_t ldy, int32_t M,
+                        int32_t N, int32_t K, float* partials, int32_t ld_partials, void* stream);
+int ifx_rowsq_partials(const ifx_bf16* x, int32_t x_row_stride, float* partials, int32_t ld_partials, int32_t rows, int32_t dim,
+                       void* stream);
+int ifx_xattn_qnorm_fwd(const ifx_bf16* q_raw, int32_t ldq, const float* partials, const ifx_bf16* wq, float eps, ifx_bf16* out,
+                        int32_t ldo, const ifx_kv_view* kv, int32_t q_rows, int32_t heads, int32_t kv_len,
+                        int32_t last_key_multiplicity, float scale, void* stream);
 
 enum { IFX_LN_PLAIN = 0, IFX_LN_AFFINE = 1, IFX_LN_MODULATE = 2 };
 int ifx_layernorm(const ifx_bf16* x, ifx_bf16* y, int32_t rows, int32_t dim, float eps, int32_t mode,
diff --git a/inferix_amd/_hip.py b/inferix_amd/_hip.py
--- a/inferix_amd/_hip.py
+++ b/inferix_amd/_hip.py
@@ -13,6 +13,7 @@
 IFX_EPI_BIAS, IFX_EPI_GELU_TANH, IFX_EPI_RESIDUAL, IFX_EPI_GATE_RES, IFX_EPI_GELU_ERF = 0, 1, 2, 3, 4
 IFX_ACT_SILU, IFX_ACT_TANH = 0, 1
 IFX_Q_FP8_E4M3, IFX_Q_INT8 = 0, 1
+IFX_EFALLBACK = -4
 
 
 class HipLibraryMissing(RuntimeError):
@@ -127,6 +128,9 @@
     "ifx_silu_and_mul": (C.c_int, [_vp, _i32, _vp, _i32, _vp, _i32, _vp, _i32, _i32, _i32, _vp]),
     "ifx_kv_split_rows": (C.c_int, [_vp, _vp, _vp, _i32, _i32, _i32, _i32, _i32, _vp]),
     "ifx_attn_fwd_dedup": (C.c_int, [_vp, _vp, C.POINTER(KvView), _i32, _i32, _i32, _i32, _f32, _vp]),
+    "ifx_gemm_bf16_rowsq": (C.c_int, [_vp, _i32, _vp, _vp, _vp, _i32, _i32, _i32, _i32, _vp, _i32, _vp]),
+    "ifx_rowsq_partials": (C.c_int, [_vp, _i32, _vp, _i32, _i32, _i32, _vp]),
+    "ifx_xattn_qnorm_fwd": (C.c_int, [_vp, _i32, _vp, _vp, _f32, _vp, _i32, C.POINTER(KvView), _i32, _i32, _i32, _i32, _f32, _vp]),
     "ifx_attn_fwd_ranges": (C.c_int, [_vp, _i32, _vp, _i32, C.POINTER(KvView), _i32, _i32, _i32, C.POINTER(_i32), C.POINTER(_i32), _f32, _vp]),
     "ifx_gemm_workspace_bytes": (C.c_int64, [_i32, _i32, _i32]),
     "ifx_gemm_bf16_ws": (C.c_int, [_vp, _i32, _vp, _vp, _vp, _i32, _i32, _i32, _i32, C.POINTER(Epilogue), _vp, C.c_int64, _vp]),
diff --git a/inferix_amd/csrc/ifx_gemm.hip b/inferix_amd/csrc/ifx_gemm.hip
--- a/inferix_amd/csrc/ifx_gemm.hip
+++ b/inferix_amd/csrc/ifx_gemm.hip
@@ -175,6 +175,24 @@
   return ifx_gemm_bf16_ws(x, ldx, w, bias, y, ldy, M, N, K, epi, nullptr, 0, stream);
 }
 
+extern "C" int ifx_gemm_bf16_rowsq(const ifx_bf16* x, int32_t ldx, const ifx_bf16* w, const ifx_bf16* bias, ifx_bf16* y, int32_t ldy,
+                                   int32_t M, int32_t N, int32_t K, float* partials, int32_t ld_partials, void* stream) {
+  IFX_REQUIRE(x && w && y && partials && M >= 0 && N > 0 && K > 0, "ifx_gemm_bf16_rowsq: null/empty operand");
+  IFX_REQUIRE(K % BK == 0, "ifx_gemm_bf16_rowsq: K (%d) must be a multiple of %d", K, BK);
+  IFX_REQUIRE(N % 4 == 0 && ldx % 8 == 0 && ldy % 4 == 0, "ifx_gemm_bf16_rowsq: N %% 4, ldx %% 8, ldy %% 4 required");
+  IFX_REQUIRE(!(((uintptr_t)x | (uintptr_t)w) & 15), "ifx_gemm_bf16_rowsq: x and w must be 16-byte aligned");
+  IFX_REQUIRE(!(((uintptr_t)y | (uintptr_t)bias) & 7) && !((uintptr_t)partials & 3), "ifx_gemm_bf16_rowsq: y and bias must be 8-byte aligned");
+  IFX_REQUIRE(ld_partials >= (N + 63) / 64, "ifx_gemm_bf16_rowsq: ld_partials (%d) must be >= ceil(N / 64)", ld_partials);
+  int mode;
+  EpiArgsP ea;
+  if (const int rc = resolve_epilogue(nullptr, bias, "ifx_gemm_bf16_rowsq", &mode, &ea)) return rc;
+  const GemmRequest r = gemm_request(M, N, K, mode, ea, y, ldy, nullptr, 0);
+  const GemmPlan plan = gemm_plan(r, gemm_variant(), gemm_small_split());
+  if (gemm_variant() != 0 || M < 2048 || N % 64 != 0 || plan.path != kGemmPathPp || plan.tj != 2 || plan.ks != 1 || plan.ws_bytes > 0)
+    return IFX_EFALLBACK;
+  return launch_gemm_pp(x, ldx, w, y, ldy, M, N, K, mode, ea, (hipStream_t)stream, 2, 1, nullptr, 0, partials, ld_partials);
+}
+
 extern "C" int64_t ifx_gemm_workspace_bytes(int32_t M, int32_t N, int32_t K) {
   if (M <= 0 || N <= 0 || K <= 0) return 0;
   const GemmVariant v = gemm_variant_row(gemm_variant());
diff --git a/inferix_amd/csrc/ifx_gemm_epilogue.h b/inferix_amd/csrc/ifx_gemm_epilogue.h
--- a/inferix_amd/csrc/ifx_gemm_epilogue.h
+++ b/inferix_amd/csrc/ifx_gemm_epilogue.h
@@ -126,6 +126,7 @@
 int launch_gemm_w4(const unsigned short* x, int ldx, const unsigned short* w, unsigned short* y, int ldy, int M, int N, int K,
                    int mode, const EpiArgs& ea, hipStream_t s, int splits, void* workspace);
 int launch_gemm_pp(const unsigned short* x, int ldx, const unsigned short* w, unsigned short* y, int ldy, int M, int N, int K,
-                   int mode, const EpiArgsP& ea, hipStream_t s, int tj, int ks, void* workspace, int q8_int8 = 0);
+                   int mode, const EpiArgsP& ea, hipStream_t s, int tj, int ks, void* workspace, int q8_int8 = 0, float* rowsq = nullptr,
+                   int ld_rowsq = 0);
 
 }
diff --git a/inferix_amd/csrc/ifx_gemm_pp.hip b/inferix_amd/csrc/ifx_gemm_pp.hip
--- a/inferix_amd/csrc/ifx_gemm_pp.hip
+++ b/inferix_amd/csrc/ifx_gemm_pp.hip
@@ -2,6 +2,7 @@
 #include <stdlib.h>
 
 #include "ifx_gemm_epilogue.h"
+#include "ifx_rows.h"
 
 #ifndef IFX_PP_TRACE
 #define IFX_PP_TRACE 0
@@ -57,15 +58,18 @@
 };
 }
 
-template <int EPI, int TJ, int KS, int Q8 = 0, int LW = 0>
-__global__ __launch_bounds__(LW ? 768 : 512, LW ? 3 : 2) void gemm_pp_kernel(const unsigned short* __restrict__ x, int ldx,
+template <int EPI, int TJ, int KS, int Q8 = 0, int LWR = 0>
+__global__ __launch_bounds__((LWR & 1) ? 768 : 512, (LWR & 1) ? 3 : 2) void gemm_pp_kernel(const unsigned short* __restrict__ x, int ldx,
                                                          const unsigned short* __restrict__ w, unsigned short* __restrict__ y,
                                                          int ldy, int M, int N, int K, int tiles_m, int total, int per_xcd,
                                                          int wg_per_xcd, EpiArgsP ea, unsigned long long* __restrict__ trace, int dbg,
                                                          float* __restrict__ ws_part, unsigned* __restrict__ ws_flag,
                                                          unsigned* __restrict__ err_word, long long spin_ticks) {
   using namespace gpp;
+  constexpr int LW = LWR & 1;
+  constexpr bool RSQ = (LWR & 2) != 0;
   static_assert(!LW || (TJ == 2 && KS == 1 && Q8 == 0), "the loader-wave form is the unsplit bf16 128-token tile");
+  static_assert(!RSQ || (TJ == 2 && KS == 1 && Q8 == 0 && EPI == IFX_EPI_BIAS), "the row-statistic epilogue is built for the unsplit bf16 128-token tile, bias epilogue");
   dbg = IFX_PP_LAB ? dbg : (dbg & 32);
   constexpr int BM = 64 * TJ;
   constexpr int GM = 4;
@@ -545,6 +549,10 @@
           }
         }
         if (m < M && n_ok) *reinterpret_cast<u16x8*>(yrow + (size_t)(j * 32 + p * 8) * ldo) = o;
+        if constexpr (RSQ) {
+          const float sq = rowsq_group(rowsq8(o));
+          if (cc == 0 && m < M && n_ok) ws_part[(size_t)m * (int)spin_ticks + (e_n0 >> 6)] = sq;
+        }
       }
     }
   };
@@ -758,7 +766,7 @@
 }
 
 int launch_gemm_pp(const unsigned short* x, int ldx, const unsigned short* w, unsigned short* y, int ldy, int M, int N, int K,
-                   int mode, const EpiArgsP& ea, hipStream_t s, int tj, int ks, void* workspace, int q8_int8) {
+                   int mode, const EpiArgsP& ea, hipStream_t s, int tj, int ks, void* workspace, int q8_int8, float* rowsq, int ld_rowsq) {
   using namespace gpp;
   const bool q8 = ea.sa != nullptr;
   IFX_REQUIRE(ea.y2 == nullptr || !(q8 || ea.split_col <= 0 || ea.split_col % BN != 0 || ea.split_col >= N || ea.ldy2 % 8 != 0 || ((uintptr_t)ea.y2 & 15)),
@@ -808,17 +816,26 @@
     if (e) trace = (unsigned long long*)strtoull(e, nullptr, 0);
   }
 #endif
-#define IFX_LAUNCH_PP(E, T, S, Q, L)                                                                                                 \
+#define IFX_LAUNCH_PP_AS(E, T, S, Q, L, WS_PART, SPIN)                                                                               \
   do {                                                                                                                               \
     static bool attr_set = false;                                                                                                    \
     if (!attr_set) {                                                                                                                 \
       (void)hipFuncSetAttribute((const void*)gemm_pp_kernel<E, T, S, Q, L>, hipFuncAttributeMaxDynamicSharedMemorySize, (int)LDS_BYTES); \
       attr_set = true;                                                                                                               \
     }                                                                                                                                \
-    hipLaunchKernelGGL((gemm_pp_kernel<E, T, S, Q, L>), grid, dim3(L ? 768 : 512), LDS_BYTES, s, x, ldx, w, y, ldy, M, N, K, tiles_m, \
-                       total, per_xcd, wg_per_xcd, ea, trace, dbg_launch, ws_part, ws_flag, err_word, spin_ticks);                   \
+    hipLaunchKernelGGL((gemm_pp_kernel<E, T, S, Q, L>), grid, dim3(((L) & 1) ? 768 : 512), LDS_BYTES, s, x, ldx, w, y, ldy, M, N, K, tiles_m, \
+                       total, per_xcd, wg_per_xcd, ea, trace, dbg_launch, WS_PART, ws_flag, err_word, SPIN);                         \
   } while (0)
+#define IFX_LAUNCH_PP(E, T, S, Q, L) IFX_LAUNCH_PP_AS(E, T, S, Q, L, ws_part, spin_ticks)
   const int fmt = !q8 ? 0 : q8_int8 ? 2 : 1;
+  if (rowsq != nullptr) {
+    IFX_REQUIRE(fmt == 0 && tj == 2 && ks == 1 && mode == IFX_EPI_BIAS && ea.y2 == nullptr && ld_rowsq >= N / 64,
+                "ifx_gemm_bf16_rowsq: the row-statistic epilogue needs the unsplit bf16 128-token tile and the bias epilogue");
+    constexpr int E = IFX_EPI_BIAS;
+    if (gemm_pp_variant() != 1) IFX_LAUNCH_PP_AS(E, 2, 1, 0, 3, rowsq, (long long)ld_rowsq);
+    else IFX_LAUNCH_PP_AS(E, 2, 1, 0, 2, rowsq, (long long)ld_rowsq);
+    return check_launch("ifx_gemm_bf16_rowsq(pp)");
+  }
   const int lw = fmt == 0 && tj == 2 && ks == 1 && gemm_pp_variant() != 1;
   int rc = INT_MIN;
 #define IFX_PP_CASE(T, S, Q, L) \
@@ -830,6 +847,7 @@
   IFX_PP_CASE(4, 1, 2, 0) IFX_PP_CASE(3, 1, 2, 0) IFX_PP_CASE(2, 1, 2, 0) IFX_PP_CASE(4, 2, 2, 0)
 #undef IFX_PP_CASE
 #undef IFX_LAUNCH_PP
+#undef IFX_LAUNCH_PP_AS
   IFX_REQUIRE(rc != INT_MIN, q8 ? "ifx_gemm_q8: no ping-pong tile of %d tokens" : "ifx_gemm_bf16: no ping-pong tile of %d tokens", 64 * tj);
   if (rc != IFX_OK) return rc;
   return check_launch("ifx_gemm_bf16(pp)");
diff --git a/inferix_amd/csrc/ifx_norm.hip b/inferix_amd/csrc/ifx_norm.hip
--- a/inferix_amd/csrc/ifx_norm.hip
+++ b/inferix_amd/csrc/ifx_norm.hip
@@ -116,6 +116,22 @@
 }
 
 template <int NCH>
+__global__ __launch_bounds__(256) void rowsq_partials_kernel(const unsigned short* __restrict__ x, int ldx, float* __restrict__ partials,
+                                                             int ldp, int rows, int dim) {
+  const int lane = threadIdx.x & 63;
+  const int r = blockIdx.x * 4 + (threadIdx.x >> 6);
+  if (r >= rows) return;
+  u16x8 xr[NCH];
+  load_chunks<NCH>(xr, x + (size_t)r * ldx, dim, lane);
+#pragma unroll
+  for (int c = 0; c < NCH; ++c) {
+    const int col = c * 512 + lane * 8;
+    const float s = rowsq_group(rowsq8(xr[c]));
+    if ((lane & 7) == 0 && col < dim) partials[(size_t)r * ldp + (col >> 6)] = s;
+  }
+}
+
+template <int NCH>
 __global__ __launch_bounds__(256) void rmsnorm_rope_append_kernel(
     const unsigned short* __restrict__ qkv, int ld, unsigned short* __restrict__ q_out,
     const unsigned short* __restrict__ wq, const unsigned short* __restrict__ wk, RopeArgs ra, int has_rope,
@@ -260,6 +276,18 @@
   if (rows == 0) return IFX_OK;
   return dispatch_norm(dim, [&](auto nch) {
     return launch_rows("ifx_rmsnorm", rmsnorm_kernel<decltype(nch)::value>, rows, stream, x, ldx, y, ldy, w, rows, dim, eps);
+  });
+}
+
+extern "C" int ifx_rowsq_partials(const ifx_bf16* x, int32_t ldx, float* partials, int32_t ld_partials, int32_t rows, int32_t dim,
+                                  void* stream) {
+  IFX_REQUIRE(x && partials && rows >= 0 && dim > 0 && dim % 64 == 0 && ldx % 8 == 0 && ldx >= dim && ld_partials >= dim / 64,
+              "ifx_rowsq_partials: bad arguments (dim %d must be a multiple of 64, ldx %d >= dim, ld_partials %d >= dim / 64)", dim, ldx,
+              ld_partials);
+  if (rows == 0) return IFX_OK;
+  return dispatch_norm(dim, [&](auto nch) {
+    return launch_rows("ifx_rowsq_partials", rowsq_partials_kernel<decltype(nch)::value>, rows, stream, x, ldx, partials, ld_partials, rows,
+                       dim);
   });
 }
 
diff --git a/inferix_amd/csrc/ifx_rows.h b/inferix_amd/csrc/ifx_rows.h
--- a/inferix_amd/csrc/ifx_rows.h
+++ b/inferix_amd/csrc/ifx_rows.h
@@ -42,6 +42,30 @@
     return s;
   }
 };
+
+__device__ __forceinline__ float rowsq8(const u16x8 u) {
+  float s = 0.f;
+#pragma unroll
+  for (int i = 0; i < 8; ++i) {
+    const float v = bf2f(u[i]);
+    s += v * v;
+  }
+  return s;
+}
+__device__ __forceinline__ float rowsq_group(float s) {
+  s += dpp_or<0xB1, 0xf>(0.f, s);
+  s += dpp_or<0x4E, 0xf>(0.f, s);
+  s += dpp_or<0x141, 0xf>(0.f, s);
+  return s;
+}
+__device__ __forceinline__ float rowsq_scale(const float* __restrict__ partials, int groups, int dim, float eps) {
+  float total = partials[0];
+  for (int g = 1; g < groups; ++g) total += partials[g];
+  return 1.0f / sqrtf(total / (float)dim + eps);
+}
+__device__ __forceinline__ unsigned short rowsq_norm(unsigned short v, float rs, unsigned short w) {
+  return f2bf(rbf(bf2f(v) * rs) * bf2f(w));
+}
 
 template <int NCH>
 __device__ __forceinline__ void ln_stats(const Row<NCH>& row, int dim, float eps, int lane, float& mean, float& rstd) {
diff --git a/inferix_amd/csrc/ifx_xattn.hip b/inferix_amd/csrc/ifx_xattn.hip
--- /dev/null
+++ b/inferix_amd/csrc/ifx_xattn.hip
@@ -0,0 +1,249 @@
+#include "ifx_rows.h"
+#include "ifx_attn.h"
+
+namespace ifx {
+
+namespace xa {
+constexpr int QT = 128, KT = 64, HD = 128, MAX_KEYS = 128;
+
+struct Args {
+  const unsigned short* q;
+  const float* partials;
+  const unsigned short* wq;
+  unsigned short* out;
+  const unsigned short* k;
+  const unsigned short* v;
+  KvAddr ka;
+  int q_rows, heads, kv_len, q_tiles, per_xcd, total;
+  int ldq, ldo, dim, groups;
+  int kv_heads, q_per_kv;
+  float eps, last_key_bias, scale_log2;
+};
+
+typedef __attribute__((address_space(3))) void* lds_ptr_t;
+
+__device__ __forceinline__ void dma16(const unsigned short* src, unsigned lds) {
+  asm volatile("s_mov_b32 m0, %0\n\ts_nop 0\n\tglobal_load_lds_dwordx4 %1, off" : : "s"(lds), "v"(src) : "memory");
+}
+}
+
+template <bool PAGED, int G4>
+__global__ __launch_bounds__(256, 2) void xattn_qnorm_kernel(xa::Args A) {
+  using namespace xa;
+  __shared__ __attribute__((aligned(16))) unsigned char smem[65536];
+  const int tid = threadIdx.x, lane = tid & 63;
+  const int wave = __builtin_amdgcn_readfirstlane(tid >> 6);
+  const int hi = lane >> 5, l31 = lane & 31;
+
+  const int xcd = blockIdx.x & 7, slot_i = blockIdx.x >> 3;
+  const int wi = xcd * A.per_xcd + slot_i;
+  if (slot_i >= A.per_xcd || wi >= A.total) return;
+  const int head = wi / A.q_tiles, qt = wi - head * A.q_tiles;
+  const int kv_stride = A.kv_heads * HD;
+  const int kvh = head / A.q_per_kv;
+  const int nkeys = A.kv_len;
+  const int NB = (nkeys + 31) >> 5;
+
+  {
+    const int d_row = lane >> 4, d_pc = lane & 15;
+    const unsigned short* kbase = A.k + kvh * HD;
+    const unsigned short* vbase = A.v + kvh * HD;
+    const unsigned lds0 = (unsigned)(unsigned long long)(lds_ptr_t)smem + wave * 1024;
+    for (int t = 0; t * KT < nkeys; ++t) {
+#pragma unroll
+      for (int r = 0; r < 4; ++r) {
+        const int row = (r * 4 + wave) * 4 + d_row;
+        const int key = min(t * KT + row, nkeys - 1);
+        const size_t off = (size_t)(PAGED ? A.ka.slot(key) : key) * kv_stride;
+        dma16(kbase + off + (d_pc ^ (row & 15)) * 8, lds0 + t * 32768 + r * 4096);
+        dma16(vbase + off + ((((d_pc >> 2) ^ (row & 3)) << 2) | (d_pc & 3)) * 8, lds0 + t * 32768 + 16384 + r * 4096);
+      }
+    }
+  }
+
+  const int qrow = qt * QT + wave * 32 + l31;
+  const int qrow_c = min(qrow, A.q_rows - 1);
+  bf16x8 qf[8];
+  {
+    const unsigned short* qp = A.q + (size_t)qrow_c * A.ldq + head * HD + hi * 8;
+    const unsigned short* wp = A.wq + head * HD + hi * 8;
+    const float* pp = A.partials + (size_t)qrow_c * A.groups;
+    u16x8 qr[8], wv[8];
+#pragma unroll
+    for (int ks = 0; ks < 8; ++ks) qr[ks] = *reinterpret_cast<const u16x8*>(qp + ks * 16);
+#pragma unroll
+    for (int ks = 0; ks < 8; ++ks) wv[ks] = *reinterpret_cast<const u16x8*>(wp + ks * 16);
+    float rs;
+    if constexpr (G4 > 0) {
+      f32x4 pv[G4];
+#pragma unroll
+      for (int i = 0; i < G4; ++i) pv[i] = *reinterpret_cast<const f32x4*>(pp + 4 * i);
+      float total = pv[0][0];
+#pragma unroll
+      for (int i = 0; i < G4; ++i)
+#pragma unroll
+        for (int e = (i == 0 ? 1 : 0); e < 4; ++e) total += pv[i][e];
+      rs = 1.0f / sqrtf(total / (float)A.dim + A.eps);
+    } else {
+      rs = rowsq_scale(pp, A.groups, A.dim, A.eps);
+    }
+#pragma unroll
+    for (int ks = 0; ks < 8; ++ks) {
+      u16x8 n;
+#pragma unroll
+      for (int e = 0; e < 8; ++e) n[e] = rowsq_norm(qr[ks][e], rs, wv[ks][e]);
+      qf[ks] = __builtin_bit_cast(bf16x8, n);
+    }
+  }
+  asm volatile("s_waitcnt vmcnt(0)" ::: "memory");
+  __builtin_amdgcn_s_barrier();
+
+  const int kswz = l31 & 15;
+  const int vi = lane & 15, vg1 = (lane >> 4) & 1;
+  const int v_rowq = vi >> 2;
+  const int v_in = (vg1 << 5) | ((vi & 3) << 3);
+  auto ldK = [&](bf16x8(&f)[4], int b, int kh) {
+    const unsigned char* krow = smem + (b >> 1) * 32768 + (32 * (b & 1) + l31) * 256;
+#pragma unroll
+    for (int k4 = 0; k4 < 4; ++k4) f[k4] = *reinterpret_cast<const bf16x8*>(krow + (((2 * (4 * kh + k4) + hi) ^ kswz) << 4));
+  };
+  auto ldV = [&](bf16x8(&f)[4], int b, int s2) {
+    const unsigned char* vr0 = smem + (b >> 1) * 32768 + 16384 + (32 * (b & 1) + 16 * s2 + 4 * hi + v_rowq) * 256 + v_in;
+    const unsigned char* vr1 = vr0 + 8 * 256;
+#pragma unroll
+    for (int d = 0; d < 4; ++d) {
+      const int ch = (d ^ v_rowq) << 6;
+      const bf16x4 t0 = __builtin_amdgcn_ds_read_tr16_b64_v4bf16((bf16x4 __attribute__((address_space(3)))*)(vr0 + ch));
+      const bf16x4 t1 = __builtin_amdgcn_ds_read_tr16_b64_v4bf16((bf16x4 __attribute__((address_space(3)))*)(vr1 + ch));
+      f[d] = __builtin_shufflevector(t0, t1, 0, 1, 2, 3, 4, 5, 6, 7);
+    }
+  };
+
+  float sc[4][16];
+  float mx = -INFINITY;
+#pragma unroll
+  for (int b = 0; b < 4; ++b) {
+    if (b < NB) {
+      bf16x8 kA[4], kB[4];
+      ldK(kA, b, 0);
+      ldK(kB, b, 1);
+      f32x16 s;
+#pragma unroll
+      for (int r = 0; r < 16; ++r) s[r] = 0.f;
+#pragma unroll
+      for (int k4 = 0; k4 < 4; ++k4) s = __builtin_amdgcn_mfma_f32_32x32x16_bf16(kA[k4], qf[k4], s, 0, 0, 0);
+#pragma unroll
+      for (int k4 = 0; k4 < 4; ++k4) s = __builtin_amdgcn_mfma_f32_32x32x16_bf16(kB[k4], qf[4 + k4], s, 0, 0, 0);
+      const int kidx = 32 * b + 4 * hi;
+      const bool tail = 32 * b + 32 >= nkeys;
+#pragma unroll
+      for (int r = 0; r < 16; ++r) {
+        const int kk = kidx + (r & 3) + 8 * (r >> 2);
+        float sv = s[r];
+        if (tail) {
+          sv = kk == nkeys - 1 ? sv + A.last_key_bias : sv;
+          sv = kk >= nkeys ? -INFINITY : sv;
+        }
+        sc[b][r] = sv;
+        mx = fmaxf(mx, sv);
+      }
+      __builtin_amdgcn_sched_barrier(0);
+    }
+  }
+  const float m = attn_half_max(mx);
+  const float c2 = A.scale_log2, mc = m * c2;
+  float l_run = 0.f;
+  bf16x8 p[4][2];
+#pragma unroll
+  for (int b = 0; b < 4; ++b) {
+    if (b < NB) {
+#pragma unroll
+      for (int r = 0; r < 16; ++r) {
+        const float e = __builtin_amdgcn_exp2f(sc[b][r] * c2 - mc);
+        l_run += e;
+        p[b][r >> 3][r & 7] = static_cast<__bf16>(e);
+      }
+    }
+  }
+  f32x16 o[4];
+#pragma unroll
+  for (int d = 0; d < 4; ++d)
+#pragma unroll
+    for (int r = 0; r < 16; ++r) o[d][r] = 0.f;
+#pragma unroll
+  for (int b = 0; b < 4; ++b) {
+    if (b < NB) {
+      bf16x8 vA[4], vB[4];
+      ldV(vA, b, 0);
+      ldV(vB, b, 1);
+#pragma unroll
+      for (int d = 0; d < 4; ++d) o[d] = __builtin_amdgcn_mfma_f32_32x32x16_bf16(vA[d], p[b][0], o[d], 0, 0, 0);
+#pragma unroll
+      for (int d = 0; d < 4; ++d) o[d] = __builtin_amdgcn_mfma_f32_32x32x16_bf16(vB[d], p[b][1], o[d], 0, 0, 0);
+      __builtin_amdgcn_sched_barrier(0);
+    }
+  }
+
+  const float l_tot = l_run + __shfl_xor(l_run, 32, 64);
+  const float inv = 1.0f / l_tot;
+  if (qrow < A.q_rows) {
+    unsigned short* op = A.out + (size_t)qrow * A.ldo + head * HD + 4 * hi;
+#pragma unroll
+    for (int d = 0; d < 4; ++d)
+#pragma unroll
+      for (int g = 0; g < 4; ++g) {
+        u16x4 w;
+#pragma unroll
+        for (int e = 0; e < 4; ++e) w[e] = f2bf(o[d][4 * g + e] * inv);
+        *reinterpret_cast<u16x4*>(op + 32 * d + 8 * g) = w;
+      }
+  }
+}
+
+}
+
+using namespace ifx;
+
+extern "C" int ifx_xattn_qnorm_fwd(const ifx_bf16* q_raw, int32_t ldq, const float* partials, const ifx_bf16* wq, float eps, ifx_bf16* out,
+                                   int32_t ldo, const ifx_kv_view* kv, int32_t q_rows, int32_t heads, int32_t kv_len,
+                                   int32_t last_key_multiplicity, float scale, void* stream) {
+  IFX_REQUIRE(q_raw && partials && wq && out && kv && kv->k && kv->v, "ifx_xattn_qnorm_fwd: null argument");
+  IFX_REQUIRE(kv->head_dim == xa::HD, "ifx_xattn_qnorm_fwd: head_dim %d not built (128 only)", kv->head_dim);
+  IFX_REQUIRE(kv_len >= 1 && kv_len <= xa::MAX_KEYS, "ifx_xattn_qnorm_fwd: kv_len %d outside [1, %d] (longer contexts: ifx_rmsnorm + ifx_attn_fwd_dedup)",
+              kv_len, xa::MAX_KEYS);
+  IFX_REQUIRE(heads > 0 && kv->kv_heads > 0 && heads % kv->kv_heads == 0, "ifx_xattn_qnorm_fwd: heads %d is not a multiple of kv_heads %d", heads,
+              kv->kv_heads);
+  const int dim = heads * xa::HD;
+  IFX_REQUIRE(ldq >= dim && ldo >= dim && ldq % 8 == 0 && ldo % 8 == 0, "ifx_xattn_qnorm_fwd: row strides (%d, %d) must be >= heads * 128 and multiples of 8",
+              ldq, ldo);
+  IFX_REQUIRE(!(((uintptr_t)q_raw | (uintptr_t)wq) & 15) && !((uintptr_t)out & 7) && !((uintptr_t)partials & 3),
+              "ifx_xattn_qnorm_fwd: q_raw and wq must be 16-byte aligned, out 8-byte aligned");
+  IFX_REQUIRE(q_rows >= 0 && kv_len <= kv->num_slots && last_key_multiplicity >= 1, "ifx_xattn_qnorm_fwd: kv_len %d exceeds the capacity %d, or multiplicity %d < 1",
+              kv_len, kv->num_slots, last_key_multiplicity);
+  IFX_REQUIRE(!kv->page_table || kv->page_size > 0, "ifx_xattn_qnorm_fwd: page_size must be > 0");
+  if (q_rows == 0) return IFX_OK;
+  xa::Args a;
+  a.q = q_raw, a.partials = partials, a.wq = wq, a.out = out, a.k = kv->k, a.v = kv->v;
+  a.ka = KvAddr{kv->page_table, kv->page_size, kv->page_table ? 0 : kv->seg_split, kv->page_table ? 0 : kv->seg_delta};
+  a.q_rows = q_rows, a.heads = heads, a.kv_len = kv_len;
+  a.q_tiles = (q_rows + xa::QT - 1) / xa::QT;
+  a.total = a.q_tiles * heads;
+  a.per_xcd = (a.total + 7) / 8;
+  a.ldq = ldq, a.ldo = ldo, a.dim = dim, a.groups = dim / 64;
+  a.kv_heads = kv->kv_heads, a.q_per_kv = heads / kv->kv_heads;
+  a.eps = eps;
+  const float sc = scale > 0.f ? scale : 0.08838834764831845f;
+  a.scale_log2 = sc * 1.4426950408889634f;
+  a.last_key_bias = last_key_multiplicity > 1 ? logf((float)last_key_multiplicity) / sc : 0.f;
+  const dim3 grid(a.per_xcd * 8), block(256);
+  hipStream_t s = (hipStream_t)stream;
+  const bool paged = kv->page_table || kv->seg_split > 0;
+  const bool vec = a.groups % 4 == 0 && !((uintptr_t)partials & 15);
+#define IFX_XA_LAUNCH(P, G) hipLaunchKernelGGL((xattn_qnorm_kernel<P, G>), grid, block, 0, s, a)
+  if (paged) IFX_XA_LAUNCH(true, 0);
+  else if (vec && a.groups == 24) IFX_XA_LAUNCH(false, 6);
+  else if (vec && a.groups == 4) IFX_XA_LAUNCH(false, 1);
+  else IFX_XA_LAUNCH(false, 0);
+#undef IFX_XA_LAUNCH
+  return check_launch("ifx_xattn_qnorm_fwd");
+}
diff --git a/inferix_amd/hip_ops.py b/inferix_amd/hip_ops.py
--- a/inferix_amd/hip_ops.py
+++ b/inferix_amd/hip_ops.py
@@ -868,6 +868,55 @@
     return out
 
 
+XATTN_QNORM_MAX_KEYS = 128
+
+
+def xattn_qnorm_eligible(kv_len: int, head_dim: int, dim: int) -> bool:
+    return head_dim == 128 and 1 <= kv_len <= XATTN_QNORM_MAX_KEYS and dim % 128 == 0
+
+
+def rowsq_partials(x: torch.Tensor, partials: Optional[torch.Tensor] = None) -> torch.Tensor:
+    rows, dim, ldx = _rows2d(x, "x")
+    assert dim % 64 == 0
+    if partials is None:
+        partials = torch.empty(rows, dim // 64, dtype=torch.float32, device=x.device)
+    assert partials.dim() == 2 and partials.shape[0] >= rows and partials.shape[1] == dim // 64 and partials.stride(1) == 1
+    with _timed("rowsq_partials", 0.0, 2.0 * rows * dim):
+        _hip.check(_hip.load().ifx_rowsq_partials(_dev(x, "x"), ldx, _dev(partials, "partials", torch.float32), partials.stride(0), rows, dim,
+                                                  _stream()), "ifx_rowsq_partials")
+    return partials
+
+
+def linear_rowsq(x: torch.Tensor, w: torch.Tensor, bias: Optional[torch.Tensor], out: torch.Tensor, partials: torch.Tensor) -> bool:
+    lib = _hip.load()
+    M, K, ldx = _rows2d(x, "x")
+    N = w.shape[0]
+    assert w.shape[1] == K and w.is_contiguous()
+    _, _, ldy = _rows2d(out, "out")
+    assert partials.dim() == 2 and partials.shape[0] >= M and partials.shape[1] * 64 >= N and partials.stride(1) == 1
+    with _timed("gemm", 2.0 * M * N * K, 2.0 * (M * K + N * K + M * N)):
+        rc = lib.ifx_gemm_bf16_rowsq(_dev(x, "x"), ldx, _dev(w, "w"), _dev(bias, "bias") if bias is not None else None, _dev(out, "out"), ldy,
+                                     M, N, K, _dev(partials, "partials", torch.float32), partials.stride(0), _stream())
+    if rc == _hip.IFX_EFALLBACK:
+        return False
+    _hip.check(rc, "ifx_gemm_bf16_rowsq")
+    return True
+
+
+def xattn_qnorm(q_raw: torch.Tensor, partials: torch.Tensor, wq: torch.Tensor, eps: float, kv: KvCacheView, kv_len: int,
+                last_key_multiplicity: int, out: torch.Tensor, heads: int, scale: float = 0.0, tag: str = "attn") -> torch.Tensor:
+    assert q_raw.dim() == 2 and out.dim() == 2 and q_raw.stride(1) == 1 and out.stride(1) == 1
+    rows = q_raw.shape[0]
+    assert partials.dim() == 2 and partials.shape == (rows, heads * 2) and partials.is_contiguous()
+    ks = kv.struct()
+    nk = kv_len - 1 + last_key_multiplicity
+    with _timed(tag, 4.0 * rows * nk * heads * 128, 0.0):
+        _hip.check(_hip.load().ifx_xattn_qnorm_fwd(_dev(q_raw, "q_raw"), q_raw.stride(0), _dev(partials, "partials", torch.float32),
+                                                   _dev(wq, "wq"), float(eps), _dev(out, "out"), out.stride(0), C.byref(ks), rows, heads,
+                                                   int(kv_len), int(last_key_multiplicity), float(scale), _stream()), "ifx_xattn_qnorm_fwd")
+    return out
+
+
 def vit_head_prep(qkv: torch.Tensor, *, batch: int, heads: int, cls_tokens: int, norm: bool, eps: float = 1e-5,
                   sin: Optional[torch.Tensor] = None, cos: Optional[torch.Tensor] = None) -> torch.Tensor:
     rows, width, ld = _rows2d(qkv, "qkv")
diff --git a/inferix_amd/wan/causal_model.py b/inferix_amd/wan/causal_model.py
--- a/inferix_amd/wan/causal_model.py
+++ b/inferix_amd/wan/causal_model.py
@@ -114,6 +114,7 @@
         self._scratch: Dict[Tuple, torch.Tensor] = {}
         self.cross_dedup = True
         self._cross_dedup: Dict[str, Tuple[int, int]] = {}
+        self.xattn_qnorm = True
         self._roll_scratch: Optional[torch.Tensor] = None
         self.v_direct = os.environ.get("IFX_V_DIRECT", "1") != "0"
         self._temb_cache: Dict[Tuple, Tuple] = {}
@@ -181,6 +182,14 @@
         self._temb_cache.clear()
         return self
 
+    def _buf_f32(self, name: str, *shape) -> torch.Tensor:
+        key = (self._chain, name, shape, "f32")
+        b = self._scratch.get(key)
+        if b is None:
+            b = torch.empty(*shape, dtype=torch.float32, device=self.device_)
+            self._scratch[key] = b
+        return b
+
     def _buf(self, name: str, *shape) -> torch.Tensor:
         key = (self._chain, name, shape)
         b = self._scratch.get(key)
@@ -270,6 +279,19 @@
             return ops.linear_q8(xq, xs, w[key + "_q"], w[key + "_s"], w[key + "_b"], fmt, **kw)
         ops.layernorm(x, self.eps, out=h, **norm_kw)
         return ops.linear(h, w[key + "_w"], w[key + "_b"], **kw)
+
+    def _cross_q_rowsq(self, w: Dict[str, torch.Tensor], xact: torch.Tensor, h: torch.Tensor, qb: torch.Tensor) -> torch.Tensor:
+        rows, d = qb.shape
+        parts = self._buf_f32("qsq", rows, d // 64)
+        if "cq_q" in w:
+            self._norm_lin(w, "cq", xact, h, dict(gamma=w["n3_w"], beta=w["n3_b"]), out=qb)
+            ops.rowsq_partials(qb, parts)
+            return parts
+        ops.layernorm(xact, self.eps, out=h, gamma=w["n3_w"], beta=w["n3_b"])
+        if not ops.linear_rowsq(h, w["cq_w"], w["cq_b"], qb, parts):
+            ops.linear(h, w["cq_w"], w["cq_b"], out=qb)
+            ops.rowsq_partials(qb, parts)
+        return parts
 
     def _run_block(self, l: int, xact: torch.Tensor, El: torch.Tensor, st: dict, meta: dict, cmeta: dict,
                    kv_cache_manager, kv_cache_requests) -> None:
@@ -375,14 +397,24 @@
                     self.index_trace.append((int(smp["current_start"]), int(stp.global_end), int(stp.local_end)))
         self._lin(w, "o", ab, epilogue=_hip.IFX_EPI_GATE_RES, residual=xact, mod=El, gate_slot=2,
                   rows_per_group=rows_per_group, out=xact)
-        self._norm_lin(w, "cq", xact, h, dict(gamma=w["n3_w"], beta=w["n3_b"]), out=qb)
-        ops.rmsnorm(qb, w["cnq"], self.eps, out=qb)
+        groups = []
         b = 0
         while b < len(samples):
             req = samples[b]["req"]
             nb = 1
             while b + nb < len(samples) and samples[b + nb]["req"] is req:
                 nb += 1
+            nkeys, mult = self._cross_dedup.get(req.request_id, (self.text_len, 1)) if self.cross_dedup else (self.text_len, 1)
+            groups.append((b, nb, nkeys, mult))
+            b += nb
+        fused = self.xattn_qnorm and all(ops.xattn_qnorm_eligible(nk, hd, d) for _, _, nk, _ in groups)
+        if fused:
+            parts = self._cross_q_rowsq(w, xact, h, qb)
+        else:
+            self._norm_lin(w, "cq", xact, h, dict(gamma=w["n3_w"], beta=w["n3_b"]), out=qb)
+            ops.rmsnorm(qb, w["cnq"], self.eps, out=qb)
+        for b, nb, nkeys, mult in groups:
+            req = samples[b]["req"]
             cview = self._kv_view(kv_cache_manager, req, blk.kv_cache_manager.cross_name)
             if not cmeta["is_init"]:
                 ci = samples[b]["ctx_index"]
@@ -390,13 +422,15 @@
                 kx = self._lin(w, "ck", cb)
                 ops.rmsnorm(kx, w["cnk"], self.eps, out=cview.k.view(self.text_len, d))
                 self._lin(w, "cv", cb, out=cview.v.view(self.text_len, d))
-            nkeys, mult = self._cross_dedup.get(req.request_id, (self.text_len, 1)) if self.cross_dedup else (self.text_len, 1)
+            if fused:
+                ops.xattn_qnorm(qb[b * N:(b + nb) * N], parts[b * N:(b + nb) * N], w["cnq"], self.eps, cview, nkeys, mult,
+                                ab[b * N:(b + nb) * N], H, tag="attn_cross")
+                continue
             qv, av = qb[b * N:(b + nb) * N].view(nb * N, H, hd), ab[b * N:(b + nb) * N].view(nb * N, H, hd)
             if mult > 1:
                 ops.attention_dedup(qv, cview, nkeys, mult, out=av, tag="attn_cross")
             else:
                 ops.attention(qv, cview, self.text_len, out=av, tag="attn_cross")
-            b += nb
         cmeta["is_init"] = True
         self._lin(w, "co", ab, epilogue=_hip.IFX_EPI_RESIDUAL, residual=xact, out=xact)
         self._norm_lin(w, "f0", xact, h, dict(mod=El, shift_slot=3, scale_slot=4, rows_per_group=rows_per_group),
```
